# Amos-Chen98/neo-planner

Measured on AMD Instinct MI355X. Metric: trajectories/sec (batched replan), higher is better.
Workload: dtype f32x; 1 GPU; cfg2: 40 x 4096 trajectories x 20 waypoints per step per GPU, 1 x 300^3 f32 ESDF per GPU (trilinear, pillars + 80 canopy boxes), each optimised to L-BFGS-B termination; batch_per_launch=4096, pieces=21, dims=3, esdf_voxels=27000000, layout=brick, parallelism=scene-sharded x1, launches_in_flight_per_gpu=4

## Files before the change

include/neo_planner.h:

```cpp
#ifndef NEO_PLANNER_H
#define NEO_PLANNER_H

#include <stddef.h>
#include <stdint.h>

#ifdef __cplusplus
extern "C" {
#endif

#define NEO_ABI_VERSION 1
#define NEO_MAX_PIECES 64
#define NEO_MAX_DIM 3
#define NEO_LBFGS_M 10

typedef struct neo_ctx neo_ctx;

enum {
  NEO_OK = 0,
  NEO_ERR_INVALID = 1,
  NEO_ERR_HIP = 2,
  NEO_ERR_NO_MAP = 3,
  NEO_ERR_UNSUPPORTED = 4,
};

enum {
  NEO_TRAJ_CONVERGED_GRAD = 0,
  NEO_TRAJ_CONVERGED_F = 1,
  NEO_TRAJ_ABNORMAL = 2,
  NEO_TRAJ_MAXITER = 3,
  NEO_TRAJ_NUMERIC_RANGE = 4,
  NEO_TRAJ_NONFINITE = 5,
  NEO_TRAJ_BAD_SCENE = 6,
  NEO_TRAJ_SUSPENDED = 7,
};
#define NEO_TRAJ_FLAG_COLLISION 0x100

enum {
  NEO_INTERP_NEAREST_2D_REF = 0,
  NEO_INTERP_TRILINEAR_3D = 1,
};

enum { NEO_F64 = 0, NEO_F32 = 1, NEO_F16 = 2 };

enum {
  NEO_LAYOUT_LINEAR = 0,
  NEO_LAYOUT_YZ4 = 1,
  NEO_LAYOUT_CELL8 = 2,
  NEO_LAYOUT_BRICK = 3,
};

typedef struct neo_params {
  double v_max;
  double T_min;
  double T_max;
  double safe_dis;
  double delta_t;
  double weights[4];
  double collision_cost_tol;
  double ftol;
  double gtol;
  int32_t maxls;
  int32_t maxiter;
  int32_t maxfun;
  int32_t bugcompat_stale_T;
  int32_t sample_dtype;
  int32_t flags;
} neo_params;

#define NEO_FLAG_ONE_WAVE_PER_SIMD 32
#define NEO_FLAG_TWO_WAVES_PER_SIMD 64
#define NEO_FLAG_LANE_GROUPS 128
#define NEO_FLAG_F32_SOLVE 2048

int neo_abi_version(void);
int neo_ctx_create(int device_id, void *stream, neo_ctx **out);
int neo_ctx_destroy(neo_ctx *ctx);
const char *neo_last_error(neo_ctx *ctx);
int neo_params_default(neo_params *p);
int neo_params_set(neo_ctx *ctx, const neo_params *p);
int neo_ctx_synchronize(neo_ctx *ctx);
int neo_ctx_set_stream(neo_ctx *ctx, void *stream);

int neo_esdf_upload_2d(neo_ctx *ctx, int scene_id, const double *dist, const double *grad_x,
                       const double *grad_y, int width, int height, double resolution,
                       double origin_x, double origin_y);
int neo_esdf_build_2d(neo_ctx *ctx, int scene_id, const int8_t *occupancy, int width, int height,
                      double resolution, double origin_x, double origin_y, double *out_dist,
                      double *out_grad_x, double *out_grad_y);
int neo_esdf_build_2d_batch_dev(neo_ctx *ctx, const int32_t *scene_ids, int n, const int8_t *occupancy, int width,
                                int height, double resolution, const double *origins);
int neo_esdf_upload_3d(neo_ctx *ctx, int scene_id, const void *dist, int src_dtype,
                       int src_is_device, int nx, int ny, int nz, double resolution,
                       const double origin[3], int store_dtype, int layout);
int neo_esdf_build_3d(neo_ctx *ctx, int scene_id, const uint8_t *occupancy, int occ_is_device, int nx,
                      int ny, int nz, double resolution, const double origin[3], int store_dtype,
                      int layout, float *out_dist);
#define NEO_EDT_GENERIC_LINES 1
int neo_esdf_build_config(neo_ctx *ctx, int flags);
int neo_esdf_drop(neo_ctx *ctx, int scene_id);
int neo_esdf_query(neo_ctx *ctx, int scene_id, int n, const double *pts, double *dist, double *grad);

int neo_cost_grad_batch(neo_ctx *ctx, int scene_id, int B, int M, int D, const double *x,
                        const double *head, const double *tail, double *cost, double *costs4,
                        double *grad, double *coeffs, int32_t *status);
int neo_cost_grad_batch_dev(neo_ctx *ctx, int scene_id, int B, int M, int D, const double *x,
                            const double *head, const double *tail, double *cost, double *costs4,
                            double *grad, double *coeffs, int32_t *status);

int neo_sampled_terms_batch(neo_ctx *ctx, int scene_id, int B, int M, int D, const double *coeffs,
                            const double *ts, double *costs2, double *grad_C, double *grad_T);
int neo_sampled_terms_batch_dev(neo_ctx *ctx, int scene_id, int B, int M, int D, const double *coeffs,
                                const double *ts, double *costs2, double *grad_C, double *grad_T);
int neo_sampled_terms_batch_f32(neo_ctx *ctx, int scene_id, int B, int M, int D, const float *coeffs,
                                const double *ts, double *costs2, float *grad_C, float *grad_T);
int neo_sampled_terms_batch_f32_dev(neo_ctx *ctx, int scene_id, int B, int M, int D, const float *coeffs,
                                    const double *ts, double *costs2, float *grad_C, float *grad_T);

int neo_optimize_batch(neo_ctx *ctx, int scene_id, const int32_t *scene_ids, int B, int M, int D,
                       double *x, const double *head, const double *tail, double *costs4,
                       double *costs4_last, int32_t *nit, int32_t *nfev, int32_t *status);
int neo_optimize_batch_dev(neo_ctx *ctx, int scene_id, const int32_t *scene_ids, int B, int M,
                           int D, double *x, const double *head, const double *tail,
                           double *costs4, double *costs4_last, int32_t *nit, int32_t *nfev,
                           int32_t *status);
int neo_optimize_batch_from_dev(neo_ctx *ctx, int scene_id, const int32_t *scene_ids, int B, int M,
                                int D, const double *x0, double *x, const double *head,
                                const double *tail, double *costs4, double *costs4_last, int32_t *nit,
                                int32_t *nfev, int32_t *status);
size_t neo_optimize_state_bytes(int M, int D);
int neo_optimize_batch_budget_dev(neo_ctx *ctx, int scene_id, int B, int M, int D, const double *x0, double *x,
                                  const double *head, const double *tail, double *costs4, double *costs4_last,
                                  int32_t *nit, int32_t *nfev, int32_t *status, void *state, int eval_budget,
                                  const int32_t *subset, int n_subset, int resume);
int neo_scene_slot(neo_ctx *ctx, int scene_id);
size_t neo_optimize_workspace_bytes(int B, int M, int D);

int neo_eval_traj_batch(neo_ctx *ctx, int B, int M, int D, const double *x, const double *head,
                        const double *tail, double hz, int K, double *state, int32_t *count);

enum {
  NEO_AUDIT_PATH_LENGTH = 0,
  NEO_AUDIT_FEASIBILITY = 1,
  NEO_AUDIT_COLLISION = 2,
  NEO_AUDIT_WEIGHTED = 3,
  NEO_AUDIT_MIN_CLEARANCE = 4,
  NEO_AUDIT_T_MIN_CLEARANCE = 5,
  NEO_AUDIT_MAX_SPEED = 6,
  NEO_AUDIT_MAX_ACC = 7,
  NEO_AUDIT_T_FIRST_UNSAFE = 8,
  NEO_AUDIT_DURATION = 9,
  NEO_AUDIT_FIELDS = 10,
};
#define NEO_AUDIT_FLAG_UNSAFE 1
#define NEO_AUDIT_FLAG_METRIC_FAIL 2
#define NEO_AUDIT_FLAG_OUTSIDE_MAP 4
#define NEO_AUDIT_FLAG_NONFINITE 8
int neo_audit_traj_batch(neo_ctx *ctx, int scene_id, const int32_t *scene_ids, int B, int M, int D,
                         const double *x, const double *head, const double *tail, double hz,
                         const double *weights3, double *audit, int32_t *count, int32_t *flags);
int neo_audit_traj_batch_dev(neo_ctx *ctx, int scene_id, const int32_t *scene_ids, int B, int M, int D,
                             const double *x, const double *head, const double *tail, double hz,
                             const double *weights3, double *audit, int32_t *count, int32_t *flags);

#define NEO_GEO_FLAG_NO_PATH 1
#define NEO_GEO_FLAG_START_OUTSIDE 2
#define NEO_GEO_FLAG_CAPPED 4
#define NEO_GEO_FLAG_PATH_TRUNCATED 8
#define NEO_GEO_FLAG_BAD_SCENE 16
int neo_geo_search_batch(neo_ctx *ctx, int scene_id, const int32_t *scene_ids, int B, const double *start,
                         const double *target, int max_expansions, int path_cap, double *key_pts, double *path,
                         int32_t *path_len, double *path_cost, int32_t *expansions, int32_t *flags);
int neo_geo_search_batch_dev(neo_ctx *ctx, int scene_id, const int32_t *scene_ids, int B, const double *start,
                             const double *target, int max_expansions, int path_cap, double *key_pts, double *path,
                             int32_t *path_len, double *path_cost, int32_t *expansions, int32_t *flags);
int neo_geo_prune_batch(neo_ctx *ctx, int scene_id, const int32_t *scene_ids, int B, const double *paths,
                        const int32_t *path_len, int path_stride, double *key_pts);
int neo_geo_workspace_budget(neo_ctx *ctx, size_t bytes);

#define NEO_FLEET_FLAG_TARGET_CAPPED 1
#define NEO_FLEET_FLAG_CMD_FULL 2
#define NEO_FLEET_FLAG_BAD_SCENE 4
#define NEO_FLEET_FLAG_SPLICE_FAILED 8
#define NEO_FLEET_FLAG_ABANDONED 16
int neo_fleet_target_batch(neo_ctx *ctx, int scene_id, const int32_t *scene_ids, int B, const int32_t *subset,
                           int n_subset, const double *cur_pos, const double *goal, const double *jitter,
                           double longitu_step_dis, double lateral_step_length, double move_vel, double *tail,
                           int32_t *near_goal, int32_t *lateral_steps, int32_t *flags);
int neo_fleet_target_batch_dev(neo_ctx *ctx, int scene_id, const int32_t *scene_ids, int B, const int32_t *subset,
                               int n_subset, const double *cur_pos, const double *goal, const double *jitter,
                               double longitu_step_dis, double lateral_step_length, double move_vel, double *tail,
                               int32_t *near_goal, int32_t *lateral_steps, int32_t *flags);
int neo_fleet_advance_dev(neo_ctx *ctx, int B, const int32_t *subset, int n_subset, const double *cmd, int cap,
                          const int32_t *cmd_len, int32_t *cmd_index, int32_t *future_index, int step, int ahead,
                          double *cur_pos, double *head);
int neo_fleet_pose_dev(neo_ctx *ctx, int B, const int32_t *subset, int n_subset, const double *cmd, int cap,
                       const int32_t *cmd_len, const int32_t *cmd_index, const double *cur_pos, const double *goal,
                       double eye_z, double *pose);
int neo_fleet_splice_dev(neo_ctx *ctx, int B, const int32_t *subset, int n_subset, int M, const double *x,
                         const double *head, const double *tail, const int32_t *solved, double hz, int first,
                         double *cmd, int cap, int32_t *cmd_len, int32_t *cmd_index, int32_t *future_index,
                         int32_t *flags);
int neo_fleet_audit_batch(neo_ctx *ctx, int scene_id, const int32_t *scene_ids, int B, const int32_t *subset,
                          int n_subset, const double *cmd, int cap, const int32_t *n_flown, int stride, double cmd_hz,
                          const double *weights3, double *audit, int32_t *count, int32_t *flags);
int neo_fleet_audit_batch_dev(neo_ctx *ctx, int scene_id, const int32_t *scene_ids, int B, const int32_t *subset,
                              int n_subset, const double *cmd, int cap, const int32_t *n_flown, int stride,
                              double cmd_hz, const double *weights3, double *audit, int32_t *count, int32_t *flags);

int neo_record_state_dev(neo_ctx *ctx, int B, const int32_t *subset, int n_subset, const double *cmd, int cap,
                         const int32_t *cmd_len, const int32_t *cmd_index, const double *head, double *cur_vel);
int neo_record_commit_dev(neo_ctx *ctx, int B, const int32_t *subset, int n_subset, int M, const double *x,
                          const double *head, const double *tail, const int32_t *solved, const double *pose,
                          const double *cur_vel, const uint8_t *staging, int width, int height,
                          const int32_t *mission_ids, int tick, int round, int capacity, double *motion,
                          double *wpts_local, double *tau, double *pose_rows, int32_t *meta, uint8_t *images,
                          int32_t *row_of, int32_t *n_rows, int32_t *dropped);

#define NEO_BATCH_MAX_CANDIDATES 8
int neo_batch_candidates(neo_ctx *ctx, int B, const int32_t *subset, int n_subset, int M, int D, int K,
                         const double *head, const double *tail, const int32_t *slots, const double *tau,
                         const double *lateral_offsets, double *x0, double *head_k, double *tail_k, int32_t *slots_k);
int neo_batch_candidates_dev(neo_ctx *ctx, int B, const int32_t *subset, int n_subset, int M, int D, int K,
                             const double *head, const double *tail, const int32_t *slots, const double *tau,
                             const double *lateral_offsets, double *x0, double *head_k, double *tail_k,
                             int32_t *slots_k);
int neo_batch_select(neo_ctx *ctx, int B, const int32_t *subset, int n_subset, int M, int D, int K, const double *x_k,
                     const double *costs4_k, const double *costs4_last_k, const int32_t *nit_k, const int32_t *nfev_k,
                     const int32_t *status_k, const double *weights4, int32_t *chosen, double *cand_cost,
                     int32_t *solved, double *x, double *costs4, double *costs4_last, int32_t *nit, int32_t *nfev,
                     int32_t *status, int32_t *nit_total, int32_t *opt_runs, int32_t *fallback, int32_t *n_fallback);
int neo_batch_select_dev(neo_ctx *ctx, int B, const int32_t *subset, int n_subset, int M, int D, int K,
                         const double *x_k, const double *costs4_k, const double *costs4_last_k, const int32_t *nit_k,
                         const int32_t *nfev_k, const int32_t *status_k, const double *weights4, int32_t *chosen,
                         double *cand_cost, int32_t *solved, double *x, double *costs4, double *costs4_last,
                         int32_t *nit, int32_t *nfev, int32_t *status, int32_t *nit_total, int32_t *opt_runs,
                         int32_t *fallback, int32_t *n_fallback);

int neo_plan_guess(neo_ctx *ctx, int B, const int32_t *subset, int n_subset, int M, int D, const double *head,
                   const double *tail, const int32_t *slots, const double *x_init, const double *noise,
                   const double *frac, const double *tau, double *x0, double *head_k, double *tail_k, int32_t *slots_k);
int neo_plan_guess_dev(neo_ctx *ctx, int B, const int32_t *subset, int n_subset, int M, int D, const double *head,
                       const double *tail, const int32_t *slots, const double *x_init, const double *noise,
                       const double *frac, const double *tau, double *x0, double *head_k, double *tail_k,
                       int32_t *slots_k);
int neo_plan_merge(neo_ctx *ctx, int B, const int32_t *subset, int n_subset, int M, int D, int reset, const double *x_k,
                   const double *costs4_k, const double *costs4_last_k, const int32_t *nit_k, const int32_t *nfev_k,
                   const int32_t *status_k, double *x, double *costs4, double *costs4_last, int32_t *nit, int32_t *nfev,
                   int32_t *status, int32_t *attempts, int64_t *nit_total, int32_t *solved, int32_t *failed,
                   int32_t *n_failed, int32_t *bad_scene);
int neo_plan_merge_dev(neo_ctx *ctx, int B, const int32_t *subset, int n_subset, int M, int D, int reset,
                       const double *x_k, const double *costs4_k, const double *costs4_last_k, const int32_t *nit_k,
                       const int32_t *nfev_k, const int32_t *status_k, double *x, double *costs4, double *costs4_last,
                       int32_t *nit, int32_t *nfev, int32_t *status, int32_t *attempts, int64_t *nit_total,
                       int32_t *solved, int32_t *failed, int32_t *n_failed, int32_t *bad_scene);

#define NEO_DEPTH_MAX_BOXES 1024
int neo_depth_render_batch(neo_ctx *ctx, int width, int height, double focal_px, double max_range, const double *boxes,
                           const int32_t *box_begin, int n_scenes, const int32_t *scene_index, int B, const double *pose,
                           float *depth_m, uint8_t *depth_u8, float *depth_max);
int neo_depth_render_batch_dev(neo_ctx *ctx, int width, int height, double focal_px, double max_range,
                               const double *boxes, const int32_t *box_begin, int n_scenes, const int32_t *scene_index,
                               int B, const double *pose, float *depth_m, uint8_t *depth_u8, float *depth_max);
int neo_depth_box_test_counter(neo_ctx *ctx, uint64_t *dev_count);

int neo_onboard_integrate_batch(neo_ctx *ctx, int B, const int32_t *subset, int n_subset, const float *depth_m,
                                const double *pose, int width, int height, double focal_px, double max_range, int grid_w,
                                int grid_h, double res, const double *origins, double sensor_range, double z_lo,
                                double z_hi, int hit, int miss, int lo, int hi, int8_t *logodds, int8_t *occupancy,
                                int32_t *changed);
int neo_onboard_integrate_batch_dev(neo_ctx *ctx, int B, const int32_t *subset, int n_subset, const float *depth_m,
                                    const double *pose, int width, int height, double focal_px, double max_range,
                                    int grid_w, int grid_h, double res, const double *origins, double sensor_range,
                                    double z_lo, double z_hi, int hit, int miss, int lo, int hi, int8_t *logodds,
                                    int8_t *occupancy, int32_t *changed);

enum { NEO_KERNEL_EVAL = 0, NEO_KERNEL_OPTIMIZE = 1, NEO_KERNEL_ESDF_BUILD = 2, NEO_KERNEL_ESDF_SAMPLE = 3, NEO_KERNEL_COUNT = 4 };
int neo_profile_enable(neo_ctx *ctx, int on);
int neo_optimize_sample_counter(neo_ctx *ctx, int64_t *dev_counts);
int neo_optimize_progress_counter(neo_ctx *ctx, int32_t *counter);
int neo_optimize_trace(neo_ctx *ctx, double *dev_trace, int cap);
int neo_optimize_trace_xg(neo_ctx *ctx, double *dev_xg, int cap);
int neo_optimize_dispatch_order(neo_ctx *ctx, const int32_t *dev_order, int B);
size_t neo_effort_order_scratch_bytes(int B);
int neo_effort_order_dev(neo_ctx *ctx, int B, int M, int D, const double *x0, const double *head, const double *tail,
                         void *scratch, int32_t *order);
int neo_optimize_dispatch_order_host(neo_ctx *ctx, const int32_t *host_order, int B);
int neo_pack_results_dev(neo_ctx *ctx, int B, int n, const double *x, const double *costs4, const double *weights4,
                         float *out);
int neo_sampled_terms_dispatch_order(neo_ctx *ctx, const int32_t *order, int on_device, int B);
int neo_profile_read(neo_ctx *ctx, int kernel, int64_t *launches, double *total_ms);
int neo_profile_reset(neo_ctx *ctx);

#ifdef __cplusplus
}
#endif
#endif
```

neo-planner_amd/csrc/neo_abi.hip:

```cpp
#include <cstring>
#include "neo_host.hpp"
#include <rocprim/device/device_radix_sort.hpp>
#include "neo_kernels.hpp"

namespace neo {

template <int D>
__global__ __launch_bounds__(kWave) void traj_state_kernel(int B, int M, DevParams prm,
                                                            const double *__restrict__ x,
                                                            const double *__restrict__ head,
                                                            const double *__restrict__ tail, double hz, int K,
                                                            double *__restrict__ state, int *__restrict__ count) {
  __shared__ double xs[kSlots * kWave];
  __shared__ double cs[kWave * 6 * D];
  __shared__ double tcum[kWave + 1];
  const int b = blockIdx.x;
  if (b >= B) return;
  struct NoMap {};
  struct NoLookup {
    __device__ explicit NoLookup(const NoMap &) {}
  };
  DevParams p = prm;
  NoMap nm;
  DevBackend<D, kSlots, double, NoMap, NoLookup> be(p, nm);
// ... 1747 lines not shown
  HostStage st(c, kStagedUpTo);
  const RowRefs fk = stage_rows_in(st, a.packed, P, (size_t)a.n);
  const auto fsub = st.in_optional(subset, (size_t)n_subset);
  const RowRefs fo = stage_rows_inout(st, a.out, bs, (size_t)a.n);
  const auto oat = st.inout(attempts, bs);
  const auto ont = st.inout(nit_total, bs);
  const auto oso = st.inout(solved, bs);
  const auto ofl = st.out(failed, P), onl = st.out(n_failed, 1), obs = st.out(bad_scene, 1);
  rc = st.upload();
  if (rc) return rc;
  const RunRowsIn k = as_const(staged_rows(st, fk));
  const RunRows o = staged_rows(st, fo);
  rc = neo_plan_merge_dev(c, B, st.dev(fsub), n_subset, M, D, reset, k.x, k.costs4, k.costs4_last, k.nit, k.nfev, k.status, o.x,
                          o.costs4, o.costs4_last, o.nit, o.nfev, o.status, st.dev(oat), st.dev(ont), st.dev(oso), st.dev(ofl),
                          st.dev(onl), st.dev(obs));
  if (rc) return rc;
  return st.download();
}

static int geo_check(neo_ctx *c, int B, const double *start, const double *target, int max_expansions, int path_cap,
                     const double *key_pts, const double *path, const int32_t *path_len, const double *path_cost,
                     const int32_t *expansions, const int32_t *flags) {
  if (!c) return NEO_ERR_INVALID;
  if (B < 1) return fail_locked(c, NEO_ERR_INVALID, "geo: B must be >= 1");
  if (max_expansions < 0 || path_cap < 0 || (path && path_cap < 1))
    return fail_locked(c, NEO_ERR_INVALID, "geo: max_expansions and path_cap must be >= 0 (path_cap >= 1 with a path)");
  if (!start || !target || !key_pts || !path_len || !path_cost || !expansions || !flags)
    return fail_locked(c, NEO_ERR_INVALID, "geo: null buffer");
  return NEO_OK;
}

static int geo_scene_kind(neo_ctx *c, int scene_id) {
  auto it = c->maps.find(scene_id);
  if (it == c->maps.end()) return fail(c, NEO_ERR_NO_MAP, "geo: no ESDF for this scene");
  if (it->second.kind != 0) return fail(c, NEO_ERR_UNSUPPORTED, "geo: the A* warm start needs a 2-D map");
  return NEO_OK;
}

int neo_geo_search_batch_dev(neo_ctx *c, int scene_id, const int32_t *scene_ids, int B, const double *start,
                             const double *target, int max_expansions, int path_cap, double *key_pts, double *path,
                             int32_t *path_len, double *path_cost, int32_t *expansions, int32_t *flags) {
  int rc = geo_check(c, B, start, target, max_expansions, path_cap, key_pts, path, path_len, path_cost, expansions, flags);
  if (rc) return rc;
  std::lock_guard<std::recursive_mutex> g(c->mu);
  hipSetDevice(c->device);
  rc = rebuild_tables(c);
  if (rc) return rc;
  rc = geo_scene_kind(c, scene_id);
  if (rc) return rc;
  const GeoArgs ga{B, scene_ids, start, target, max_expansions, path ? path_cap : 0, key_pts, path, path_cost,
                   path_len, expansions, flags};
  return geo_search(c, scene_id, ga);
}

int neo_geo_search_batch(neo_ctx *c, int scene_id, const int32_t *scene_ids, int B, const double *start,
                         const double *target, int max_expansions, int path_cap, double *key_pts, double *path,
                         int32_t *path_len, double *path_cost, int32_t *expansions, int32_t *flags) {
  int rc = geo_check(c, B, start, target, max_expansions, path_cap, key_pts, path, path_len, path_cost, expansions, flags);
  if (rc) return rc;
  std::lock_guard<std::recursive_mutex> g(c->mu);
  hipSetDevice(c->device);
  rc = rebuild_tables(c);
  if (rc) return rc;
  const size_t bs = (size_t)B, pc = path ? (size_t)path_cap : 0;
  std::vector<int> slots;
  rc = scene_ids ? scene_slots(c, scene_ids, bs, true, slots) : geo_scene_kind(c, scene_id);
  if (rc) return rc;
  HostStage st(c, 0);
  const auto fs = st.in(start, 2 * bs), ft = st.in(target, 2 * bs);
  const auto fsl = st.in(scene_ids ? slots.data() : nullptr, bs);
  const auto fk = st.out(key_pts, 8 * bs), fc = st.out(path_cost, bs), fp = st.out(path, 2 * bs * pc);
  const auto fl = st.out(path_len, bs), fe = st.out(expansions, bs), ff = st.out(flags, bs);
  rc = st.upload();
  if (rc) return rc;
  rc = neo_geo_search_batch_dev(c, scene_ids ? scene_ids[0] : scene_id, scene_ids ? st.dev(fsl) : nullptr, B, st.dev(fs),
                                st.dev(ft), max_expansions, path_cap, st.dev(fk), path ? st.dev(fp) : nullptr, st.dev(fl),
                                st.dev(fc), st.dev(fe), st.dev(ff));
  if (rc) return rc;
  return st.download();
}

int neo_geo_prune_batch(neo_ctx *c, int scene_id, const int32_t *scene_ids, int B, const double *paths,
                        const int32_t *path_len, int path_stride, double *key_pts) {
  if (!c) return NEO_ERR_INVALID;
  if (B < 1 || path_stride < 1) return fail_locked(c, NEO_ERR_INVALID, "geo prune: B and path_stride must be >= 1");
  if (!paths || !path_len || !key_pts) return fail_locked(c, NEO_ERR_INVALID, "geo prune: null buffer");
  for (int i = 0; i < B; ++i)
    if (path_len[i] < 1 || path_len[i] > path_stride)
      return fail_locked(c, NEO_ERR_INVALID, "geo prune: path_len must be in [1, path_stride]");
  std::lock_guard<std::recursive_mutex> g(c->mu);
  hipSetDevice(c->device);
  int rc = rebuild_tables(c);
  if (rc) return rc;
  const size_t bs = (size_t)B, ps = (size_t)path_stride;
  std::vector<int> slots;
  rc = scene_ids ? scene_slots(c, scene_ids, bs, true, slots) : geo_scene_kind(c, scene_id);
  if (rc) return rc;
  HostStage st(c, 0);
  const auto fp = st.in(paths, 2 * bs * ps);
  const auto fl = st.in(path_len, bs), fsl = st.in(scene_ids ? slots.data() : nullptr, bs);
  const auto fk = st.out(key_pts, 8 * bs);
  rc = st.upload();
  if (rc) return rc;
  rc = geo_prune(c, scene_ids ? scene_ids[0] : scene_id, B, scene_ids ? st.dev(fsl) : nullptr, st.dev(fp), st.dev(fl),
                 path_stride, st.dev(fk));
  if (rc) return rc;
  return st.download();
}

int neo_geo_workspace_budget(neo_ctx *c, size_t bytes) {
  if (!c) return NEO_ERR_INVALID;
  std::lock_guard<std::recursive_mutex> g(c->mu);
  c->geo.budget = bytes;
  return NEO_OK;
}

int neo_optimize_progress_counter(neo_ctx *c, int32_t *counter) {
  if (!c) return NEO_ERR_INVALID;
  std::lock_guard<std::recursive_mutex> g(c->mu);
  c->progress = counter;
  return NEO_OK;
}

int neo_optimize_sample_counter(neo_ctx *c, int64_t *dev_counts) {
  if (!c) return NEO_ERR_INVALID;
  std::lock_guard<std::recursive_mutex> g(c->mu);
  c->sample_counter = reinterpret_cast<long long *>(dev_counts);
  return NEO_OK;
}

int neo_optimize_trace(neo_ctx *c, double *dev_trace, int cap) {
  if (!c || cap < 0) return NEO_ERR_INVALID;
  std::lock_guard<std::recursive_mutex> g(c->mu);
  if (dev_trace && cap > 0 && c->trace_xg && c->trace_cap != cap)
    return fail(c, NEO_ERR_INVALID, "neo_optimize_trace: cap differs from neo_optimize_trace_xg's");
  c->trace = (dev_trace && cap > 0) ? dev_trace : nullptr;
  if (c->trace) c->trace_cap = cap;
  if (!c->trace_xg && !c->trace) c->trace_cap = 0;
  return NEO_OK;
}

int neo_optimize_trace_xg(neo_ctx *c, double *dev_xg, int cap) {
  if (!c || cap < 0) return NEO_ERR_INVALID;
  std::lock_guard<std::recursive_mutex> g(c->mu);
  if (dev_xg && cap > 0 && c->trace && c->trace_cap != cap)
    return fail(c, NEO_ERR_INVALID, "neo_optimize_trace_xg: cap differs from neo_optimize_trace's");
  c->trace_xg = (dev_xg && cap > 0) ? dev_xg : nullptr;
  if (c->trace_xg) c->trace_cap = cap;
  if (!c->trace_xg && !c->trace) c->trace_cap = 0;
  return NEO_OK;
}

int neo_optimize_dispatch_order(neo_ctx *c, const int32_t *dev_order, int B) {
  if (!c || B < 0) return NEO_ERR_INVALID;
  std::lock_guard<std::recursive_mutex> g(c->mu);
  c->dispatch_order = (dev_order && B > 0) ? dev_order : nullptr;
  c->order_B = c->dispatch_order ? B : 0;
  return NEO_OK;
}

int neo_optimize_dispatch_order_host(neo_ctx *c, const int32_t *host_order, int B) {
  if (!c || B < 0) return NEO_ERR_INVALID;
  std::lock_guard<std::recursive_mutex> g(c->mu);
  hipSetDevice(c->device);
  if (!host_order || B == 0) {
    c->dispatch_order = nullptr;
    c->order_B = 0;
    return NEO_OK;
  }
  if ((size_t)B > c->order_cap) {
    HIPCHK(c, hipStreamSynchronize(c->stream));
    if (c->order_buf) hipFree(c->order_buf);
    c->order_buf = nullptr;
    c->order_cap = 0;
    HIPCHK(c, hipMalloc((void **)&c->order_buf, (size_t)B * sizeof(int)));
    c->order_cap = (size_t)B;
  }
  HIPCHK(c, hipMemcpyAsync(c->order_buf, host_order, (size_t)B * sizeof(int), hipMemcpyHostToDevice, c->stream));
  HIPCHK(c, hipStreamSynchronize(c->stream));
  c->dispatch_order = c->order_buf;
  c->order_B = B;
  return NEO_OK;
}

namespace neo {
__global__ void pack_results_kernel(int B, int n, const double *__restrict__ x, const double *__restrict__ costs4, double w0, double w1,
                                    double w2, double w3, float *__restrict__ out) {
  const size_t i = (size_t)blockIdx.x * blockDim.x + threadIdx.x;
  const size_t row = i / (size_t)(n + 5);
  if (row >= (size_t)B) return;
  const int col = (int)(i - row * (size_t)(n + 5));
  const double *c4 = costs4 + row * 4;
  double v;
  if (col < n)
    v = x[row * (size_t)n + col];
  else if (col == n)
    v = ((c4[0] * w0 + c4[1] * w1) + c4[2] * w2) + c4[3] * w3;
  else
    v = c4[col - n - 1];
  out[i] = (float)v;
}
}

int neo_pack_results_dev(neo_ctx *c, int B, int n, const double *x, const double *costs4, const double *weights4, float *out) {
  if (!c || B < 0 || n < 1) return NEO_ERR_INVALID;
  if (!x || !costs4 || !weights4 || !out) return fail_locked(c, NEO_ERR_INVALID, "null buffer");
  if (B == 0) return NEO_OK;
  std::lock_guard<std::recursive_mutex> g(c->mu);
  hipSetDevice(c->device);
  const size_t total = (size_t)B * (size_t)(n + 5);
  hipLaunchKernelGGL(neo::pack_results_kernel, dim3((unsigned)((total + 255) / 256)), dim3(256), 0, c->stream, B, n, x, costs4,
                     weights4[0], weights4[1], weights4[2], weights4[3], out);
  HIPCHK(c, hipGetLastError());
  return NEO_OK;
}

namespace neo {
__global__ void effort_keys_kernel(int B, int M, int D, double T_min, double T_max, double v_max, const double *__restrict__ x0,
                                   const double *__restrict__ head, const double *__restrict__ tail, double *__restrict__ keys,
                                   int *__restrict__ idx) {
  const int b = blockIdx.x * blockDim.x + threadIdx.x;
  if (b >= B) return;
  idx[b] = b;
  const int nq = D * (M - 1), n = nq + M;
  double sum = 0.0;
  for (int p = 0; p < M; ++p) sum += (T_max - T_min) / (1.0 + exp(-x0[(size_t)b * n + nq + p])) + T_min;
  double d2 = 0.0;
  for (int d = 0; d < D; ++d) {
    const double e = tail[(size_t)b * 3 * D + d] - head[(size_t)b * 3 * D + d];
    d2 += e * e;
  }
  const double dist = sqrt(d2);
  const double k = dist == dist ? sum * v_max / fmax(dist, 1e-9) : NAN;
  keys[b] = isfinite(k) ? k : 0.0;
}
}

static size_t effort_sort_temp_bytes(int B) {
  size_t tb = 0;
  (void)rocprim::radix_sort_pairs_desc(nullptr, tb, (const double *)nullptr, (double *)nullptr, (const int *)nullptr, (int *)nullptr,
                                       (unsigned)B, 0, 64, (hipStream_t)0);
  return (tb + 255) / 256 * 256;
}

static size_t align256(size_t v) { return (v + 255) / 256 * 256; }

size_t neo_effort_order_scratch_bytes(int B) {
  if (B <= 0) return 0;
  return align256((size_t)B * 16) + align256((size_t)B * 4) + effort_sort_temp_bytes(B);
}

int neo_effort_order_dev(neo_ctx *c, int B, int M, int D, const double *x0, const double *head, const double *tail, void *scratch,
                         int32_t *order) {
  int rc = check_shape(c, B, M, D);
  if (rc) return rc;
  if (!x0 || !head || !tail || !scratch || !order) return fail_locked(c, NEO_ERR_INVALID, "null buffer");
  if (((uintptr_t)scratch) & 255) return fail_locked(c, NEO_ERR_INVALID, "scratch must be 256-byte aligned");
  if (B == 0) return NEO_OK;
  std::lock_guard<std::recursive_mutex> g(c->mu);
  hipSetDevice(c->device);
  double *keys = static_cast<double *>(scratch), *keys_out = keys + B;
  int *idx = reinterpret_cast<int *>(reinterpret_cast<char *>(scratch) + align256((size_t)B * 16));
  void *temp = reinterpret_cast<char *>(idx) + align256((size_t)B * 4);
  size_t tb = effort_sort_temp_bytes(B);
  hipLaunchKernelGGL(neo::effort_keys_kernel, dim3((unsigned)((B + 255) / 256)), dim3(256), 0, c->stream, B, M, D, c->params.T_min,
                     c->params.T_max, c->params.v_max, x0, head, tail, keys, idx);
  HIPCHK(c, rocprim::radix_sort_pairs_desc(temp, tb, (const double *)keys, keys_out, (const int *)idx, (int *)order, (unsigned)B, 0, 64,
                                           c->stream));
  HIPCHK(c, hipGetLastError());
  return NEO_OK;
}

int neo_sampled_terms_dispatch_order(neo_ctx *c, const int32_t *order, int on_device, int B) {
  if (!c || B < 0) return NEO_ERR_INVALID;
  std::lock_guard<std::recursive_mutex> g(c->mu);
  hipSetDevice(c->device);
  if (!order || B == 0) {
    c->sample_order_B = 0;
    return NEO_OK;
  }
  if ((size_t)B > c->sample_order_cap) {
    HIPCHK(c, hipStreamSynchronize(c->stream));
    if (c->sample_order) hipFree(c->sample_order);
    c->sample_order = nullptr;
    c->sample_order_cap = 0;
    c->sample_order_B = 0;
    HIPCHK(c, hipMalloc((void **)&c->sample_order, (size_t)B * sizeof(int)));
    c->sample_order_cap = (size_t)B;
  }
  HIPCHK(c, hipMemcpyAsync(c->sample_order, order, (size_t)B * sizeof(int),
                           on_device ? hipMemcpyDeviceToDevice : hipMemcpyHostToDevice, c->stream));
  HIPCHK(c, hipStreamSynchronize(c->stream));
  c->sample_order_B = B;
  return NEO_OK;
}

int neo_esdf_build_config(neo_ctx *c, int flags) {
  if (!c || (flags & ~NEO_EDT_GENERIC_LINES)) return NEO_ERR_INVALID;
  std::lock_guard<std::recursive_mutex> g(c->mu);
  c->edt_flags = flags;
  return NEO_OK;
}

int neo_profile_enable(neo_ctx *c, int on) {
  if (!c) return NEO_ERR_INVALID;
  std::lock_guard<std::recursive_mutex> g(c->mu);
  c->profile = on != 0;
  return NEO_OK;
}

int neo_profile_read(neo_ctx *c, int kernel, int64_t *launches, double *total_ms) {
  if (!c || kernel < 0 || kernel >= NEO_KERNEL_COUNT) return NEO_ERR_INVALID;
  std::lock_guard<std::recursive_mutex> g(c->mu);
  hipSetDevice(c->device);
  drain_profile(c);
  if (launches) *launches = c->prof[kernel].launches;
  if (total_ms) *total_ms = c->prof[kernel].ms;
  return NEO_OK;
}

int neo_profile_reset(neo_ctx *c) {
  if (!c) return NEO_ERR_INVALID;
  std::lock_guard<std::recursive_mutex> g(c->mu);
  hipSetDevice(c->device);
  drain_profile(c);
  for (int k = 0; k < NEO_KERNEL_COUNT; ++k) {
    c->prof[k].launches = 0;
    c->prof[k].ms = 0.0;
  }
  return NEO_OK;
}

}
```

neo-planner_amd/csrc/neo_device.hpp:

```cpp
#pragma once
#include <type_traits>
#include <hip/hip_runtime.h>
#include <hip/hip_fp16.h>

#include "../../include/neo_planner.h"
#include "neo_wave.hpp"

namespace neo {

constexpr int kSlots = 4;

struct DevParams {
  double v_max, T_min, T_max, safe_dis, delta_t;
  double w[4];
  double coll_tol;
  double ftol, gtol;
  int maxls, maxiter, maxfun, stale_T;
  int dbg;
  struct F32 {
    float T_min, T_span;
    float dt, inv_dt;
    float vmax2, safe;
    float w[4];
  } f;
// ... 92 lines not shown
    if (!a.inside) return Real(10000);
    g[0] = (Real)q.r.y;
    g[1] = (Real)q.r.z;
    return (Real)q.r.x;
  }
  template <int D>
  __device__ __forceinline__ Real fetch(const Real (&pos)[D], Real (&g)[D], bool &inside) const {
    const Addr a = prepare<D>(pos);
    inside = a.inside;
    return finish<D>(a, load(a), g);
  }
};

template <typename E>
__device__ __forceinline__ float elem_to_float(E v);
template <>
__device__ __forceinline__ float elem_to_float<float>(float v) { return v; }
template <>
__device__ __forceinline__ float elem_to_float<__half>(__half v) { return __half2float(v); }

typedef unsigned long long u64_align4 __attribute__((aligned(4)));
typedef unsigned int u32_align2 __attribute__((aligned(2)));
template <typename E>
__device__ __forceinline__ void load_pair(const E *p, float &a, float &b);
template <>
__device__ __forceinline__ void load_pair<float>(const float *p, float &a, float &b) {
  const unsigned long long u = *reinterpret_cast<const u64_align4 *>(p);
  a = __uint_as_float((unsigned int)(u & 0xffffffffull));
  b = __uint_as_float((unsigned int)(u >> 32));
}
__device__ __forceinline__ void buffer_load_pair_f32(__amdgpu_buffer_rsrc_t rsrc, unsigned int off, unsigned int soff,
                                                     float &a, float &b) {
  const auto v = __builtin_amdgcn_raw_buffer_load_b64(rsrc, (int)off, (int)soff, 0);
  a = __uint_as_float(v[0]);
  b = __uint_as_float(v[1]);
}
template <>
__device__ __forceinline__ void load_pair<__half>(const __half *p, float &a, float &b) {
  const unsigned int u = *reinterpret_cast<const u32_align2 *>(p);
  a = __half2float(__ushort_as_half((unsigned short)(u & 0xffffu)));
  b = __half2float(__ushort_as_half((unsigned short)(u >> 16)));
}

template <typename Real, typename E, int LAYOUT>
struct Lookup3D {
  const Map3D &m;
  __amdgpu_buffer_rsrc_t rsrc;
  float inv, off[3], hi[3];
  __device__ __forceinline__ explicit Lookup3D(const Map3D &m_)
      : m(m_), rsrc(__builtin_amdgcn_make_buffer_rsrc(const_cast<void *>(m_.data), 0, (int)m_.bytes, 0x00020000)) {
    inv = m_.f_inv;
#pragma unroll
    for (int k = 0; k < 3; ++k) {
      off[k] = m_.f_off[k];
      hi[k] = m_.f_hi[k];
    }
  }
  struct Addr {
    int i0[3];
    Real fr[3];
    bool inside;
  };
  struct Raw {
    float c[2][2][2];
  };

  template <int D>
  __device__ __forceinline__ Addr prepare(const Real (&pos)[D], bool on = true) const {
#pragma clang fp contract(on)
    static_assert(D == 3, "the 3-D map needs D = 3");
    const int n[3] = {m.nx, m.ny, m.nz};
    const double org[3] = {m.ox, m.oy, m.oz};
    Addr a;
    a.inside = on;
    if constexpr (sizeof(Real) == 4) {
#pragma unroll
      for (int k = 0; k < 3; ++k) {
        const float um = fmaf(pos[k], inv, off[k]);
        if (!(um >= -0.5f && um < hi[k])) a.inside = false;
        const int i = min(max((int)floorf(um), 0), n[k] - 2);
        a.i0[k] = i;
        a.fr[k] = __builtin_amdgcn_fmed3f(um - (float)i, 0.0f, 1.0f);
      }
      if (!a.inside) a.i0[0] = a.i0[1] = a.i0[2] = 0;
      return a;
    }
#pragma unroll
    for (int k = 0; k < 3; ++k) {
      Real u = (Real)(((double)pos[k] - org[k]) * m.d_inv);
      if (!(u >= Real(0) && u < (Real)n[k])) a.inside = false;
      u -= Real(0.5);
      const int i = min(max((int)floor(u), 0), n[k] - 2);
      a.i0[k] = i;
      a.fr[k] = fmin(fmax(u - (Real)i, Real(0)), Real(1));
    }
    if (!a.inside) a.i0[0] = a.i0[1] = a.i0[2] = 0;
    return a;
  }
  __device__ __forceinline__ Raw load(const Addr &a) const {
    const E *vox = static_cast<const E *>(m.data);
    Raw q;
    if (LAYOUT == 2 || (LAYOUT == 9 && m.layout == NEO_LAYOUT_CELL8)) {
      const unsigned int cell = __umul24(__umul24((unsigned)a.i0[2], (unsigned)m.ny) + (unsigned)a.i0[1], (unsigned)m.nx) +
                                (unsigned)a.i0[0];
      if constexpr (sizeof(E) == 4) {
        const auto lo = __builtin_amdgcn_raw_buffer_load_b128(rsrc, (int)(cell * 32u), 0, 0);
        const auto hi = __builtin_amdgcn_raw_buffer_load_b128(rsrc, (int)(cell * 32u + 16u), 0, 0);
        q.c[0][0][0] = __uint_as_float(lo[0]); q.c[0][0][1] = __uint_as_float(lo[1]);
        q.c[0][1][0] = __uint_as_float(lo[2]); q.c[0][1][1] = __uint_as_float(lo[3]);
        q.c[1][0][0] = __uint_as_float(hi[0]); q.c[1][0][1] = __uint_as_float(hi[1]);
        q.c[1][1][0] = __uint_as_float(hi[2]); q.c[1][1][1] = __uint_as_float(hi[3]);
      } else {
        const auto v = __builtin_amdgcn_raw_buffer_load_b128(rsrc, (int)(cell * 16u), 0, 0);
#pragma unroll
        for (int w = 0; w < 4; ++w) {
          q.c[w >> 1][w & 1][0] = __half2float(__ushort_as_half((unsigned short)(v[w] & 0xffffu)));
          q.c[w >> 1][w & 1][1] = __half2float(__ushort_as_half((unsigned short)(v[w] >> 16)));
        }
      }
    } else if (LAYOUT == 3 || (LAYOUT == 9 && m.layout == NEO_LAYOUT_BRICK)) {
      constexpr int SHX = sizeof(E) == 4 ? 1 : 2, CX = (1 << SHX) + 1;
      const unsigned int bx = (unsigned)a.i0[0] >> SHX, by = (unsigned)a.i0[1] >> 1, bz = (unsigned)a.i0[2] >> 1;
      const unsigned int lx = (unsigned)a.i0[0] & ((1u << SHX) - 1u), ly = (unsigned)a.i0[1] & 1u, lz = (unsigned)a.i0[2] & 1u;
      const unsigned int blk = __umul24(__umul24(bz, (unsigned)m.nby) + by, (unsigned)m.nbx) + bx;
      const unsigned int in_line = (lz * 3u + ly) * (unsigned)CX + lx;
#pragma unroll
      for (int dz = 0; dz < 2; ++dz)
#pragma unroll
        for (int dy = 0; dy < 2; ++dy) {
          const unsigned int so = (unsigned)((dz * 3 + dy) * CX);
          if constexpr (sizeof(E) == 4) {
            const auto v = __builtin_amdgcn_raw_buffer_load_b64(rsrc, (int)(blk * 128u + in_line * 4u + so * 4u), 0, 0);
            q.c[dz][dy][0] = __uint_as_float(v[0]);
            q.c[dz][dy][1] = __uint_as_float(v[1]);
          } else {
            load_pair<E>(vox + blk * 64u + in_line + so, q.c[dz][dy][0], q.c[dz][dy][1]);
          }
        }
    } else if (LAYOUT == 0 || (LAYOUT == 9 && m.layout == NEO_LAYOUT_LINEAR)) {
      const unsigned int base = __umul24(__umul24((unsigned)a.i0[2], (unsigned)m.ny) + (unsigned)a.i0[1], (unsigned)m.nx) +
                                (unsigned)a.i0[0];
      const unsigned int sy = (unsigned)m.nx, sz = (unsigned)m.nx * (unsigned)m.ny;
#pragma unroll
      for (int dz = 0; dz < 2; ++dz)
#pragma unroll
        for (int dy = 0; dy < 2; ++dy) {
          const unsigned int so = (dy ? sy : 0u) + (dz ? sz : 0u);
          if constexpr (sizeof(E) == 4)
            buffer_load_pair_f32(rsrc, base * 4u, so * 4u, q.c[dz][dy][0], q.c[dz][dy][1]);
          else
            load_pair<E>(vox + base + so, q.c[dz][dy][0], q.c[dz][dy][1]);
        }
    } else {
      const unsigned int cell = __umul24(__umul24((unsigned)a.i0[2], (unsigned)m.ny) + (unsigned)a.i0[1], (unsigned)m.nx) +
                                (unsigned)a.i0[0];
      if constexpr (sizeof(E) == 4) {
        const auto lo = __builtin_amdgcn_raw_buffer_load_b128(rsrc, (int)(cell * 16u), 0, 0);
        const auto hi = __builtin_amdgcn_raw_buffer_load_b128(rsrc, (int)(cell * 16u + 16u), 0, 0);
        q.c[0][0][0] = __uint_as_float(lo[0]); q.c[0][1][0] = __uint_as_float(lo[1]);
        q.c[1][0][0] = __uint_as_float(lo[2]); q.c[1][1][0] = __uint_as_float(lo[3]);
        q.c[0][0][1] = __uint_as_float(hi[0]); q.c[0][1][1] = __uint_as_float(hi[1]);
        q.c[1][0][1] = __uint_as_float(hi[2]); q.c[1][1][1] = __uint_as_float(hi[3]);
      } else {
        const auto v = __builtin_amdgcn_raw_buffer_load_b128(rsrc, (int)(cell * 8u), 0, 0);
#pragma unroll
        for (int dx = 0; dx < 2; ++dx)
#pragma unroll
          for (int dz = 0; dz < 2; ++dz) {
            const unsigned int u = v[2 * dx + dz];
            q.c[dz][0][dx] = __half2float(__ushort_as_half((unsigned short)(u & 0xffffu)));
            q.c[dz][1][dx] = __half2float(__ushort_as_half((unsigned short)(u >> 16)));
          }
      }
    }
    return q;
  }
  template <int D>
  __device__ __forceinline__ Real finish(const Addr &a, const Raw &q, Real (&g)[D]) const {
#pragma clang fp contract(on)
#pragma unroll
    for (int d = 0; d < D; ++d) g[d] = Real(0);
    if (!a.inside) return Real(10000);
    const Real fx = a.fr[0], fy = a.fr[1], fz = a.fr[2];
    const Real inv_res = sizeof(Real) == 4 ? (Real)m.f_inv : (Real)m.d_inv;
    const Real c000 = (Real)q.c[0][0][0], c100 = (Real)q.c[0][0][1], c010 = (Real)q.c[0][1][0], c110 = (Real)q.c[0][1][1];
    const Real c001 = (Real)q.c[1][0][0], c101 = (Real)q.c[1][0][1], c011 = (Real)q.c[1][1][0], c111 = (Real)q.c[1][1][1];
    const Real dx00 = c100 - c000, dx10 = c110 - c010, dx01 = c101 - c001, dx11 = c111 - c011;
    const Real c00 = c000 + fx * dx00, c10 = c010 + fx * dx10;
    const Real c01 = c001 + fx * dx01, c11 = c011 + fx * dx11;
    const Real c0 = c00 + fy * (c10 - c00), c1 = c01 + fy * (c11 - c01);
    const Real dx0 = dx00 + fy * (dx10 - dx00), dx1 = dx01 + fy * (dx11 - dx01);
    const Real dy0 = c10 - c00, dy1 = c11 - c01;
    g[0] = (dx0 + fz * (dx1 - dx0)) * inv_res;
    g[1] = (dy0 + fz * (dy1 - dy0)) * inv_res;
    g[2] = (c1 - c0) * inv_res;
    return c0 + fz * (c1 - c0);
  }
  template <int D>
  __device__ __forceinline__ Real fetch(const Real (&pos)[D], Real (&g)[D], bool &inside) const {
    const Addr a = prepare<D>(pos);
    inside = a.inside;
    return finish<D>(a, load(a), g);
  }
};

__host__ __device__ __forceinline__ int sample_lanes_per_piece_fwd(int M);

struct WaveLanes {
  static constexpr int W = kWave;
  static constexpr int S = 1;
  static constexpr int dl(int D) { return D; }
  static __device__ __forceinline__ int lane() { return lane_id(); }
  static __device__ __forceinline__ int piece() { return lane_id(); }
  static __device__ __forceinline__ int dim0() { return 0; }
  static __device__ __forceinline__ int base() { return 0; }
  template <class T> static __device__ __forceinline__ T sum_dims(T v) { return v; }
  template <class T> static __device__ __forceinline__ T read(T v, int src ) { return rdlane(v, src); }
  template <class T> static __device__ __forceinline__ T prev(T v, T fill) { return from_prev(v, fill); }
  template <class T> static __device__ __forceinline__ T next(T v, T fill) { return from_next(v, fill); }
  template <class T> static __device__ __forceinline__ T sum(T v) { return wave_sum(v); }
  static __device__ __forceinline__ int any(int pred) { return __any(pred); }
  static __host__ __device__ __forceinline__ int lanes_per_piece(int M);
};

template <int W_>
struct GroupLanes {
  static_assert(W_ == 16 || W_ == 8, "a group is a DPP row or half of one");
  static constexpr int W = W_;
  static constexpr int S = 1;
  static constexpr int dl(int D) { return D; }
  static __device__ __forceinline__ int piece() { return lane_id() & (W - 1); }
  static __device__ __forceinline__ int dim0() { return 0; }
  static __device__ __forceinline__ int lane() { return lane_id() & (W - 1); }
  static __device__ __forceinline__ int base() { return lane_id() & ~(W - 1); }
  template <class T> static __device__ __forceinline__ T sum_dims(T v) { return v; }
  template <class T, class Op>
  static __device__ __forceinline__ T reduce(T v, Op op) {
    if constexpr (W == 16) {
      return __shfl(row_scan(v, op), base() + W - 1, kWave);
    } else {
      v = op(v, dpp<0xB1>(v)); v = op(v, dpp<0x4E>(v)); v = op(v, dpp<0x141>(v));
      return v;
    }
  }
  template <class T> static __device__ __forceinline__ T sum(T v) { return reduce(v, OpAdd()); }
  template <class T> static __device__ __forceinline__ T max_nonneg(T v) { return reduce(v, OpMax()); }
  static __device__ __forceinline__ int any(int pred) {
    return reduce(pred ? 1 : 0, [](int a, int b) { return a | b; });
  }
  template <class T>
  static __device__ __forceinline__ T read(T v, int src ) {
    return __shfl(v, base() + src, kWave);
  }
  template <class T> static __device__ __forceinline__ T prev(T v, T fill) {
    const T o = dpp<0x138>(v);
    return lane() == 0 ? fill : o;
  }
  template <class T> static __device__ __forceinline__ T next(T v, T fill) {
    const T o = dpp<0x130>(v);
    return lane() == W - 1 ? fill : o;
  }
  static __host__ __device__ __forceinline__ int lanes_per_piece(int M) {
    int L = W / M;
    if (L < 1) L = 1;
    if (L >= 8) L = (L >= 16 && W >= 16) ? 16 : 8;
    return L;
  }
};

template <int D_>
struct WaveLanesPD {
  static constexpr int W = kWave;
  static constexpr int S = D_;
  static constexpr int dl(int) { return 1; }
  static __device__ __forceinline__ int lane() { return lane_id(); }
  static __device__ __forceinline__ int base() { return 0; }
  static __device__ __forceinline__ int piece() { return (lane_id() * ((65536 + S - 1) / S)) >> 16; }
  static __device__ __forceinline__ int dim0() { return lane_id() - S * piece(); }
  template <class T> static __device__ __forceinline__ T read(T v, int q ) { return rdlane(v, S * q); }
  template <class T> static __device__ __forceinline__ T prev(T v, T fill) {
#pragma unroll
    for (int k = 0; k < S; ++k) v = dpp<0x138>(v);
    return lane_lt(S) ? fill : v;
  }
  template <class T> static __device__ __forceinline__ T next(T v, T fill) {
#pragma unroll
    for (int k = 0; k < S; ++k) v = dpp<0x130>(v);
    return lane_ge(kWave - S) ? fill : v;
  }
  template <class T> static __device__ __forceinline__ T sum(T v) { return wave_sum(v); }
  static __device__ __forceinline__ int any(int pred) { return __any(pred); }
  template <class T> static __device__ __forceinline__ T sum_dims(T v) {
    T acc = v, t = v;
#pragma unroll
    for (int k = 1; k < S; ++k) {
      t = dpp<0x130>(t);
      acc += t;
    }
    return acc;
  }
  static __host__ __device__ __forceinline__ int lanes_per_piece(int M) { return sample_lanes_per_piece_fwd(M); }
};

template <int D, int DL = D, typename Num = double>
struct Traj {
  int M, n, nq, L;
  Num T, tau;
  Num i1, i2, i3, i4;
  Num P0[DL], P1[DL];
  Num V0[DL], A0[DL], V1[DL], A1[DL];
  Num c[6][DL];
  int ns;
  Num N[2][2];
  const double *head, *tail;
  const Num *bnd;
  Num *pcr_xch = nullptr;
  Num *pcr_mult = nullptr;
};

template <int D, class LG, bool TAIL, int DL, typename Num>
__device__ __forceinline__ Num bstate(const Traj<D, DL, Num> &t, int k, int dl) {
  if constexpr (LG::S == 1 && LG::W == kWave)
    return (Num)(TAIL ? t.tail : t.head)[k * D + dl];
  else
    return t.bnd[((TAIL ? 3 : 0) + k) * D + (LG::S > 1 ? LG::dim0() : dl)];
}
template <int D, class LG, int DL, typename Num>
__device__ __forceinline__ void stage_boundary(Traj<D, DL, Num> &t, Num *lds) {
  if constexpr (LG::S > 1) {
    const int lane = lane_id();
    if (lane < 3 * D) lds[lane] = (Num)t.head[lane];
    if (lane < 3 * D) lds[3 * D + lane] = (Num)t.tail[lane];
    lds_wave_sync();
    t.bnd = lds;
  }
}

template <class LG = WaveLanes, typename Num = double>
__device__ __forceinline__ void thomas_factor(int M, const Num (&Lo)[2][2], const Num (&Di)[2][2],
                                              const Num (&Up)[2][2], Num (&N)[2][2], Num (&E)[2][2]) {
  const int lane = LG::piece();
#pragma unroll
  for (int i = 0; i < 2; ++i)
#pragma unroll
    for (int j = 0; j < 2; ++j) N[i][j] = E[i][j] = Num(0.0);
  for (int p = 1; p < M; ++p) {
    const Num e00 = LG::read(E[0][0], p - 1), e01 = LG::read(E[0][1], p - 1);
    const Num e10 = LG::read(E[1][0], p - 1), e11 = LG::read(E[1][1], p - 1);
    if (lane == p) {
      const Num h00 = fma(-Lo[0][1], e10, fma(-Lo[0][0], e00, Di[0][0]));
      const Num h01 = fma(-Lo[0][1], e11, fma(-Lo[0][0], e01, Di[0][1]));
      const Num h10 = fma(-Lo[1][1], e10, fma(-Lo[1][0], e00, Di[1][0]));
      const Num h11 = fma(-Lo[1][1], e11, fma(-Lo[1][0], e01, Di[1][1]));
      const Num det = fma(h00, h11, -(h01 * h10));
      const Num r = precise_rcp(det);
      N[0][0] = h11 * r;
      N[0][1] = -h01 * r;
      N[1][0] = -h10 * r;
      N[1][1] = h00 * r;
      E[0][0] = fma(N[0][0], Up[0][0], N[0][1] * Up[1][0]);
      E[0][1] = fma(N[0][0], Up[0][1], N[0][1] * Up[1][1]);
      E[1][0] = fma(N[1][0], Up[0][0], N[1][1] * Up[1][0]);
      E[1][1] = fma(N[1][0], Up[0][1], N[1][1] * Up[1][1]);
    }
  }
}

template <int DL, class LG = WaveLanes, typename Num = double>
__device__ __forceinline__ void thomas_solve(int M, const Num (&Lo)[2][2], const Num (&N)[2][2],
                                             const Num (&E)[2][2], const Num (&R)[2][DL],
                                             const Num (&y0)[2][DL], const Num (&yM)[2][DL],
                                             Num (&y)[2][DL]) {
  const int lane = LG::piece();
  Num A[2][2], b[2][DL];
  {
    const bool in = lane >= 1 && lane < M;
    A[0][0] = in ? -(N[0][0] * Lo[0][0] + N[0][1] * Lo[1][0]) : Num(0.0);
    A[0][1] = in ? -(N[0][0] * Lo[0][1] + N[0][1] * Lo[1][1]) : Num(0.0);
    A[1][0] = in ? -(N[1][0] * Lo[0][0] + N[1][1] * Lo[1][0]) : Num(0.0);
    A[1][1] = in ? -(N[1][0] * Lo[0][1] + N[1][1] * Lo[1][1]) : Num(0.0);
#pragma unroll
    for (int d = 0; d < DL; ++d) {
      const Num r0 = N[0][0] * R[0][d] + N[0][1] * R[1][d];
      const Num r1 = N[1][0] * R[0][d] + N[1][1] * R[1][d];
      b[0][d] = lane == 0 ? y0[0][d] : (in ? r0 : Num(0.0));
      b[1][d] = lane == 0 ? y0[1][d] : (in ? r1 : Num(0.0));
    }
  }
  for (int s = 1; s < M; s <<= 1) {
    Num As[2][2], bs[2][DL];
#pragma unroll
    for (int i = 0; i < 2; ++i) {
#pragma unroll
      for (int j = 0; j < 2; ++j) As[i][j] = __shfl_up(A[i][j], s * LG::S, kWave);
#pragma unroll
      for (int d = 0; d < DL; ++d) bs[i][d] = __shfl_up(b[i][d], s * LG::S, kWave);
    }
    if (lane >= s && lane < M) {
#pragma unroll
      for (int d = 0; d < DL; ++d) {
        const Num n0 = A[0][0] * bs[0][d] + A[0][1] * bs[1][d] + b[0][d];
        const Num n1 = A[1][0] * bs[0][d] + A[1][1] * bs[1][d] + b[1][d];
        b[0][d] = n0;
        b[1][d] = n1;
      }
      const Num a00 = A[0][0] * As[0][0] + A[0][1] * As[1][0], a01 = A[0][0] * As[0][1] + A[0][1] * As[1][1];
      const Num a10 = A[1][0] * As[0][0] + A[1][1] * As[1][0], a11 = A[1][0] * As[0][1] + A[1][1] * As[1][1];
      A[0][0] = a00; A[0][1] = a01; A[1][0] = a10; A[1][1] = a11;
    }
  }
  {
    const bool in = lane >= 1 && lane < M - 1;
#pragma unroll
    for (int d = 0; d < DL; ++d) {
      if (lane == M - 1) {
        b[0][d] -= E[0][0] * yM[0][d] + E[0][1] * yM[1][d];
        b[1][d] -= E[1][0] * yM[0][d] + E[1][1] * yM[1][d];
      }
    }
    A[0][0] = in ? -E[0][0] : Num(0.0);
    A[0][1] = in ? -E[0][1] : Num(0.0);
    A[1][0] = in ? -E[1][0] : Num(0.0);
    A[1][1] = in ? -E[1][1] : Num(0.0);
  }
  for (int s = 1; s < M; s <<= 1) {
    Num As[2][2], bs[2][DL];
#pragma unroll
    for (int i = 0; i < 2; ++i) {
#pragma unroll
      for (int j = 0; j < 2; ++j) As[i][j] = __shfl_down(A[i][j], s * LG::S, kWave);
#pragma unroll
      for (int d = 0; d < DL; ++d) bs[i][d] = __shfl_down(b[i][d], s * LG::S, kWave);
    }
    if (lane >= 1 && lane + s <= M - 1) {
#pragma unroll
      for (int d = 0; d < DL; ++d) {
        const Num n0 = A[0][0] * bs[0][d] + A[0][1] * bs[1][d] + b[0][d];
        const Num n1 = A[1][0] * bs[0][d] + A[1][1] * bs[1][d] + b[1][d];
        b[0][d] = n0;
        b[1][d] = n1;
      }
      const Num a00 = A[0][0] * As[0][0] + A[0][1] * As[1][0], a01 = A[0][0] * As[0][1] + A[0][1] * As[1][1];
      const Num a10 = A[1][0] * As[0][0] + A[1][1] * As[1][0], a11 = A[1][0] * As[0][1] + A[1][1] * As[1][1];
      A[0][0] = a00; A[0][1] = a01; A[1][0] = a10; A[1][1] = a11;
    }
  }
#pragma unroll
  for (int d = 0; d < DL; ++d) {
    y[0][d] = b[0][d];
    y[1][d] = b[1][d];
  }
}

template <int DL, class LG, typename Num>
__device__ __forceinline__ void pcr_solve(int M, Num (&L)[2][2], Num (&Dg)[2][2], Num (&U)[2][2], Num (&R)[2][DL],
                                          Num (&y)[2][DL], Num *mult = nullptr, Num *xch = nullptr) {
  static_assert(LG::W == kWave, "written for lane groups that span the wavefront");
  const int p = LG::piece();
  const bool in = p >= 1 && p < M;
#pragma unroll
  for (int i = 0; i < 2; ++i) {
#pragma unroll
    for (int j = 0; j < 2; ++j) {
      L[i][j] = in ? L[i][j] : Num(0.0);
      U[i][j] = in ? U[i][j] : Num(0.0);
      Dg[i][j] = in ? Dg[i][j] : Num(i == j ? 1.0 : 0.0);
    }
#pragma unroll
    for (int d = 0; d < DL; ++d) R[i][d] = in ? R[i][d] : Num(0.0);
  }
  const int lane = lane_id();
  const int s_end = sizeof(Num) == 4 ? min(M - 1, 32) : M - 1;
  typedef Num Quad __attribute__((ext_vector_type(4)));
  const bool writer = mult != nullptr && in && LG::dim0() == opaque_uniform(0);
  int level = 0;
  if constexpr (sizeof(Num) == 4) {
    typedef float f2 __attribute__((ext_vector_type(2)));
    auto fma2 = [](f2 x, f2 y, f2 z) { return __builtin_elementwise_fma(x, y, z); };
    f2 Lr[2] = {{L[0][0], L[0][1]}, {L[1][0], L[1][1]}}, Dr[2] = {{Dg[0][0], Dg[0][1]}, {Dg[1][0], Dg[1][1]}};
    f2 Ur[2] = {{U[0][0], U[0][1]}, {U[1][0], U[1][1]}}, Ir[2];
    auto invert = [&]() {
      const float det = fmaf(Dr[0].x, Dr[1].y, -(Dr[0].y * Dr[1].x));
      const float r = precise_rcp(det);
      Ir[0].x = Dr[1].y * r;
      Ir[0].y = -Dr[0].y * r;
      Ir[1].x = -Dr[1].x * r;
      Ir[1].y = Dr[0].x * r;
    };
    auto fetch = [&](const f2 v, int src) { return f2{__shfl(v.x, src, kWave), __shfl(v.y, src, kWave)}; };
    const bool keep = mult != nullptr;
    const int ps = min(p, M);
    for (int s = 1; s < s_end; s <<= 1, ++level) {
      invert();
      const int sp = lane - s * LG::S, sn = lane + s * LG::S;
      f2 Ip[2], Lp[2], Upv[2], In[2], Ln[2], Un[2];
      Num Rp[2][DL], Rn[2][DL];
      if (xch != nullptr) {
        Quad *tab = reinterpret_cast<Quad *>(xch);
        f2 *rx = reinterpret_cast<f2 *>(xch + (size_t)(M + 1) * 12);
        lds_wave_sync();
        tab[ps * 3 + 0] = Quad{Ir[0].x, Ir[0].y, Ir[1].x, Ir[1].y};
        tab[ps * 3 + 1] = Quad{Lr[0].x, Lr[0].y, Lr[1].x, Lr[1].y};
        tab[ps * 3 + 2] = Quad{Ur[0].x, Ur[0].y, Ur[1].x, Ur[1].y};
#pragma unroll
        for (int d = 0; d < DL; ++d) rx[lane * DL + d] = f2{R[0][d], R[1][d]};
        lds_wave_sync();
        const int pp = min(max(p - s, 0), M - 1), pn = min(p + s, M - 1);
        const Quad qi = tab[pp * 3 + 0], ql = tab[pp * 3 + 1], qu = tab[pp * 3 + 2];
        const Quad ni = tab[pn * 3 + 0], nl = tab[pn * 3 + 1], nu = tab[pn * 3 + 2];
        Ip[0] = qi.xy; Ip[1] = qi.zw; Lp[0] = ql.xy; Lp[1] = ql.zw; Upv[0] = qu.xy; Upv[1] = qu.zw;
        In[0] = ni.xy; In[1] = ni.zw; Ln[0] = nl.xy; Ln[1] = nl.zw; Un[0] = nu.xy; Un[1] = nu.zw;
#pragma unroll
        for (int d = 0; d < DL; ++d) {
          const f2 rp = rx[(sp & (kWave - 1)) * DL + d], rn = rx[(sn & (kWave - 1)) * DL + d];
          Rp[0][d] = rp.x; Rp[1][d] = rp.y;
          Rn[0][d] = rn.x; Rn[1][d] = rn.y;
        }
      } else {
#pragma unroll
        for (int i = 0; i < 2; ++i) {
          Ip[i] = fetch(Ir[i], sp);
          Upv[i] = fetch(Ur[i], sp);
          In[i] = fetch(Ir[i], sn);
          Ln[i] = fetch(Lr[i], sn);
          Lp[i] = fetch(Lr[i], sp);
          Un[i] = fetch(Ur[i], sn);
#pragma unroll
          for (int d = 0; d < DL; ++d) {
            Rp[i][d] = __shfl(R[i][d], sp, kWave);
            Rn[i][d] = __shfl(R[i][d], sn, kWave);
          }
        }
      }
      f2 pa[2], pg[2];
#pragma unroll
      for (int i = 0; i < 2; ++i) {
        pa[i] = fma2(Lr[i].xx, Ip[0], Lr[i].yy * Ip[1]);
        pg[i] = fma2(Ur[i].xx, In[0], Ur[i].yy * In[1]);
      }
      if (keep) {
        Quad *dst = reinterpret_cast<Quad *>(mult + ((size_t)level * (M + 1) + ps) * 8);
        dst[0] = Quad{pa[0].x, pa[0].y, pa[1].x, pa[1].y};
        dst[1] = Quad{pg[0].x, pg[0].y, pg[1].x, pg[1].y};
      }
#pragma unroll
      for (int i = 0; i < 2; ++i) {
        const f2 ai = -pa[i], gi = -pg[i];
        const f2 ln2 = fma2(ai.xx, Lp[0], ai.yy * Lp[1]);
        const f2 un2 = fma2(gi.xx, Un[0], gi.yy * Un[1]);
        Dr[i] = fma2(gi.yy, Ln[1], fma2(gi.xx, Ln[0], fma2(ai.yy, Upv[1], fma2(ai.xx, Upv[0], Dr[i]))));
#pragma unroll
        for (int d = 0; d < DL; ++d)
          R[i][d] = fmaf(gi.y, Rn[1][d], fmaf(gi.x, Rn[0][d], fmaf(ai.y, Rp[1][d], fmaf(ai.x, Rp[0][d], R[i][d]))));
        Lr[i] = ln2;
        Ur[i] = un2;
      }
    }
    invert();
    if (xch != nullptr) lds_wave_sync();
    if (keep) *reinterpret_cast<Quad *>(mult + (size_t)level * (M + 1) * 8 + (size_t)ps * 4) = Quad{Ir[0].x, Ir[0].y, Ir[1].x, Ir[1].y};
#pragma unroll
    for (int d = 0; d < DL; ++d) {
      y[0][d] = fmaf(Ir[0].x, R[0][d], Ir[0].y * R[1][d]);
      y[1][d] = fmaf(Ir[1].x, R[0][d], Ir[1].y * R[1][d]);
    }
    return;
  }
  Num I[2][2];
  auto invert = [&]() {
    const Num det = fma(Dg[0][0], Dg[1][1], -(Dg[0][1] * Dg[1][0]));
    const Num r = precise_rcp(det);
    I[0][0] = Dg[1][1] * r;
    I[0][1] = -Dg[0][1] * r;
    I[1][0] = -Dg[1][0] * r;
    I[1][1] = Dg[0][0] * r;
  };
  for (int s = 1; s < s_end; s <<= 1, ++level) {
    invert();
    const int lp = lane - s * LG::S, ln = lane + s * LG::S;
    const int sp = lp >= 0 ? lp : lane, sn = ln < kWave ? ln : lane;
    const bool last = 2 * s >= s_end;
    Num Ip[2][2], Lp[2][2], Upv[2][2], Rp[2][DL], In[2][2], Ln[2][2], Un[2][2], Rn[2][DL];
#pragma unroll
    for (int i = 0; i < 2; ++i) {
#pragma unroll
      for (int j = 0; j < 2; ++j) {
        Ip[i][j] = __shfl(I[i][j], sp, kWave);
        Upv[i][j] = __shfl(U[i][j], sp, kWave);
        In[i][j] = __shfl(I[i][j], sn, kWave);
        Ln[i][j] = __shfl(L[i][j], sn, kWave);
        Lp[i][j] = Un[i][j] = Num(0.0);
        if (!last) {
          Lp[i][j] = __shfl(L[i][j], sp, kWave);
          Un[i][j] = __shfl(U[i][j], sn, kWave);
        }
      }
#pragma unroll
      for (int d = 0; d < DL; ++d) {
        Rp[i][d] = __shfl(R[i][d], sp, kWave);
        Rn[i][d] = __shfl(R[i][d], sn, kWave);
      }
    }
    Num a[2][2], g[2][2];
#pragma unroll
    for (int i = 0; i < 2; ++i)
#pragma unroll
      for (int j = 0; j < 2; ++j) {
        a[i][j] = -fma(L[i][0], Ip[0][j], L[i][1] * Ip[1][j]);
        g[i][j] = -fma(U[i][0], In[0][j], U[i][1] * In[1][j]);
      }
    if (writer) {
      Quad *dst = reinterpret_cast<Quad *>(mult + ((size_t)level * (M + 1) + p) * 8);
      dst[0] = Quad{-a[0][0], -a[0][1], -a[1][0], -a[1][1]};
      dst[1] = Quad{-g[0][0], -g[0][1], -g[1][0], -g[1][1]};
    }
    Num Ln2[2][2], Un2[2][2];
#pragma unroll
    for (int i = 0; i < 2; ++i) {
#pragma unroll
      for (int j = 0; j < 2; ++j) {
        Ln2[i][j] = Un2[i][j] = Num(0.0);
        if (!last) {
          Ln2[i][j] = fma(a[i][0], Lp[0][j], a[i][1] * Lp[1][j]);
          Un2[i][j] = fma(g[i][0], Un[0][j], g[i][1] * Un[1][j]);
        }
        Dg[i][j] = fma(g[i][1], Ln[1][j], fma(g[i][0], Ln[0][j], fma(a[i][1], Upv[1][j], fma(a[i][0], Upv[0][j], Dg[i][j]))));
      }
#pragma unroll
      for (int d = 0; d < DL; ++d)
        R[i][d] = fma(g[i][1], Rn[1][d], fma(g[i][0], Rn[0][d], fma(a[i][1], Rp[1][d], fma(a[i][0], Rp[0][d], R[i][d]))));
    }
#pragma unroll
    for (int i = 0; i < 2; ++i)
#pragma unroll
      for (int j = 0; j < 2; ++j) {
        L[i][j] = Ln2[i][j];
        U[i][j] = Un2[i][j];
      }
  }
  invert();
  if (writer) *reinterpret_cast<Quad *>(mult + (size_t)level * (M + 1) * 8 + (size_t)p * 4) = Quad{I[0][0], I[0][1], I[1][0], I[1][1]};
#pragma unroll
  for (int d = 0; d < DL; ++d) {
    y[0][d] = fma(I[0][0], R[0][d], I[0][1] * R[1][d]);
    y[1][d] = fma(I[1][0], R[0][d], I[1][1] * R[1][d]);
  }
}

__host__ __device__ __forceinline__ int pcr_levels(int M, bool f32 = true) {
  const int s_end = f32 ? (M - 1 < 32 ? M - 1 : 32) : M - 1;
  int n = 0;
  for (int s = 1; s < s_end; s <<= 1) ++n;
  return n;
}
__host__ __device__ __forceinline__ int pcr_xch_elems(int M, int DL) { return (M + 1) * 12 + kWave * 2 * DL; }
__host__ __device__ __forceinline__ int pcr_mult_elems(int M) { return (pcr_levels(M) * 8 + 4) * (M + 1); }

template <int DL, class LG, typename Num>
__device__ __forceinline__ void pcr_solve_transposed(int M, const Num *mult, const Num (&R)[2][DL], Num (&y)[2][DL]) {
  static_assert(LG::W == kWave, "written for lane groups that span the wavefront");
  typedef Num Quad __attribute__((ext_vector_type(4)));
  const int p = LG::piece();
  const bool in = p >= 1 && p < M;
  const int pj = in ? p : 1;
  const int lane = lane_id();
  const int nlev = pcr_levels(M, sizeof(Num) == 4);
  Num w[2][DL];
  {
    const Quad I = *reinterpret_cast<const Quad *>(mult + (size_t)nlev * (M + 1) * 8 + (size_t)pj * 4);
#pragma unroll
    for (int d = 0; d < DL; ++d) {
      w[0][d] = in ? fma(I.x, R[0][d], I.z * R[1][d]) : Num(0.0);
      w[1][d] = in ? fma(I.y, R[0][d], I.w * R[1][d]) : Num(0.0);
    }
  }
  for (int k = nlev - 1; k >= 0; --k) {
    const int s = 1 << k;
    const Quad *src = reinterpret_cast<const Quad *>(mult + ((size_t)k * (M + 1) + pj) * 8);
    const Quad a = src[0], g = src[1];
    const int ln = lane + s * LG::S, lp = lane - s * LG::S;
    const bool hn = ln < kWave, hp = lp >= 0;
#pragma unroll
    for (int d = 0; d < DL; ++d) {
      const Num pa0 = fma(a.x, w[0][d], a.z * w[1][d]), pa1 = fma(a.y, w[0][d], a.w * w[1][d]);
      const Num qg0 = fma(g.x, w[0][d], g.z * w[1][d]), qg1 = fma(g.y, w[0][d], g.w * w[1][d]);
      const Num n0 = __shfl(pa0, hn ? ln : lane, kWave), n1 = __shfl(pa1, hn ? ln : lane, kWave);
      const Num m0 = __shfl(qg0, hp ? lp : lane, kWave), m1 = __shfl(qg1, hp ? lp : lane, kWave);
      if (in) {
        w[0][d] -= (hn ? n0 : Num(0.0)) + (hp ? m0 : Num(0.0));
        w[1][d] -= (hn ? n1 : Num(0.0)) + (hp ? m1 : Num(0.0));
      }
    }
  }
#pragma unroll
  for (int d = 0; d < DL; ++d) {
    y[0][d] = w[0][d];
    y[1][d] = w[1][d];
  }
}

template <class TrajT, typename Num>
__device__ __forceinline__ void joint_blocks(const TrajT &t, Num a1, Num a2, Num a3,
                                             Num (&Lo)[2][2], Num (&Di)[2][2], Num (&Up)[2][2]) {
  Lo[0][0] = -Num(24.0) * a2;  Lo[0][1] = -Num(3.0) * a1;
  Lo[1][0] = -Num(168.0) * a3; Lo[1][1] = -Num(24.0) * a2;
  Di[0][0] = -Num(36.0) * a2 + Num(36.0) * t.i2;    Di[0][1] = Num(9.0) * a1 + Num(9.0) * t.i1;
  Di[1][0] = -Num(192.0) * a3 - Num(192.0) * t.i3;  Di[1][1] = Num(36.0) * a2 - Num(36.0) * t.i2;
  Up[0][0] = Num(24.0) * t.i2;   Up[0][1] = -Num(3.0) * t.i1;
  Up[1][0] = -Num(168.0) * t.i3; Up[1][1] = Num(24.0) * t.i2;
}

template <int D, class LG = WaveLanes, typename Num = double, bool PCR = (sizeof(Num) == 4 && LG::W == kWave)>
__device__ __forceinline__ int minco_forward(Traj<D, LG::dl(D), Num> &t, const DevParams &prm, double &energy,
                                             double &time_sum) {
  constexpr int DL = LG::dl(D);
  const int lane = LG::piece();
  const bool act = lane < t.M;
  int bad = 0;
  {
    const Num tau = act ? t.tau : Num(0.0);
    if (-tau > Num(709.782712893384)) bad = 1;
    Num ex;
    if constexpr (sizeof(Num) == 8 || LG::W != kWave) {
      ex = exp(-tau);
      t.T = par_T_span<Num>(prm) / (Num(1.0) + ex) + par_T_min<Num>(prm);
    } else {
      ex = __expf(-tau);
      t.T = fmaf(par_T_span<Num>(prm), precise_rcp(Num(1.0) + ex), par_T_min<Num>(prm));
    }
    if constexpr (sizeof(Num) == 8) t.tau = ex; else t.tau = -tau;
  }
  if (LG::any(bad)) return 4;
  t.i1 = (sizeof(Num) == 8 || LG::W != kWave) ? Num(1.0) / t.T : precise_rcp(t.T);
  t.i2 = t.i1 * t.i1;
  t.i3 = t.i2 * t.i1;
  t.i4 = t.i2 * t.i2;
  if constexpr (sizeof(Num) == 8 || LG::W != kWave)
    t.ns = act ? (int)(t.T / par_dt<Num>(prm)) : 0;
  else
    t.ns = act ? (int)(t.T * par_inv_dt<Num>(prm)) : 0;

  if (t.M > 1) {
    Num Lo[2][2], Di[2][2], Up[2][2], E[2][2], R[2][DL], y0[2][DL], yM[2][DL], y[2][DL];
    const Num a1 = LG::prev(t.i1, Num(1.0)), a2 = a1 * a1, a3 = a2 * a1, a4 = a2 * a2;
    joint_blocks(t, a1, a2, a3, Lo, Di, Up);
    constexpr bool kPcr = PCR;
    if constexpr (!kPcr) thomas_factor<LG, Num>(NEO_DBG(prm, 2 | 8) ? 1 : t.M, Lo, Di, Up, t.N, E);
#pragma unroll
    for (int d = 0; d < DL; ++d) {
      const Num dPb = t.P1[d] - t.P0[d];
      const Num dPa = LG::prev(dPb, Num(0.0));
      R[0][d] = -(Num(60.0) * a3 * dPa - Num(60.0) * t.i3 * dPb);
      R[1][d] = -(Num(360.0) * a4 * dPa + Num(360.0) * t.i4 * dPb);
      y0[0][d] = bstate<D, LG, false>(t, 1, d);
      y0[1][d] = bstate<D, LG, false>(t, 2, d);
      yM[0][d] = bstate<D, LG, true>(t, 1, d);
      yM[1][d] = bstate<D, LG, true>(t, 2, d);
    }
    if constexpr (kPcr) {
#pragma unroll
      for (int d = 0; d < DL; ++d) {
        if (lane == 1) {
          R[0][d] -= Lo[0][0] * y0[0][d] + Lo[0][1] * y0[1][d];
          R[1][d] -= Lo[1][0] * y0[0][d] + Lo[1][1] * y0[1][d];
        }
        if (lane == t.M - 1) {
          R[0][d] -= Up[0][0] * yM[0][d] + Up[0][1] * yM[1][d];
          R[1][d] -= Up[1][0] * yM[0][d] + Up[1][1] * yM[1][d];
        }
      }
#pragma unroll
      for (int i = 0; i < 2; ++i)
#pragma unroll
        for (int j = 0; j < 2; ++j) {
          Lo[i][j] = lane == 1 ? Num(0.0) : Lo[i][j];
          Up[i][j] = lane == t.M - 1 ? Num(0.0) : Up[i][j];
        }
      NEO_MARK("fwd_pcr_begin");
      pcr_solve<DL, LG, Num>(t.M, Lo, Di, Up, R, y, t.pcr_mult, t.pcr_xch);
      NEO_MARK("fwd_pcr_end");
    } else {
      thomas_solve<DL, LG, Num>(NEO_DBG(prm, 2 | 16) ? 1 : t.M, Lo, t.N, E, R, y0, yM, y);
    }
#pragma unroll
    for (int d = 0; d < DL; ++d) {
      t.V0[d] = lane == 0 ? bstate<D, LG, false>(t, 1, d) : y[0][d];
      t.A0[d] = lane == 0 ? bstate<D, LG, false>(t, 2, d) : y[1][d];
    }
  } else {
#pragma unroll
    for (int d = 0; d < DL; ++d) {
      t.V0[d] = bstate<D, LG, false>(t, 1, d);
      t.A0[d] = bstate<D, LG, false>(t, 2, d);
    }
  }
#pragma unroll
  for (int d = 0; d < DL; ++d) {
    const Num v1 = LG::next(t.V0[d], Num(0.0)), a1 = LG::next(t.A0[d], Num(0.0));
    t.V1[d] = (lane == t.M - 1) ? bstate<D, LG, true>(t, 1, d) : v1;
    t.A1[d] = (lane == t.M - 1) ? bstate<D, LG, true>(t, 2, d) : a1;
  }
  Num e = Num(0.0);
  const Num T = t.T, T2 = T * T, T3 = T2 * T, T4 = T2 * T2, T5 = T4 * T;
#pragma unroll
  for (int d = 0; d < DL; ++d) {
    const Num ep = t.P1[d] - t.P0[d] - T * t.V0[d] - Num(0.5) * T2 * t.A0[d];
    const Num ev = t.V1[d] - t.V0[d] - T * t.A0[d];
    const Num ea = t.A1[d] - t.A0[d];
    t.c[0][d] = t.P0[d];
    t.c[1][d] = t.V0[d];
    t.c[2][d] = Num(0.5) * t.A0[d];
    t.c[3][d] = (Num(10.0) * ep - Num(4.0) * T * ev + Num(0.5) * T2 * ea) * t.i3;
    t.c[4][d] = (-Num(15.0) * ep + Num(7.0) * T * ev - T2 * ea) * t.i4;
    t.c[5][d] = (Num(6.0) * ep - Num(3.0) * T * ev + Num(0.5) * T2 * ea) * t.i4 * t.i1;
    const Num c3 = t.c[3][d], c4 = t.c[4][d], c5 = t.c[5][d];
    e += Num(36.0) * T * c3 * c3 + Num(144.0) * T2 * c3 * c4 + Num(240.0) * T3 * c3 * c5 + Num(192.0) * T3 * c4 * c4 +
         Num(720.0) * T4 * c4 * c5 + Num(720.0) * T5 * c5 * c5;
  }
  energy = LG::sum(act ? e : Num(0.0));
  time_sum = LG::sum((act && LG::dim0() == opaque_uniform(0)) ? t.T : Num(0.0));
  return 0;
}

template <typename Real, int D>
__device__ __forceinline__ void piece_pos_vel(const Real (&c)[6][D], Real s, Real (&pos)[D], Real (&vel)[D]) {
#pragma clang fp contract(on)
#pragma unroll
  for (int d = 0; d < D; ++d) {
    if constexpr (sizeof(Real) == 4) {
      Real a = c[5][d], b = c[5][d];
      a = fmaf(a, s, c[4][d]); b = fmaf(b, s, a);
      a = fmaf(a, s, c[3][d]); b = fmaf(b, s, a);
      a = fmaf(a, s, c[2][d]); b = fmaf(b, s, a);
      a = fmaf(a, s, c[1][d]); b = fmaf(b, s, a);
      a = fmaf(a, s, c[0][d]);
      pos[d] = a;
      vel[d] = b;
    } else {
      pos[d] = c[0][d] + s * (c[1][d] + s * (c[2][d] + s * (c[3][d] + s * (c[4][d] + s * c[5][d]))));
      vel[d] = c[1][d] + s * (Real(2) * c[2][d] + s * (Real(3) * c[3][d] + s * (Real(4) * c[4][d] + s * (Real(5) * c[5][d]))));
    }
  }
}

__host__ __device__ __forceinline__ int sample_lanes_per_piece(int M) {
  int L = kWave / M;
  if (L < 1) L = 1;
  if (L >= 8) L = L >= 64 ? 64 : (L >= 32 ? 32 : (L >= 16 ? 16 : 8));
  return L;
}

__host__ __device__ __forceinline__ int WaveLanes::lanes_per_piece(int M) { return sample_lanes_per_piece(M); }
__host__ __device__ __forceinline__ int sample_lanes_per_piece_fwd(int M) { return sample_lanes_per_piece(M); }

template <typename Real, int N>
__device__ __forceinline__ void fold_piece_lanes(Real (&v)[N], int L, int r) {
  if (L <= 4) {
    Real t[N];
#pragma unroll
    for (int q = 0; q < N; ++q) t[q] = v[q];
    for (int i = 1; i < L; ++i) {
#pragma unroll
      for (int q = 0; q < N; ++q) {
        t[q] = dpp<0x130>(t[q]);
        v[q] += t[q];
      }
    }
    return;
  }
  if ((L & (L - 1)) == 0) {
    if (L >= 16) {
#pragma unroll
      for (int q = 0; q < N; ++q) v[q] += dpp<0x108>(v[q]);
    }
#pragma unroll
    for (int q = 0; q < N; ++q) {
      v[q] += dpp<0x104>(v[q]);
      v[q] += dpp<0x102>(v[q]);
      v[q] += dpp<0x101>(v[q]);
    }
    if (L >= 32) {
#pragma unroll
      for (int q = 0; q < N; ++q) v[q] += __shfl_down(v[q], 16, kWave);
    }
    if (L >= 64) {
#pragma unroll
      for (int q = 0; q < N; ++q) v[q] += __shfl_down(v[q], 32, kWave);
    }
    return;
  }
  for (int sft = 1; sft < L; sft <<= 1) {
#pragma unroll
    for (int q = 0; q < N; ++q) {
      const Real o = __shfl_down(v[q], sft, kWave);
      if (r + sft < L) v[q] += o;
    }
  }
}

struct SampleLanes {
  int piece;
  int r;
  int L;
  bool act;
  int rounds;
  int lmax;
  int first;
  int Lp;
  int total;
};

template <class LG>
__device__ __forceinline__ SampleLanes fixed_sample_lanes(int M, int L, int ns_of_my_piece_if_known = -1) {
  (void)ns_of_my_piece_if_known;
  const int lane = LG::lane();
  SampleLanes sl;
  sl.piece = (lane * ((65536 + L - 1) / L)) >> 16;
  sl.r = lane - sl.piece * L;
  sl.L = L;
  sl.act = sl.piece < M;
  sl.rounds = -1;
  sl.lmax = 0;
  sl.first = lane * L;
  sl.Lp = L;
  sl.total = -1;
  return sl;
}

template <class LG>
__device__ __forceinline__ SampleLanes group_sample_lanes(int M, int ns_piece) {
  constexpr int W = LG::W;
  const int L0 = W / M, extra = W - M * L0;
  if (extra == 0) return fixed_sample_lanes<LG>(M, L0);
  const int lane = LG::lane();
  const int base = LG::base();
  const int mine = lane < M ? ns_piece : -1;
  int rank = 0;
  for (int q = 0; q < M; ++q) {
    const int o = __shfl(mine, base + q, kWave);
    rank += (o > mine || (o == mine && q < lane)) ? 1 : 0;
  }
  const int Lp = lane < M ? L0 + (rank < extra ? 1 : 0) : 0;
  SampleLanes sl;
  sl.piece = 0;
  sl.r = 0;
  sl.L = L0;
  sl.first = 0;
  int acc = 0;
  for (int q = 0; q < M; ++q) {
    const int lq = __shfl(Lp, base + q, kWave);
    if (q == lane) sl.first = acc;
    if (lane >= acc && lane < acc + lq) {
      sl.piece = q;
      sl.r = lane - acc;
      sl.L = lq;
    }
    acc += lq;
  }
  sl.act = lane < acc;
  sl.rounds = -1;
  sl.lmax = L0 + 1;
  sl.Lp = Lp;
  sl.total = -1;
  return sl;
}

__device__ __forceinline__ SampleLanes balanced_sample_lanes(int M, int ns_piece, int *seg) {
  const int lane = lane_id();
  lds_wave_sync();
  const int mine = lane < M ? ns_piece : 0;
  const int total = wave_sum(mine);
  int R = max(1, (total + kWave - 1) / kWave);
  int Lp = 0;
  for (;;) {
    const float fr = (float)R;
    Lp = mine > 0 ? (int)(((float)mine + fr - 0.5f) * __builtin_amdgcn_rcpf(fr)) : 0;
    if (wave_sum(Lp) <= kWave) break;
    ++R;
  }
  const int incl = wave_scan_add(Lp);
  const int start = incl - Lp;
  seg[lane] = 0;
  lds_wave_sync();
  if (Lp > 0) seg[start] = ((lane + 1) << 16) | (Lp << 8) | start;
  lds_wave_sync();
  const int key = wave_scan_max_nonneg(seg[lane]);
  lds_wave_sync();
  SampleLanes sl;
  sl.piece = max((key >> 16) - 1, 0);
  sl.L = max((key >> 8) & 0xff, 1);
  sl.r = lane - (key & 0xff);
  sl.act = key != 0 && sl.r < sl.L;
  sl.rounds = R;
  sl.lmax = wave_max_nonneg(Lp);
  sl.first = start;
  sl.Lp = Lp;
  sl.total = total;
  return sl;
}

template <typename Real, int N>
__device__ __forceinline__ void fold_piece_segments(Real (&v)[N], int r, int L, int lmax) {
  for (int sft = 1; sft < lmax; sft <<= 1) {
#pragma unroll
    for (int q = 0; q < N; ++q) {
      const Real o = __shfl_down(v[q], sft, kWave);
      if (r + sft < L) v[q] += o;
    }
  }
}

template <typename Real, int D, class LookupT>
__device__ __forceinline__ void sample_accumulate(const Real (&c)[6][D], int j, int ns, Real s, Real inv_ns, const Real (&vel)[D],
                                                  Real vv, Real vd, const LookupT &lk, const typename LookupT::Addr &ad,
                                                  const typename LookupT::Raw &rw, Real dt, Real w2, Real w3, Real (&aC)[6][D],
                                                  Real &aT, Real &aF, Real &aK) {
#pragma clang fp contract(on)
  const Real omg = (j == 0 || j == ns - 1) ? Real(0.5) : Real(1);
  const Real s2 = s * s, s3 = s2 * s, s4 = s2 * s2, s5 = s4 * s;
  if (vv > Real(0)) {
    const Real vq = vv;
    aF += omg * dt * vq * vq * vq;
    Real av = Real(0);
#pragma unroll
    for (int d = 0; d < D; ++d) {
      const Real acc = Real(2) * c[2][d] + s * (Real(6) * c[3][d] + s * (Real(12) * c[4][d] + s * (Real(20) * c[5][d])));
      av += acc * vel[d];
    }
    const Real dK = Real(3) * dt * omg * vq * vq;
    const Real b1[6] = {Real(0), Real(1), Real(2) * s, Real(3) * s2, Real(4) * s3, Real(5) * s4};
#pragma unroll
    for (int d = 0; d < D; ++d) {
      const Real uu = w2 * dK * Real(2) * vel[d];
#pragma unroll
      for (int k = 1; k < 6; ++k) aC[k][d] += b1[k] * uu;
    }
    aT += w2 * (omg * vq * vq * vq * inv_ns + dK * Real(2) * av * (Real)j * inv_ns);
  }
  if (vd > Real(0)) {
    Real g[D];
    (void)lk.template finish<D>(ad, rw, g);
    const Real vq = vd;
    aK += omg * dt * vq * vq * vq;
    const Real dK = Real(3) * dt * omg * vq * vq;
    const Real b0[6] = {Real(1), s, s2, s3, s4, s5};
    Real gv = Real(0);
#pragma unroll
    for (int d = 0; d < D; ++d) {
      gv += g[d] * vel[d];
      const Real uu = -(w3 * dK * g[d]);
#pragma unroll
      for (int k = 0; k < 6; ++k) aC[k][d] += b0[k] * uu;
    }
    aT += w3 * (omg * vq * vq * vq * inv_ns + dK * (-gv) * (Real)j * inv_ns);
  }
}

__host__ __device__ constexpr int fold_acc_stride(int D) { return (6 * D + 1 + 3) / 4 * 4; }

template <typename Real, int D, class LookupT, int U, bool SAMPLE_IO = false, class LG = WaveLanes>
__device__ __forceinline__ void minco_sample(int M, const SampleLanes &sl, int ns_in, const Real (&cp)[6][LG::dl(D)],
                                             const DevParams &prm, const LookupT &lk, Real (&gC)[6][LG::dl(D)], Real &gT,
                                             double &cost_feas, double &cost_coll, Real *fold_rows = nullptr,
                                             bool fold_acc = false) {
#pragma clang fp contract(on)
  const int lane = LG::lane();
  const int piece = sl.piece, r = sl.r, L = sl.L;
  const bool act = sl.act;
  Real c[6][D];
  int ns;
  if constexpr (SAMPLE_IO) {
#pragma unroll
    for (int k = 0; k < 6; ++k)
#pragma unroll
      for (int d = 0; d < D; ++d) c[k][d] = cp[k][d];
    ns = act ? ns_in : 0;
  } else {
#pragma unroll
    for (int k = 0; k < 6; ++k)
#pragma unroll
      for (int d = 0; d < D; ++d) {
        if constexpr (LG::S == 1)
          c[k][d] = __shfl(cp[k][d], LG::base() + piece, kWave);
        else
          c[k][d] = __shfl(cp[k][0], LG::S * piece + d, kWave);
      }
    const int ns_sh = __shfl(ns_in, LG::base() + LG::S * piece, kWave);
    ns = act ? ns_sh : 0;
  }
  const int iters = NEO_DBG(prm, 1) ? 0 : (sl.rounds >= 0 ? sl.rounds : wave_max_nonneg((ns + L - 1) / L));

  const Real dt = par_dt<Real>(prm), vmax2 = par_vmax2<Real>(prm), safe = par_safe<Real>(prm);
  const Real w2 = par_w2<Real>(prm), w3 = par_w3<Real>(prm);
  Real inv_ns;
  if constexpr (sizeof(Real) == 4 && LG::W == kWave)
    inv_ns = ns > 0 ? __builtin_amdgcn_rcpf((float)ns) : Real(0);
  else
    inv_ns = ns > 0 ? Real(1) / (Real)ns : Real(0);
  Real aC[6][D];
#pragma unroll
  for (int k = 0; k < 6; ++k)
#pragma unroll
    for (int d = 0; d < D; ++d) aC[k][d] = Real(0);
  Real aT = Real(0), aF = Real(0), aK = Real(0);

  NEO_MARK("loop_begin");
  for (int it0 = 0; it0 < iters; it0 += U) {
    Real sv[U], vel[U][D];
    typename LookupT::Addr ad[U];
    typename LookupT::Raw rw[U];
    bool on[U];
    if constexpr (SAMPLE_IO)
      if (r + it0 * L >= ns) continue;
    constexpr bool kVelLate = SAMPLE_IO && sizeof(Real) == 4;
#pragma unroll
    for (int u = 0; u < U; ++u) {
      const int j = r + (it0 + u) * L;
      on[u] = j < ns;
      const Real s = (Real)((double)j * prm.delta_t);
      sv[u] = s;
      Real pos[D];
      if constexpr (kVelLate) {
#pragma unroll
        for (int d = 0; d < D; ++d)
          pos[d] = fmaf(fmaf(fmaf(fmaf(fmaf(c[5][d], s, c[4][d]), s, c[3][d]), s, c[2][d]), s, c[1][d]), s, c[0][d]);
      } else {
        piece_pos_vel<Real, D>(c, s, pos, vel[u]);
      }
      ad[u] = lk.template prepare<D>(pos, on[u]);
    }
#pragma unroll
    for (int u = 0; u < U; ++u) rw[u] = lk.load(ad[u]);
    if constexpr (kVelLate) {
#pragma unroll
      for (int u = 0; u < U; ++u) {
        Real pos[D];
        piece_pos_vel<Real, D>(c, sv[u], pos, vel[u]);
      }
    }
    Real vv[U], vd[U];
    bool any_violation = false;
#pragma unroll
    for (int u = 0; u < U; ++u) {
      Real v2 = Real(0);
#pragma unroll
      for (int d = 0; d < D; ++d) v2 += vel[u][d] * vel[u][d];
      vv[u] = v2 - vmax2;
      Real gdrop[D];
      vd[u] = safe - lk.template finish<D>(ad[u], rw[u], gdrop);
      if (on[u] && (vv[u] > Real(0) || vd[u] > Real(0))) any_violation = true;
    }
    if (any_violation) {
#pragma unroll
      for (int u = 0; u < U; ++u) {
        if (!on[u]) continue;
        sample_accumulate<Real, D, LookupT>(c, r + (it0 + u) * L, ns, sv[u], inv_ns, vel[u], vv[u], vd[u], lk, ad[u], rw[u], dt, w2,
                                            w3, aC, aT, aF, aK);
      }
    }
  }
  NEO_MARK("loop_end");
  if constexpr (sizeof(Real) == 4 && !SAMPLE_IO && LG::S > 1) {
    if (fold_rows != nullptr && fold_acc && sl.lmax != 0) {
      typedef Real Quad __attribute__((ext_vector_type(4)));
      constexpr int RS = fold_acc_stride(D), NQ = RS / 4;
      Quad v[NQ];
      {
        Real f[RS];
#pragma unroll
        for (int q = 0; q < RS; ++q) f[q] = Real(0);
#pragma unroll
        for (int d = 0; d < D; ++d)
#pragma unroll
          for (int k = 0; k < 6; ++k) f[d * 6 + k] = aC[k][d];
        f[6 * D] = aT;
#pragma unroll
        for (int q = 0; q < NQ; ++q) v[q] = Quad{f[4 * q], f[4 * q + 1], f[4 * q + 2], f[4 * q + 3]};
      }
      Quad *mine = reinterpret_cast<Quad *>(fold_rows + (size_t)(act ? piece : 0) * RS);
      lds_wave_sync();
      for (int i = 0; i < sl.lmax; ++i) {
        if (act && r == i) {
          if (i == 0) {
#pragma unroll
            for (int q = 0; q < NQ; ++q) mine[q] = v[q];
          } else {
#pragma unroll
            for (int q = 0; q < NQ; ++q) mine[q] = mine[q] + v[q];
          }
        }
        lds_wave_sync();
      }
      {
        const int pc = LG::piece();
        const int Lp = __shfl(sl.Lp, pc < M ? pc : 0, kWave);
        const bool have = pc < M && Lp > 0;
        typedef Real Pair __attribute__((ext_vector_type(2), may_alias));
        const Pair *src = reinterpret_cast<const Pair *>(fold_rows + (size_t)(have ? pc : 0) * RS + LG::dim0() * 6);
        const Pair p0 = src[0], p1 = src[1], p2 = src[2];
        const Real tpart = fold_rows[(size_t)(have ? pc : 0) * RS + 6 * D];
        gC[0][0] = have ? p0.x : Real(0); gC[1][0] = have ? p0.y : Real(0);
        gC[2][0] = have ? p1.x : Real(0); gC[3][0] = have ? p1.y : Real(0);
        gC[4][0] = have ? p2.x : Real(0); gC[5][0] = have ? p2.y : Real(0);
        gT = have ? tpart : Real(0);
      }
      lds_wave_sync();
      cost_feas = (double)LG::sum(act ? aF : Real(0));
      cost_coll = (double)LG::sum(act ? aK : Real(0));
      return;
    }
  }
  if constexpr (sizeof(Real) == 4) {
    if (fold_rows != nullptr && sl.lmax != 0) {
      typedef Real Quad __attribute__((ext_vector_type(4)));
      constexpr int DR = LG::dl(D);
      Quad *row = reinterpret_cast<Quad *>(fold_rows + (size_t)lane * (8 * D));
#pragma unroll
      for (int d = 0; d < D; ++d) {
        row[2 * d] = Quad{aC[0][d], aC[1][d], aC[2][d], aC[3][d]};
        row[2 * d + 1] = Quad{aC[4][d], aC[5][d], aT, Real(0)};
      }
      lds_wave_sync();
      int first, Lp, dim_base = 0;
      if constexpr (SAMPLE_IO) {
        first = lane;
        Lp = (act && r == 0) ? L : 0;
      } else {
        first = sl.first;
        Lp = sl.Lp;
        if constexpr (LG::S > 1) {
          first = __shfl(sl.first, LG::piece(), kWave);
          Lp = __shfl(sl.Lp, LG::piece(), kWave);
        }
        if (LG::piece() >= M) Lp = 0;
        dim_base = LG::dim0();
      }
      Quad lo[DR], hi[DR];
#pragma unroll
      for (int dd = 0; dd < DR; ++dd) lo[dd] = hi[dd] = Quad{Real(0), Real(0), Real(0), Real(0)};
      const Quad *src = reinterpret_cast<const Quad *>(fold_rows + (size_t)first * (8 * D)) + 2 * dim_base;
      for (int i = 0; i < sl.lmax; ++i) {
        if (i < Lp) {
#pragma unroll
          for (int dd = 0; dd < DR; ++dd) {
            lo[dd] += src[i * 2 * D + 2 * dd];
            hi[dd] += src[i * 2 * D + 2 * dd + 1];
          }
        }
      }
      lds_wave_sync();
#pragma unroll
      for (int dd = 0; dd < DR; ++dd) {
        gC[0][dd] = lo[dd].x; gC[1][dd] = lo[dd].y; gC[2][dd] = lo[dd].z; gC[3][dd] = lo[dd].w;
        gC[4][dd] = hi[dd].x; gC[5][dd] = hi[dd].y;
      }
      gT = hi[0].z;
      cost_feas = (double)LG::sum(act ? aF : Real(0));
      cost_coll = (double)LG::sum(act ? aK : Real(0));
      return;
    }
  }
  Real fv[6 * D + 3];
#pragma unroll
  for (int k = 0; k < 6; ++k)
#pragma unroll
    for (int d = 0; d < D; ++d) fv[k * D + d] = aC[k][d];
  fv[6 * D] = aT;
  fv[6 * D + 1] = aF;
  fv[6 * D + 2] = aK;
  if (sl.lmax == 0)
    fold_piece_lanes<Real, 6 * D + 3>(fv, L, r);
  else
    fold_piece_segments<Real, 6 * D + 3>(fv, r, L, sl.lmax);
  if constexpr (!SAMPLE_IO) {
    int src = LG::base() + sl.first;
    if constexpr (LG::S > 1) src = __shfl(sl.first, LG::piece(), kWave);
#pragma unroll
    for (int q = 0; q < 6 * D + 3; ++q) fv[q] = __shfl(fv[q], src, kWave);
  }
  if constexpr (LG::S == 1) {
#pragma unroll
    for (int k = 0; k < 6; ++k)
#pragma unroll
      for (int d = 0; d < D; ++d) gC[k][d] = fv[k * D + d];
  } else {
    const int dm = LG::dim0();
#pragma unroll
    for (int k = 0; k < 6; ++k) {
      Real v = fv[k * D];
#pragma unroll
      for (int j = 1; j < D; ++j) v = (dm == j) ? fv[k * D + j] : v;
      gC[k][0] = v;
    }
  }
  gT = fv[6 * D];
  const Real pf = fv[6 * D + 1], pk = fv[6 * D + 2];
  const bool mine = SAMPLE_IO ? (act && r == 0) : (LG::piece() < M && LG::dim0() == opaque_uniform(0));
  cost_feas = LG::sum(mine ? (double)pf : 0.0);
  cost_coll = LG::sum(mine ? (double)pk : 0.0);
}

template <int D, class LG = WaveLanes, typename Num = double, bool PCR = (sizeof(Num) == 4 && LG::W == kWave)>
__device__ __forceinline__ int minco_backward(const Traj<D, LG::dl(D), Num> &t, const DevParams &prm,
                                              Num (&gC)[6][LG::dl(D)], Num gT, Num (&gq)[LG::dl(D)], Num &gtau) {
  constexpr int DL = LG::dl(D);
  const int lane = LG::piece();
  const int M = t.M;
  int pow_overflow = 0;
  const Num a1 = LG::prev(t.i1, Num(1.0)), a2 = a1 * a1, a3 = a2 * a1, a4 = a2 * a2;
  const Num T = t.T, T2 = T * T, T3 = T2 * T, T4 = T2 * T2, T5 = T4 * T;
  const Num w0 = par_w0<Num>(prm);
  Num jerk_end[DL], snap_end[DL], crackle[DL];
  gT = (LG::dim0() == opaque_uniform(0)) ? gT + par_w1<Num>(prm) : Num(0.0);
#pragma unroll
  for (int d = 0; d < DL; ++d) {
    const Num c3 = t.c[3][d], c4 = t.c[4][d], c5 = t.c[5][d];
    gC[3][d] += Num(2.0) * w0 * (Num(36.0) * T * c3 + Num(72.0) * T2 * c4 + Num(120.0) * T3 * c5);
    gC[4][d] += Num(2.0) * w0 * (Num(72.0) * T2 * c3 + Num(192.0) * T3 * c4 + Num(360.0) * T4 * c5);
    gC[5][d] += Num(2.0) * w0 * (Num(120.0) * T3 * c3 + Num(360.0) * T4 * c4 + Num(720.0) * T5 * c5);
    jerk_end[d] = Num(6.0) * c3 + Num(24.0) * T * c4 + Num(60.0) * T2 * c5;
    snap_end[d] = Num(24.0) * c4 + Num(120.0) * T * c5;
    crackle[d] = Num(120.0) * c5;
    if constexpr (sizeof(Num) == 8) {
      if (lane < M && fabs(jerk_end[d]) > Num(1.3407807929942596e154)) pow_overflow = 1;
    } else {
      if (lane < M && !(fabs(jerk_end[d]) <= Num(3.4028234663852886e38))) pow_overflow = 1;
    }
    gT += w0 * jerk_end[d] * jerk_end[d];
  }
  Num gz[6][DL];
#pragma unroll
  for (int d = 0; d < DL; ++d) {
    const Num gep = Num(10.0) * gC[3][d] * t.i3 - Num(15.0) * gC[4][d] * t.i4 + Num(6.0) * gC[5][d] * t.i4 * t.i1;
    const Num gev = -Num(4.0) * gC[3][d] * t.i2 + Num(7.0) * gC[4][d] * t.i3 - Num(3.0) * gC[5][d] * t.i4;
    const Num gea = Num(0.5) * gC[3][d] * t.i1 - gC[4][d] * t.i2 + Num(0.5) * gC[5][d] * t.i3;
    gz[0][d] = gC[0][d] - gep;
    gz[1][d] = gC[1][d] - T * gep - gev;
    gz[2][d] = Num(0.5) * gC[2][d] - Num(0.5) * T2 * gep - T * gev - gea;
    gz[3][d] = gep;
    gz[4][d] = gev;
    gz[5][d] = gea;
  }
  Num S[3][DL];
#pragma unroll
  for (int k = 0; k < 3; ++k)
#pragma unroll
    for (int d = 0; d < DL; ++d) S[k][d] = LG::prev(gz[3 + k][d], Num(0.0)) + gz[k][d];

  Num lam[2][DL];
#pragma unroll
  for (int d = 0; d < DL; ++d) lam[0][d] = lam[1][d] = Num(0.0);
  constexpr bool kPcr = PCR;
  if constexpr (kPcr) {
    if (M > 1 && t.pcr_mult != nullptr) {
      Num R[2][DL], y[2][DL];
#pragma unroll
      for (int d = 0; d < DL; ++d) {
        R[0][d] = S[1][d];
        R[1][d] = S[2][d];
      }
      NEO_MARK("bwd_pcr_begin");
      pcr_solve_transposed<DL, LG, Num>(M, t.pcr_mult, R, y);
      NEO_MARK("bwd_pcr_end");
#pragma unroll
      for (int d = 0; d < DL; ++d) {
        lam[0][d] = (lane >= 1 && lane < M) ? y[0][d] : Num(0.0);
        lam[1][d] = (lane >= 1 && lane < M) ? y[1][d] : Num(0.0);
      }
    } else if (M > 1) {
      Num LoT[2][2], DiT[2][2], UpT[2][2], R[2][DL], y[2][DL];
      LoT[0][0] = Num(24.0) * a2;  LoT[0][1] = -Num(168.0) * a3;
      LoT[1][0] = -Num(3.0) * a1;  LoT[1][1] = Num(24.0) * a2;
      DiT[0][0] = -Num(36.0) * a2 + Num(36.0) * t.i2;  DiT[0][1] = -Num(192.0) * a3 - Num(192.0) * t.i3;
      DiT[1][0] = Num(9.0) * a1 + Num(9.0) * t.i1;     DiT[1][1] = Num(36.0) * a2 - Num(36.0) * t.i2;
      UpT[0][0] = -Num(24.0) * t.i2;  UpT[0][1] = -Num(168.0) * t.i3;
      UpT[1][0] = -Num(3.0) * t.i1;   UpT[1][1] = -Num(24.0) * t.i2;
#pragma unroll
      for (int i = 0; i < 2; ++i)
#pragma unroll
        for (int j = 0; j < 2; ++j) {
          LoT[i][j] = lane == 1 ? Num(0.0) : LoT[i][j];
          UpT[i][j] = lane == M - 1 ? Num(0.0) : UpT[i][j];
        }
#pragma unroll
      for (int d = 0; d < DL; ++d) {
        R[0][d] = S[1][d];
        R[1][d] = S[2][d];
      }
      NEO_MARK("bwd_pcr_begin");
      pcr_solve<DL, LG, Num>(M, LoT, DiT, UpT, R, y);
      NEO_MARK("bwd_pcr_end");
#pragma unroll
      for (int d = 0; d < DL; ++d) {
        lam[0][d] = (lane >= 1 && lane < M) ? y[0][d] : Num(0.0);
        lam[1][d] = (lane >= 1 && lane < M) ? y[1][d] : Num(0.0);
      }
    }
  } else if (M > 1) {
    Num LoT[2][2], NT[2][2], ET[2][2], R[2][DL], z0[2][DL], y[2][DL];
    LoT[0][0] = Num(24.0) * a2;  LoT[0][1] = -Num(168.0) * a3;
    LoT[1][0] = -Num(3.0) * a1;  LoT[1][1] = Num(24.0) * a2;
    NT[0][0] = t.N[0][0]; NT[0][1] = t.N[1][0]; NT[1][0] = t.N[0][1]; NT[1][1] = t.N[1][1];
    {
      const Num u00 = -Num(24.0) * t.i2, u01 = -Num(168.0) * t.i3;
      const Num u10 = -Num(3.0) * t.i1, u11 = -Num(24.0) * t.i2;
      ET[0][0] = NT[0][0] * u00 + NT[0][1] * u10;
      ET[0][1] = NT[0][0] * u01 + NT[0][1] * u11;
      ET[1][0] = NT[1][0] * u00 + NT[1][1] * u10;
      ET[1][1] = NT[1][0] * u01 + NT[1][1] * u11;
    }
#pragma unroll
    for (int d = 0; d < DL; ++d) {
      R[0][d] = S[1][d];
      R[1][d] = S[2][d];
      z0[0][d] = z0[1][d] = Num(0.0);
    }
    thomas_solve<DL, LG, Num>(NEO_DBG(prm, 2 | 16) ? 1 : M, LoT, NT, ET, R, z0, z0, y);
#pragma unroll
    for (int d = 0; d < DL; ++d) {
      lam[0][d] = (lane >= 1 && lane < M) ? y[0][d] : Num(0.0);
      lam[1][d] = (lane >= 1 && lane < M) ? y[1][d] : Num(0.0);
    }
  }
  Num Gt[3][DL];
#pragma unroll
  for (int d = 0; d < DL; ++d) {
    const Num l1 = lam[0][d], l2 = lam[1][d];
    const Num dp_prev = -Num(60.0) * a3 * l1 - Num(360.0) * a4 * l2;
    const Num dp_here = (Num(60.0) * a3 + Num(60.0) * t.i3) * l1 + (Num(360.0) * a4 - Num(360.0) * t.i4) * l2;
    const Num dp_next = -Num(60.0) * t.i3 * l1 + Num(360.0) * t.i4 * l2;
    const Num from_left = LG::prev(dp_next, Num(0.0));
    const Num from_right = LG::next(dp_prev, Num(0.0));
    gq[d] = S[0][d] - dp_here - (lane >= 2 ? from_left : Num(0.0)) - (lane + 1 <= M - 1 ? from_right : Num(0.0));
    const Num lt1 = (M > 1) ? l1 : Num(0.0), lt2 = (M > 1) ? l2 : Num(0.0);
    Gt[0][d] = gz[3][d] - (-Num(60.0) * t.i3 * lt1 + Num(360.0) * t.i4 * lt2);
    Gt[1][d] = gz[4][d] - (Num(24.0) * t.i2 * lt1 - Num(168.0) * t.i3 * lt2);
    Gt[2][d] = gz[5][d] - (-Num(3.0) * t.i1 * lt1 + Num(24.0) * t.i2 * lt2);
  }
  Num gTt = gT;
#pragma unroll
  for (int d = 0; d < DL; ++d) {
    const Num v1 = t.V1[d], a1 = t.A1[d], je = jerk_end[d];
    gTt -= gz[3][d] * v1 + gz[4][d] * a1 + gz[5][d] * je;
    const Num ln1 = LG::next(lam[0][d], Num(0.0)), ln2 = LG::next(lam[1][d], Num(0.0));
    if (lane + 1 <= M - 1) {
      const Num d_je = snap_end[d] - (Num(60.0) * t.i3 * v1 - Num(36.0) * t.i2 * a1 + Num(9.0) * t.i1 * je);
      const Num d_se = crackle[d] - (Num(360.0) * t.i4 * v1 - Num(192.0) * t.i3 * a1 + Num(36.0) * t.i2 * je);
      gTt -= ln1 * d_je + ln2 * d_se;
    }
    if (lane >= 1) {
      const Num d_js = -(Num(60.0) * t.i3 * v1 - Num(24.0) * t.i2 * a1 + Num(3.0) * t.i1 * je);
      const Num d_ss = -(-Num(360.0) * t.i4 * v1 + Num(168.0) * t.i3 * a1 - Num(24.0) * t.i2 * je);
      gTt += lam[0][d] * d_js + lam[1][d] * d_ss;
    }
  }
  {
    const Num Ts = LG::prev(T, T);
    if (prm.stale_T && M >= 2 && lane == M - 1) {
      const Num S2 = Ts * Ts, S3 = S2 * Ts, S4 = S2 * S2;
#pragma unroll
      for (int d = 0; d < DL; ++d) {
        const Num c1 = t.c[1][d], c2 = t.c[2][d], c3 = t.c[3][d], c4 = t.c[4][d], c5 = t.c[5][d];
        const Num velL = c1 + Num(2.0) * T * c2 + Num(3.0) * T2 * c3 + Num(4.0) * T3 * c4 + Num(5.0) * T4 * c5;
        const Num velS = c1 + Num(2.0) * Ts * c2 + Num(3.0) * S2 * c3 + Num(4.0) * S3 * c4 + Num(5.0) * S4 * c5;
        const Num accL = Num(2.0) * c2 + Num(6.0) * T * c3 + Num(12.0) * T2 * c4 + Num(20.0) * T3 * c5;
        const Num accS = Num(2.0) * c2 + Num(6.0) * Ts * c3 + Num(12.0) * S2 * c4 + Num(20.0) * S3 * c5;
        const Num jrkL = Num(6.0) * c3 + Num(24.0) * T * c4 + Num(60.0) * T2 * c5;
        const Num jrkS = Num(6.0) * c3 + Num(24.0) * Ts * c4 + Num(60.0) * S2 * c5;
        gTt += Gt[0][d] * (velL - velS) + Gt[1][d] * (accL - accS) + Gt[2][d] * (jrkL - jrkS);
      }
    }
  }
  if constexpr (sizeof(Num) == 8) {
    const Num ex = t.tau;
    if (lane < M && (Num(1.0) + ex) > Num(1.3407807929942596e154)) pow_overflow = 1;
    gtau = LG::sum_dims(gTt) * (Num(prm.T_max) - Num(prm.T_min)) * ex / ((Num(1.0) + ex) * (Num(1.0) + ex));
  } else {
    const Num nt = t.tau;
    if (lane < M && nt > Num(354.891356446692)) pow_overflow = 1;
    Num ex, s;
    if constexpr (LG::W == kWave) {
      ex = fmin(__expf(nt), Num(3.4028234663852886e38));
      s = precise_rcp(Num(1.0) + ex);
    } else {
      ex = fmin(exp(nt), Num(3.4028234663852886e38));
      s = Num(1.0) / (Num(1.0) + ex);
    }
    gtau = LG::sum_dims(gTt) * par_T_span<Num>(prm) * ((ex * s) * s);
  }
  return LG::any(pow_overflow) ? 4 : 0;
}

}
```

neo-planner_amd/csrc/neo_host.hpp:

```cpp
#pragma once
#include <hip/hip_runtime.h>

#include <algorithm>
#include <cmath>
#include <cstdint>
#include <cstdio>
#include <cstring>
#include <map>
#include <mutex>
#include <string>
#include <vector>

#include "../../include/neo_planner.h"
#include "neo_device.hpp"
#include "neo_launch_list.hpp"

namespace neo {
struct MapEntry {
  int kind = -1;
  int elem = NEO_F64;
  void *data = nullptr;
  Map2D m2{};
  Map3D m3{};
  int slot = -1;
  unsigned long long version = 0;
};

struct GeoMask {
  void *bits = nullptr;
  unsigned long long version = 0;
};
struct GeoState {
  std::map<int, GeoMask> masks;
  void *cells = nullptr, *heap = nullptr;
  unsigned *epochs = nullptr;
  int *work = nullptr;
  size_t cells_cap = 0;
  int nslots = 0;
  unsigned long long searches = 0;
  size_t budget = size_t(2) << 30;
  void *table = nullptr;
  std::vector<char> table_host;
};

struct DepthState {
  float *uv = nullptr;
  unsigned *max_bits = nullptr;
  size_t max_cap = 0;
  unsigned long long *box_tests = nullptr;
};

struct ProfileSlot {
  std::vector<std::pair<hipEvent_t, hipEvent_t>> pending;
  int64_t launches = 0;
  double ms = 0.0;
};

}

struct neo_ctx {
  int device = 0;
  hipStream_t stream = nullptr;
  bool own_stream = false;
  hipStream_t home_stream = nullptr;
  neo_params params{};
  neo::DevParams dev{};
  std::map<int, neo::MapEntry> maps;
  std::string err;
  std::recursive_mutex mu;
  int *tickets = nullptr;
  unsigned ticket_next = 0;
  void *table2d = nullptr, *table3d = nullptr;
  int n2d = 0, n3d = 0;
  bool table_dirty = true;
  void *scratch = nullptr;
  size_t scratch_bytes = 0;
  void *pinned = nullptr;
  size_t pinned_bytes = 0;
  bool profile = false;
  neo::ProfileSlot prof[NEO_KERNEL_COUNT];
  long long *sample_counter = nullptr;
  int *progress = nullptr;
  const int *dispatch_order = nullptr;
  int order_B = 0;
  double *trace = nullptr;
  double *trace_xg = nullptr;
  int trace_cap = 0;
  int *order_buf = nullptr;
  size_t order_cap = 0;
  int *sample_order = nullptr;
  size_t sample_order_cap = 0;
  int sample_order_B = 0;
  int edt_flags = 0;
  unsigned long long map_serial = 0;
  neo::GeoState geo;
  neo::DepthState depth;
};

namespace neo {

inline int fail(neo_ctx *c, int code, const std::string &msg) {
  if (c) c->err = msg;
  return code;
}

#define HIPCHK(c, call)                                                                     \
  do {                                                                                      \
    hipError_t e_ = (call);                                                                 \
    if (e_ != hipSuccess)                                                                   \
      return fail(c, NEO_ERR_HIP, std::string(#call) + ": " + hipGetErrorString(e_));       \
  } while (0)

struct DevBuf {
  void *p = nullptr;
  DevBuf() = default;
  DevBuf(const DevBuf &) = delete;
  DevBuf &operator=(const DevBuf &) = delete;
  ~DevBuf() {
    if (p) hipFree(p);
  }
  hipError_t alloc(size_t bytes) { return hipMalloc(&p, bytes); }
  void *release() {
    void *q = p;
    p = nullptr;
    return q;
  }
  template <typename T>
  T *as() const { return static_cast<T *>(p); }
};

struct ProfScope {
  neo_ctx *c;
  int k;
  hipEvent_t a = nullptr, b = nullptr;
  ProfScope(neo_ctx *c_, int k_) : c(c_), k(k_) {
    if (c->profile) {
      hipEventCreate(&a);
      hipEventCreate(&b);
      hipEventRecord(a, c->stream);
    }
  }
  ~ProfScope() {
    if (c->profile) {
      hipEventRecord(b, c->stream);
      c->prof[k].pending.emplace_back(a, b);
    }
  }
};

struct EvalArgs {
  int B, M;
  const double *x, *head, *tail;
  double *cost, *costs4, *grad, *coeffs;
  int *status;
};

struct OptArgs {
  int B, M;
  const void *table;
  const int *slots;
  int nmaps;
  const double *x0;
  double *x;
  const double *head, *tail;
  double *costs4, *costs4_last;
  int *nit, *nfev, *status;
  double *state = nullptr;
  int state_doubles = 0;
  int budget = 0;
  int resume = 0;
  const int *subset = nullptr;
  int n_subset = 0;
  int traj_total = 0;
};

struct SampleArgs {
  int B, M;
  const void *coeffs;
  const double *ts;
  double *costs2;
  void *grad_C, *grad_T;
  bool io32 = false;
};

struct AuditArgs {
  int B, M;
  MapRef maps;
  const double *x, *head, *tail;
  double hz, w[3];
  double *audit;
  int *count, *flags;
};

struct FleetTargetArgs {
  const double *cur_pos, *goal, *jitter;
  double longitu, lateral, move_vel;
  double *tail;
  int *near_goal, *lateral_steps, *flags;
};
struct FleetCmd {
  double *cmd;
  int cap;
  int *cmd_len, *cmd_index, *future_index;
};
struct FleetSpliceArgs {
  int M;
  const double *x, *head, *tail;
  const int *solved;
  double hz;
  int first;
  int *flags;
};
struct FleetAuditArgs {
  const double *cmd;
  int cap;
  const int *n_flown;
  int stride;
  double hz, w[3];
  double *audit;
  int *count, *flags;
};
int fleet_target(neo_ctx *c, const LaunchList &l, const MapRef &m, const FleetTargetArgs &a);
int fleet_advance(neo_ctx *c, const LaunchList &l, const FleetCmd &m, int step, int ahead, double *cur_pos, double *head);
int fleet_splice(neo_ctx *c, const LaunchList &l, const FleetCmd &m, const FleetSpliceArgs &a);
int fleet_audit(neo_ctx *c, const LaunchList &l, const MapRef &m, const FleetAuditArgs &a);
int fleet_pose(neo_ctx *c, const LaunchList &l, const FleetCmd &m, const double *cur_pos, const double *goal, double eye_z,
               double *pose);

struct RecordCommitArgs {
  int M;
  const double *x, *head, *tail;
  const int *solved;
  const double *pose, *cur_vel;
  const unsigned char *staging;
  int W, H;
  const int *mission_ids;
  int tick, round, capacity;
  double *motion, *wpts_local, *tau, *pose_rows;
  int *meta;
  unsigned char *images;
  int *row_of, *n_rows, *dropped;
};
int record_state(neo_ctx *c, const LaunchList &l, const double *cmd, int cap, const int *cmd_len, const int *cmd_index,
                 const double *head, double *cur_vel);
int record_commit(neo_ctx *c, const LaunchList &l, const RecordCommitArgs &a);

struct BatchCandArgs {
  int M, K;
  const double *head, *tail;
  const int *slots;
  const double *tau, *off;
  double *x0, *head_k, *tail_k;
  int *slots_k;
};
struct BatchSelectArgs {
  int n, K;
  RunRowsIn packed;
  const double *w;
  int *chosen;
  double *cand_cost;
  int *solved;
  RunRows out;
  int *nit_total, *opt_runs;
  int *fallback, *n_fallback;
};
int batch_candidates(neo_ctx *c, const LaunchList &l, const BatchCandArgs &a);
int batch_select(neo_ctx *c, const LaunchList &l, const BatchSelectArgs &a);
int batch_compact(neo_ctx *c, int P, int *pending, int *n_pending);

struct PlanGuessArgs {
  int M;
  const double *head, *tail;
  const int *slots;
  const double *x_init;
  const double *noise;
  const double *frac, *tau;
  double *x0, *head_k, *tail_k;
  int *slots_k;
};
struct PlanMergeArgs {
  int n, reset;
  RunRowsIn packed;
  RunRows out;
  int *attempts;
  long long *nit_total;
  int *solved;
  int *failed, *n_failed, *bad_scene;
};
int plan_guess(neo_ctx *c, const LaunchList &l, int D, const PlanGuessArgs &a);
int plan_merge(neo_ctx *c, const LaunchList &l, const PlanMergeArgs &a);

struct GeoArgs {
  int B;
  const int *slots;
  const double *start, *target;
  int max_exp, path_cap;
  double *key_pts, *path, *path_cost;
  int *path_len, *expansions, *flags;
};
int geo_search(neo_ctx *c, int scene_id, const GeoArgs &a);
int geo_prune(neo_ctx *c, int scene_id, int B, const int *slots, const double *paths, const int *path_len, int stride,
              double *key_pts);
void geo_release(neo_ctx *c);
void geo_forget(neo_ctx *c, int scene_id);

struct DepthCall {
  int W, H;
  double focal, max_range;
  const double *boxes;
  const int *box_begin;
  int n_scenes;
  const int *scene_index;
  int B;
  const double *pose;
  float *depth_m;
  unsigned char *depth_u8;
  float *depth_max;
};
int depth_render(neo_ctx *c, const DepthCall &a);
void depth_release(neo_ctx *c);

struct OnboardCall {
  LaunchList list;
  const float *depth_m;
  const double *pose;
  int W, H;
  double focal;
  int grid_w, grid_h;
  double res;
  const double *origins;
  double range, z_lo, z_hi;
  int l_hit, l_miss, l_lo, l_hi;
  int N, half;
  int8_t *logodds, *occupancy;
  int *changed;
};
int onboard_window_half(int width, double focal, double range, double res);
size_t onboard_lds_need(int half, int N, int height);
size_t onboard_lds_limit();
int onboard_integrate(neo_ctx *c, const OnboardCall &k);

struct Edt2DWork {
  const int8_t *occ;
  int *g, *v;
  double *z;
  double *dist, *gx, *gy;
};
void esdf_build_2d(neo_ctx *c, const Edt2DWork &w, int W, int H, double res, double4 *rec);
void esdf_build_2d_batch(neo_ctx *c, const Edt2DWork &w, int nmap, int W, int H, double res, double4 *const *recs);
void esdf_pack_2d(neo_ctx *c, const double *dist, const double *gx, const double *gy, size_t ncell, double4 *rec);
void esdf_pack_3d(neo_ctx *c, const void *src, int src_dtype, int nx, int ny, int nz, int store_dtype, int layout, int nbx,
                  int nby, int nbz, void *dst);
void esdf_edt_3d(neo_ctx *c, const uint8_t *occ, int nx, int ny, int nz, double res, uint16_t *gx, uint32_t *sq, float *dist);
void esdf_query(neo_ctx *c, const MapEntry &e, int n, const double *pts, double *dist, double *grad);

inline int slots_for(int M, int D) {
  const int n = D * (M - 1) + M;
  const int ns = (n + kWave - 1) / kWave;
  return ns <= 3 ? (ns < 1 ? 1 : ns) : 4;
}

template <class T>
struct Type {
  using type = T;
};
template <class Tag>
using type_of = typename Tag::type;
template <int V>
using Int = std::integral_constant<int, V>;
template <typename... E>
struct Elems {};
template <int... LAY>
struct Layouts {};
template <typename E>
constexpr int elem_code = std::is_same<E, float>::value ? NEO_F32 : NEO_F16;

template <typename Real, typename E, class F, int... LAY>
bool visit_layout(int layout, int &rc, F &f, Layouts<LAY...>) {
  return ((layout == LAY && (rc = f(Type<Lookup3D<Real, E, LAY>>{}), true)) || ...);
}
template <typename Real, class F, typename... E, int... LAY>
int visit_field(neo_ctx *c, int elem, int layout, Elems<E...>, Layouts<LAY...> lays, F f) {
  int rc = NEO_OK;
  if (((elem == elem_code<E> && visit_layout<Real, E>(layout, rc, f, lays)) || ...)) return rc;
// ... 43 lines not shown
```

neo-planner_amd/csrc/neo_kernels.hpp:

```cpp
#pragma once
#include <type_traits>
#include <hip/hip_runtime.h>
#include <hip/hip_fp16.h>

#include "../../include/neo_planner.h"
#ifndef NEO_FUSED_U
#define NEO_FUSED_U (sizeof(Real) == 4 ? 4 : 2)
#endif
#ifndef NEO_W2_U
#define NEO_W2_U 1
#endif
#ifndef NEO_W2_OCC
#define NEO_W2_OCC 2
#endif
#ifndef NEO_X_OCC
#define NEO_X_OCC 3
#endif
#ifndef NEO_SM_MAX_SLOTS
#define NEO_SM_MAX_SLOTS 2
#endif
#ifndef NEO_W2_MAX_SLOTS
#define NEO_W2_MAX_SLOTS 4
#endif
#include "neo_device.hpp"
#include "neo_lbfgs.hpp"
#include "neo_lbfgs_sm.hpp"

namespace neo {

template <typename Num, int NS>
using opt_scalar_t = std::conditional_t<sizeof(Num) == 4 && (NS <= NEO_SM_MAX_SLOTS), float, double>;

template <int D, int NS, typename Real>
__host__ __device__ constexpr int stage_doubles() {
  constexpr int fold = sizeof(Real) == 4 ? kWave * 8 * D * (int)sizeof(Real) : 0;
  return (NS * kWave * 8 > fold ? NS * kWave * 8 : fold) / 8;
}

constexpr int kSlCacheInts = kWave / 4 + kWave + 4;

template <typename Real, int NS, int WAVES>
__host__ __device__ constexpr bool pairs_in_f32() {
  return sizeof(Real) == 4 && WAVES == 2 && NS > 2;
}
template <int D, int NS, typename Real, class MapT, class LookupT, int SU = NEO_FUSED_U, class LG = WaveLanes,
          bool PAIRS32 = false, typename Num = double>
struct DevBackend {
  static constexpr int DL = LG::dl(D);
  static constexpr int kSlotsN = NS;
  static constexpr bool kPcr = sizeof(Num) == 4 && LG::W == kWave;
  struct Vec {
    Num v[NS];
  };
  Traj<D, DL, Num> t;
  const DevParams &prm;
  const MapT &map;
  double *xs;
  static constexpr int kStage = stage_doubles<D, NS, Real>();
  int *sl_cache = nullptr;
  bool fold_rows = true;
  bool fold_acc = false;
  using Scalar = opt_scalar_t<Num, NS>;
  LineSearchT<Scalar> *lsp;
  double *cst;
  using Hist = std::conditional_t<PAIRS32, float, double>;
  Hist *hist;
  int npad, m;
  double *coeff_out;
  long long samples = 0;
  int last_ns = 0;
  double *trace = nullptr;
  double *trace_xg = nullptr;
  int trace_cap = 0;

  __device__ DevBackend(const DevParams &p, const MapT &mp) : prm(p), map(mp) {}

  __device__ __forceinline__ double dot(const Vec &a, const Vec &b) const {
    Num s = Num(0);
#pragma unroll
    for (int k = 0; k < NS; ++k) s += a.v[k] * b.v[k];
    return uni((double)wave_sum(s));
  }
  __device__ __forceinline__ double uni(double v) const { return uniform(v); }
  __device__ __forceinline__ float uni(float v) const { return uniform(v); }
  __device__ __forceinline__ double amax(const Vec &a) const {
    Num s = Num(0);
#pragma unroll
    for (int k = 0; k < NS; ++k) s = fmax(s, fabs(a.v[k]));
    return wave_max_nonneg(s);
  }
  __device__ __forceinline__ void copy(Vec &d, const Vec &s) const {
#pragma unroll
    for (int k = 0; k < NS; ++k) d.v[k] = s.v[k];
  }
  __device__ __forceinline__ void neg(Vec &d, const Vec &s) const {
#pragma unroll
    for (int k = 0; k < NS; ++k) d.v[k] = -s.v[k];
  }
  __device__ __forceinline__ void axpy(double a, const Vec &x, Vec &y) const {
#pragma unroll
    for (int k = 0; k < NS; ++k) y.v[k] += (Num)a * x.v[k];
  }
  __device__ __forceinline__ void lincomb(Vec &o, const Vec &a, double s, const Vec &b) const {
#pragma unroll
    for (int k = 0; k < NS; ++k) o.v[k] = a.v[k] + (Num)s * b.v[k];
  }
  __device__ __forceinline__ void scale(Vec &v, double s) const {
#pragma unroll
    for (int k = 0; k < NS; ++k) v.v[k] *= (Num)s;
  }
  static constexpr int kFull = NS == 3 ? 2 : NS / 2;
  __device__ __forceinline__ bool in_range(int k, int lane) const { return k < kFull || k * kWave + lane < t.n; }
  __device__ __forceinline__ void hist_put(int slot, const Vec &s, const Vec &y) {
    const int lane = lane_id();
#pragma unroll
    for (int k = 0; k < NS; ++k)
      if (in_range(k, lane)) {
        hist[slot * t.n + k * kWave + lane] = (Hist)s.v[k];
        hist[(m + slot) * t.n + k * kWave + lane] = (Hist)y.v[k];
      }
    lds_wave_sync();
  }
  __device__ __forceinline__ void hist_get(int row, Vec &v) const {
    const int lane = lane_id();
#pragma unroll
    for (int k = 0; k < NS; ++k) v.v[k] = in_range(k, lane) ? (Num)hist[row * t.n + k * kWave + lane] : Num(0);
  }
  __device__ __forceinline__ void hist_get_s(int slot, Vec &v) const { hist_get(slot, v); }
  __device__ __forceinline__ void hist_get_y(int slot, Vec &v) const { hist_get(m + slot, v); }
  __device__ __forceinline__ void hist_get_sy(int slot, Vec &s, Vec &y) const {
    const int lane = lane_id();
    const Hist *ps = hist + slot * t.n + lane, *py = hist + (m + slot) * t.n + lane;
#pragma unroll
    for (int k = 0; k < NS; ++k) {
      s.v[k] = Num(0);
      y.v[k] = Num(0);
      if (in_range(k, lane)) {
        s.v[k] = (Num)ps[k * kWave];
        y.v[k] = (Num)py[k * kWave];
      }
    }
  }
  Num sreg = Num(0);
  __device__ __forceinline__ void sput(int i, double v) { sreg = (lane_id() == i) ? (Num)v : sreg; }
  __device__ __forceinline__ double sget(int i) const { return (double)rdlane(sreg, i); }
  __device__ __forceinline__ double sdiff(int i, double b) const { return (double)(rdlane(sreg, i) - (Num)b); }
  __device__ __forceinline__ double rho_dot(int slot, const Vec &a, const Vec &b) const {
    Num s = Num(0);
#pragma unroll
    for (int k = 0; k < NS; ++k) s += a.v[k] * b.v[k];
    return (double)(rdlane(sreg, slot) * wave_sum(s));
  }
  static constexpr bool kOwnDirection = sizeof(Num) == 4;
  __device__ __forceinline__ void direction(const Vec &g, Vec &d, int col, int head, int mm, Num theta) {
    if (col == 0) {
      neg(d, g);
      return;
    }
    auto slot_of = [&](int k) { return head + k < mm ? head + k : head + k - mm; };
    auto dot3 = [&](const Vec &a0, const Vec &b0, const Vec &a1, const Vec &b1, const Vec &a2, const Vec &b2, Num &t0, Num &t1,
                    Num &t2) {
      Num p0 = Num(0), p1 = Num(0), p2 = Num(0);
#pragma unroll
      for (int k = 0; k < NS; ++k) {
        p0 += a0.v[k] * b0.v[k];
        p1 += a1.v[k] * b1.v[k];
        p2 += a2.v[k] * b2.v[k];
      }
      Num unused;
      wave_sum4((float)p0, (float)p1, (float)p2, 0.0f, t0, t1, t2, unused);
    };
    copy(d, g);
    Vec sA, yA, sB, yB;
    int k = col - 1;
    for (; k >= 1; k -= 2) {
      const int A = slot_of(k), B = slot_of(k - 1);
      hist_get_sy(A, sA, yA);
      hist_get_sy(B, sB, yB);
      Num t0, t1, t2;
      dot3(sA, d, sB, d, sB, yA, t0, t1, t2);
      const Num aA = rdlane(sreg, A) * t0;
      const Num aB = rdlane(sreg, B) * (t1 - aA * t2);
      sput(mm + A, (double)aA);
      sput(mm + B, (double)aB);
#pragma unroll
      for (int q = 0; q < NS; ++q) d.v[q] = (d.v[q] - aA * yA.v[q]) - aB * yB.v[q];
    }
    if (k == 0) {
      const int A = slot_of(0);
      hist_get_sy(A, sA, yA);
      const Num aA = (Num)rho_dot(A, sA, d);
      sput(mm + A, (double)aA);
      axpy(-(double)aA, yA, d);
    }
    scale(d, (double)(Num(1) / theta));
    k = 0;
    for (; k + 1 < col; k += 2) {
      const int A = slot_of(k), B = slot_of(k + 1);
      hist_get_sy(A, sA, yA);
      hist_get_sy(B, sB, yB);
      Num t0, t1, t2;
      dot3(yA, d, yB, d, yB, sA, t0, t1, t2);
      const Num cA = rdlane(sreg, mm + A) - rdlane(sreg, A) * t0;
      const Num cB = rdlane(sreg, mm + B) - rdlane(sreg, B) * (t1 + cA * t2);
#pragma unroll
      for (int q = 0; q < NS; ++q) d.v[q] = (d.v[q] + cA * sA.v[q]) + cB * sB.v[q];
    }
    if (k < col) {
      const int A = slot_of(k);
      hist_get_sy(A, sA, yA);
      const double b = rho_dot(A, yA, d);
      axpy(sdiff(mm + A, b), sA, d);
    }
    scale(d, -1.0);
  }

  __device__ __forceinline__ LineSearchT<Scalar> &ls() { return *lsp; }
  __device__ __forceinline__ double *cost_store() { return cst; }

  __device__ __forceinline__ void note_eval(int nfev, int iter, double stp, double f, const Vec &x, const Vec &g) {
    if (nfev > trace_cap) return;
    if (trace != nullptr && lane_id() == 0) {
      double *r = trace + (size_t)(nfev - 1) * 4;
      r[0] = f;
      r[1] = stp;
      r[2] = (double)last_ns;
      r[3] = (double)iter;
    }
    if (trace_xg != nullptr) {
      const int lane = lane_id();
      double *r = trace_xg + (size_t)(nfev - 1) * 2 * t.n;
#pragma unroll
      for (int k = 0; k < NS; ++k)
        if (k * kWave + lane < t.n) {
          r[k * kWave + lane] = (double)x.v[k];
          r[t.n + k * kWave + lane] = (double)g.v[k];
        }
    }
  }

  __device__ __forceinline__ void scatter_x(const Vec &x) {
    const int lane = opaque(lane_id());
    lds_wave_sync();
    Num *xn = reinterpret_cast<Num *>(xs);
#pragma unroll
    for (int k = 0; k < NS; ++k)
      if (in_range(k, lane)) xn[k * kWave + lane] = x.v[k];
    lds_wave_sync();
    const int M = t.M;
    const int p = opaque(LG::piece());
    const bool act = p < M;
    t.tau = act ? xn[t.nq + p] : Num(0);
#pragma unroll
    for (int d = 0; d < DL; ++d) {
      const int dg = LG::dim0() + d;
      t.P0[d] = (p == 0 || !act) ? bstate<D, LG, false>(t, 0, d) : xn[dg * (M - 1) + (p > 0 ? p - 1 : 0)];
      t.P1[d] = (p >= M - 1) ? bstate<D, LG, true>(t, 0, d) : xn[dg * (M - 1) + p];
    }
  }

  __device__ __forceinline__ int eval(const Vec &x, double &f, Vec &g, double *costs) {
    const int lane = lane_id();
    const int p = LG::piece();
    NEO_MARK("eval_begin");
    const int M_all = t.M;
    t.M = opaque_uniform(M_all);
    scatter_x(x);
    NEO_MARK("scatter_done");
    Num *xn = reinterpret_cast<Num *>(xs);
    double energy, tsum;
    const int st = minco_forward<D, LG, Num, kPcr>(t, prm, energy, tsum);
    NEO_MARK("forward_done");
    if (st != 0) {
      f = 0.0;
#pragma unroll
      for (int k = 0; k < 4; ++k) costs[k] = 0.0;
      return st;
    }
    if (coeff_out != nullptr && p < t.M) {
#pragma unroll
      for (int k = 0; k < 6; ++k)
#pragma unroll
        for (int d = 0; d < DL; ++d) coeff_out[(size_t)(6 * p + k) * D + LG::dim0() + d] = (double)t.c[k][d];
    }
    Num gC[6][DL], gT = Num(0);
    double cf, ck;
    {
      Real cr[6][DL], gCr[6][DL], gTr;
#pragma unroll
      for (int k = 0; k < 6; ++k)
#pragma unroll
        for (int d = 0; d < DL; ++d) cr[k][d] = (Real)t.c[k][d];
      LookupT lk(map);
      int ns_by_piece = t.ns;
      if constexpr (LG::S > 1) ns_by_piece = __shfl(t.ns, min(LG::S * lane, kWave - 1), kWave);
      NEO_MARK("assign_begin");
      t.M = opaque_uniform(M_all);
      SampleLanes sl;
      bool cached = false;
      const int ns_key = lane < t.M ? ns_by_piece : 0;
      if (sl_cache != nullptr) cached = __ballot(ns_key == (int)reinterpret_cast<const unsigned char *>(sl_cache)[lane]) == ~0ull;
      if (cached) {
        const unsigned pk = (unsigned)sl_cache[kWave / 4 + lane];
        sl.piece = pk & 63;
        sl.r = (pk >> 6) & 63;
        sl.L = (pk >> 12) & 127;
        sl.act = ((pk >> 19) & 1) != 0;
        sl.first = (pk >> 20) & 63;
        sl.Lp = pk >> 26;
        sl.rounds = __builtin_amdgcn_readfirstlane(sl_cache[kWave / 4 + kWave]);
        sl.lmax = __builtin_amdgcn_readfirstlane(sl_cache[kWave / 4 + kWave + 1]);
        sl.total = __builtin_amdgcn_readfirstlane(sl_cache[kWave / 4 + kWave + 2]);
      } else {
        sl = balanced_sample_lanes(t.M, ns_by_piece, reinterpret_cast<int *>(xs));
        if (sl_cache != nullptr) {
          const bool fits = sl.lmax < 64 && ns_key < 255;
          reinterpret_cast<unsigned char *>(sl_cache)[lane] = (unsigned char)(__ballot(!fits) == 0 ? ns_key : 255);
          sl_cache[kWave / 4 + lane] = (int)((unsigned)sl.piece | ((unsigned)sl.r << 6) | ((unsigned)sl.L << 12) |
                                             ((sl.act ? 1u : 0u) << 19) | ((unsigned)sl.first << 20) | ((unsigned)sl.Lp << 26));
          if (lane == 0) {
            sl_cache[kWave / 4 + kWave] = sl.rounds;
            sl_cache[kWave / 4 + kWave + 1] = sl.lmax;
            sl_cache[kWave / 4 + kWave + 2] = sl.total;
          }
          lds_wave_sync();
        }
      }
      last_ns = sl.total;
      samples += (long long)last_ns;
      NEO_MARK("assign_done");
      minco_sample<Real, D, LookupT, SU, false, LG>(t.M, sl, t.ns, cr, prm, lk, gCr, gTr, cf, ck,
                                                    fold_rows ? reinterpret_cast<Real *>(xs) : nullptr, fold_acc);
#pragma unroll
      for (int k = 0; k < 6; ++k)
#pragma unroll
        for (int d = 0; d < DL; ++d) gC[k][d] = (Num)gCr[k][d];
      gT = (Num)gTr;
    }
    costs[0] = uniform(energy);
    costs[1] = uniform(tsum);
    costs[2] = uniform(cf);
    costs[3] = uniform(ck);
    f = uniform(costs[0] * prm.w[0] + costs[1] * prm.w[1] + costs[2] * prm.w[2] + costs[3] * prm.w[3]);
    Num gq[DL], gtau;
    NEO_MARK("sample_done");
    t.M = opaque_uniform(M_all);
    const int bst = minco_backward<D, LG, Num, kPcr>(t, prm, gC, gT, gq, gtau);
    NEO_MARK("backward_done");
    if (bst != 0) return bst;
    lds_wave_sync();
    const int pg = opaque(p), lg = opaque(lane);
    if (pg >= 1 && pg < t.M) {
#pragma unroll
      for (int d = 0; d < DL; ++d) xn[(LG::dim0() + d) * (t.M - 1) + pg - 1] = gq[d];
    }
    if (pg < t.M && LG::dim0() == opaque_uniform(0)) xn[t.nq + pg] = gtau;
    lds_wave_sync();
#pragma unroll
    for (int k = 0; k < NS; ++k) g.v[k] = in_range(k, lg) ? xn[k * kWave + lg] : Num(0);
    NEO_MARK("gather_done");
    return 0;
  }
};

__host__ __device__ inline size_t opt_state_doubles(int n, int m) { return 64 + 5 * (size_t)n + kWave + 2 * (size_t)m * (size_t)n; }

template <class BE, class Mach>
__device__ __forceinline__ void save_run(BE &be, const Mach &mc, double *st) {
  const int lane = lane_id(), n = be.t.n;
  lds_wave_sync();
  if (lane == 0) {
    const int iv[9] = {mc.phase, mc.status, mc.nfev, mc.nit, mc.iter, mc.col, mc.head, mc.task, mc.ifun};
#pragma unroll
    for (int k = 0; k < 9; ++k) st[k] = (double)iv[k];
    const double dv[7] = {(double)mc.f, (double)mc.fold, (double)mc.stp, (double)mc.gd, (double)mc.gdold, (double)mc.theta,
                          (double)mc.stp_evaluated};
#pragma unroll
    for (int k = 0; k < 7; ++k) st[9 + k] = dv[k];
    st[16] = (double)be.samples;
    st[17] = (double)be.last_ns;
    const auto &L = *be.lsp;
    const double lv[20] = {(double)L.ftol, (double)L.gtol, (double)L.xtol, (double)L.stpmin, (double)L.stpmax, (double)L.brackt,
                           (double)L.stage, (double)L.ginit, (double)L.gtest, (double)L.gx, (double)L.gy, (double)L.finit,
                           (double)L.fx, (double)L.fy, (double)L.stx, (double)L.sty, (double)L.stmin, (double)L.stmax,
                           (double)L.width, (double)L.width1};
#pragma unroll
    for (int k = 0; k < 20; ++k) st[20 + k] = lv[k];
#pragma unroll
    for (int k = 0; k < 12; ++k) st[40 + k] = be.cst[k];
  }
  double *v = st + 64;
#pragma unroll
  for (int k = 0; k < BE::kSlotsN; ++k)
    if (k * kWave + lane < n) {
      const int e = k * kWave + lane;
      v[e] = (double)mc.x.v[k];
      v[n + e] = (double)mc.g.v[k];
      v[2 * n + e] = (double)mc.t.v[k];
      v[3 * n + e] = (double)mc.r.v[k];
      v[4 * n + e] = (double)mc.d.v[k];
    }
  v[5 * n + lane] = (double)be.sreg;
  double *h = v + 5 * n + kWave;
  for (int i = lane; i < 2 * be.m * n; i += kWave) h[i] = (double)be.hist[i];
}

template <class BE, class Mach>
__device__ __forceinline__ void load_run(BE &be, Mach &mc, const double *st) {
  using Num = decltype(be.sreg);
  const int lane = lane_id(), n = be.t.n;
  auto iu = [&](int k) { return (int)uniform(st[k]); };
  mc.phase = iu(0); mc.status = iu(1); mc.nfev = iu(2); mc.nit = iu(3); mc.iter = iu(4);
  mc.col = iu(5); mc.head = iu(6); mc.task = iu(7); mc.ifun = iu(8);
  using S = typename Mach::S;
  mc.f = (S)uniform(st[9]); mc.fold = (S)uniform(st[10]); mc.stp = (S)uniform(st[11]); mc.gd = (S)uniform(st[12]);
  mc.gdold = (S)uniform(st[13]); mc.theta = (S)uniform(st[14]); mc.stp_evaluated = (S)uniform(st[15]);
  be.samples = (long long)uniform(st[16]);
  be.last_ns = iu(17);
  if (lane == 0) {
    auto &L = *be.lsp;
    L.ftol = (S)st[20]; L.gtol = (S)st[21]; L.xtol = (S)st[22]; L.stpmin = (S)st[23]; L.stpmax = (S)st[24];
    L.brackt = (int)st[25]; L.stage = (int)st[26];
    L.ginit = (S)st[27]; L.gtest = (S)st[28]; L.gx = (S)st[29]; L.gy = (S)st[30]; L.finit = (S)st[31]; L.fx = (S)st[32];
    L.fy = (S)st[33]; L.stx = (S)st[34]; L.sty = (S)st[35]; L.stmin = (S)st[36]; L.stmax = (S)st[37]; L.width = (S)st[38];
    L.width1 = (S)st[39];
#pragma unroll
    for (int k = 0; k < 12; ++k) be.cst[k] = st[40 + k];
  }
  const double *v = st + 64;
#pragma unroll
  for (int k = 0; k < BE::kSlotsN; ++k) {
    const int e = k * kWave + lane;
    const bool in = e < n;
    mc.x.v[k] = in ? (Num)v[e] : Num(0);
    mc.g.v[k] = in ? (Num)v[n + e] : Num(0);
    mc.t.v[k] = in ? (Num)v[2 * n + e] : Num(0);
    mc.r.v[k] = in ? (Num)v[3 * n + e] : Num(0);
    mc.d.v[k] = in ? (Num)v[4 * n + e] : Num(0);
  }
  be.sreg = (Num)v[5 * n + lane];
  const double *h = v + 5 * n + kWave;
  for (int i = lane; i < 2 * be.m * n; i += kWave) be.hist[i] = (typename BE::Hist)h[i];
  lds_wave_sync();
}

template <class LG = WaveLanes, int D, int DL, typename Num>
__device__ __forceinline__ void load_boundary(Traj<D, DL, Num> &t, const double *head, const double *tail, int M,
                                              Num *bnd_lds = nullptr) {
  t.M = M;
  t.nq = D * (M - 1);
  t.n = t.nq + M;
  t.L = sample_lanes_per_piece(M);
  t.head = head;
  t.tail = tail;
  stage_boundary<D, LG>(t, bnd_lds);
}

struct MapTable {
  const void *maps;
};

template <int D, int NS, typename Real, class MapT, class LookupT, class LG = WaveLanes, typename Num = double>
__global__ __launch_bounds__(kWave) void eval_kernel(int B, int M, DevParams prm, MapT map,
                                                      const double *__restrict__ x,
                                                      const double *__restrict__ head,
                                                      const double *__restrict__ tail,
                                                      double *__restrict__ cost, double *__restrict__ costs4,
                                                      double *__restrict__ grad, double *__restrict__ coeffs,
                                                      int *__restrict__ status) {
  __shared__ __attribute__((aligned(16))) double xs[stage_doubles<D, NS, Real>()];
  __shared__ LineSearchT<opt_scalar_t<Num, NS>> lsm;
  __shared__ double cst[12];
  __shared__ Num bnd[6 * D];
  constexpr bool kKeep = sizeof(Num) == 4 && LG::S > 1;
  __shared__ __attribute__((aligned(16))) Num mult_s[kKeep ? (5 * 8 + 4) * (kWave / LG::S + 1) : 4];
  const int b = blockIdx.x;
  if (b >= B) return;
  using BE = DevBackend<D, NS, Real, MapT, LookupT, NEO_FUSED_U, LG, false, Num>;
  BE be(prm, map);
  if constexpr (kKeep) be.t.pcr_mult = mult_s;
  be.xs = xs;
  if constexpr (sizeof(Num) == 4 && LG::W == kWave)
    if (pcr_xch_elems(M, LG::dl(D)) * (int)sizeof(Num) <= stage_doubles<D, NS, Real>() * 8) be.t.pcr_xch = reinterpret_cast<Num *>(xs);
  be.lsp = &lsm;
  be.cst = cst;
  be.hist = nullptr;
  be.m = NEO_LBFGS_M;
  load_boundary<LG>(be.t, head + (size_t)b * 3 * D, tail + (size_t)b * 3 * D, M, bnd);
  const int n = be.t.n;
  be.npad = NS * kWave;
  be.coeff_out = coeffs ? coeffs + (size_t)b * 6 * M * D : nullptr;
  const int lane = lane_id();
  typename BE::Vec xv, gv;
#pragma unroll
  for (int k = 0; k < NS; ++k) xv.v[k] = (k * kWave + lane < n) ? x[(size_t)b * n + k * kWave + lane] : 0.0;
  double f;
  double *costs = cst;
  const int st = be.eval(xv, f, gv, costs);
#pragma unroll
  for (int k = 0; k < NS; ++k)
    if (k * kWave + lane < n) grad[(size_t)b * n + k * kWave + lane] = gv.v[k];
  if (lane == 0) {
    cost[b] = f;
#pragma unroll
    for (int k = 0; k < 4; ++k) costs4[(size_t)b * 4 + k] = costs[k];
    if (status) status[b] = st;
  }
}

template <int D, int NS, typename Real, class MapT, class LookupT, int WAVES, class LG = WaveLanes, typename Num = double,
          bool BUDGET = false>
__global__ __launch_bounds__(kWave, (WAVES == 2 ? (sizeof(Num) == 4 && NS <= 2 ? NEO_X_OCC : NEO_W2_OCC) : 1)) void optimize_kernel(int B, int M, DevParams prm, const MapT *maps,
                                                          const int *__restrict__ scene_slot, int nmaps,
                                                          const double *x0, double *x,
                                                          const double *__restrict__ head,
                                                          const double *__restrict__ tail,
                                                          double *__restrict__ costs4,
                                                          double *__restrict__ costs4_last,
                                                          int *__restrict__ nit, int *__restrict__ nfev,
                                                          int *__restrict__ status,
                                                          long long *__restrict__ nsamples,
                                                          const int *__restrict__ order, double *__restrict__ trace,
                                                          double *__restrict__ trace_xg, int trace_cap, int stage, int pcr_off,
                                                          double *state, int state_doubles, int budget, int resume,
                                                          int traj_total) {
  extern __shared__ __attribute__((aligned(16))) double dyn_lds[];
  __shared__ LineSearchT<opt_scalar_t<Num, NS>> lsm;
  __shared__ double cst[12];
  __shared__ Num bnd[6 * D];
  constexpr bool kSlCache = sizeof(Num) == 4;
  __shared__ __attribute__((aligned(8))) int slc[kSlCache ? kSlCacheInts : 2];
  if ((int)blockIdx.x >= B) return;
  const int b = order ? order[blockIdx.x] : (int)blockIdx.x;
  if constexpr (BUDGET)
    if (b < 0 || b >= traj_total) return;
  using BE = DevBackend<D, NS, Real, MapT, LookupT, (WAVES == 2 ? NEO_W2_U : NEO_FUSED_U), LG,
                        pairs_in_f32<Real, NS, WAVES>() || sizeof(Num) == 4, Num>;
  const int slot = scene_slot ? scene_slot[b] : 0;
  if (slot < 0 || slot >= nmaps) {
    if (lane_id() == 0) {
      status[b] = NEO_TRAJ_BAD_SCENE;
      nit[b] = 0;
      nfev[b] = 0;
      if constexpr (!BUDGET)
        if (state != nullptr) __hip_atomic_fetch_add(reinterpret_cast<int *>(state), 1, __ATOMIC_RELEASE, __HIP_MEMORY_SCOPE_SYSTEM);
    }
    return;
  }
  const MapT map = maps[slot];
  BE be(prm, map);
  be.xs = dyn_lds;
  be.fold_rows = stage >= stage_doubles<D, NS, Real>();
  if constexpr (sizeof(Num) == 4 && LG::S > 1) {
    if (pcr_off != 0) {
      be.t.pcr_mult = reinterpret_cast<Num *>(dyn_lds + pcr_off);
      be.fold_rows = true;
      be.fold_acc = true;
    }
  }
  if constexpr (sizeof(Num) == 4 && LG::W == kWave)
    if (be.fold_rows && pcr_xch_elems(M, LG::dl(D)) * (int)sizeof(Num) <= stage * 8) be.t.pcr_xch = reinterpret_cast<Num *>(dyn_lds);
  be.lsp = &lsm;
  be.cst = cst;
  be.m = NEO_LBFGS_M;
  be.coeff_out = nullptr;
  if constexpr (kSlCache) {
    if (lane_id() < kWave / 4) slc[lane_id()] = -1;
    be.sl_cache = slc;
  }
  be.trace = trace ? trace + (size_t)b * trace_cap * 4 : nullptr;
  be.trace_cap = (trace != nullptr || trace_xg != nullptr) ? trace_cap : 0;
  be.trace_xg = trace_xg ? trace_xg + (size_t)b * trace_cap * 2 * (D * (M - 1) + M) : nullptr;
  load_boundary<LG>(be.t, head + (size_t)b * 3 * D, tail + (size_t)b * 3 * D, M, bnd);
  const int n = be.t.n;
  be.npad = NS * kWave;
  be.hist = reinterpret_cast<typename BE::Hist *>(dyn_lds + stage);
  const int lane = lane_id();
  typename BE::Vec xv;
#pragma unroll
  for (int k = 0; k < NS; ++k) xv.v[k] = (k * kWave + lane < n) ? x0[(size_t)b * n + k * kWave + lane] : 0.0;
  LbfgsOpts o{prm.ftol, prm.gtol, prm.maxls, prm.maxiter, prm.maxfun, NEO_LBFGS_M};
  LbfgsResult res;
  bool suspended = false;
  if constexpr (NS <= NEO_SM_MAX_SLOTS) {
    LbfgsMachine<BE> mach(be, o);
    if constexpr (BUDGET) {
      double *st = state + (size_t)b * (size_t)state_doubles;
      if (resume) {
        if (status[b] != NEO_TRAJ_SUSPENDED) return;
        load_run(be, mach, st);
      } else {
        mach.x = xv;
        mach.begin();
      }
      int evals = 0;
      while (mach.need_eval()) {
        if (evals >= budget) {
          save_run(be, mach, st);
          suspended = true;
          break;
        }
        double fe;
        const int est = be.eval(mach.x, fe, mach.g, mach.costs());
        mach.f = (typename BE::Scalar)fe;
        mach.advance(est);
        ++evals;
      }
    } else {
      mach.x = xv;
      mach.begin();
      while (mach.need_eval()) {
        double fe;
        const int est = be.eval(mach.x, fe, mach.g, mach.costs());
        mach.f = (typename BE::Scalar)fe;
        mach.advance(est);
      }
    }
    mach.result(res);
    xv = mach.x;
  } else {
    lbfgs_minimize<BE>(be, xv, o, res);
  }
#pragma unroll
  for (int k = 0; k < NS; ++k)
    if (k * kWave + lane < n) x[(size_t)b * n + k * kWave + lane] = xv.v[k];
  if (lane == 0) {
    int st = res.status;
    if (res.costs_last[3] * prm.w[3] > prm.coll_tol) st |= NEO_TRAJ_FLAG_COLLISION;
    if (suspended) st = NEO_TRAJ_SUSPENDED;
#pragma unroll
    for (int k = 0; k < 4; ++k) {
      costs4[(size_t)b * 4 + k] = res.costs[k];
      if (costs4_last) costs4_last[(size_t)b * 4 + k] = res.costs_last[k];
    }
    nit[b] = res.nit;
    nfev[b] = res.nfev;
    status[b] = st;
    if (nsamples) nsamples[b] = be.samples;
  }
  if constexpr (!BUDGET) {
    if (state != nullptr && lane == 0)
      __hip_atomic_fetch_add(reinterpret_cast<int *>(state), 1, __ATOMIC_RELEASE, __HIP_MEMORY_SCOPE_SYSTEM);
  }
}

#ifndef NEO_SAMPLE_U
#define NEO_SAMPLE_U 1
#endif
#ifndef NEO_SAMPLE_OCC
#define NEO_SAMPLE_OCC 5
#endif
template <int D, typename Real, class MapT, class LookupT, typename IO = double>
__device__ __forceinline__ void sample_wave_per_piece(int b, int M, const DevParams &prm, const MapT &map,
                                                      const IO *__restrict__ coeffs, const double *__restrict__ ts,
                                                      double *__restrict__ costs2, IO *__restrict__ grad_C,
                                                      IO *__restrict__ grad_T, int *seg, Real *rows) {
  typedef IO IOPair __attribute__((ext_vector_type(2)));
  const int lane = lane_id();
  const double Tp = lane < M ? ts[(size_t)b * M + lane] : 1.0;
  const int ns_p = lane < M ? (int)(Tp / prm.delta_t) : 0;
  const SampleLanes sl = balanced_sample_lanes(M, ns_p, seg);
  const int piece = sl.piece, r = sl.r;
  const bool act = sl.act;
  const double T = act ? ts[(size_t)b * M + piece] : 1.0;
  const int ns = act ? (int)(T / prm.delta_t) : 0;
  Real c[6][D], gC[6][D], gT;
  {
    const IOPair *src = reinterpret_cast<const IOPair *>(coeffs + ((size_t)b * 6 * M + 6 * (act ? piece : 0)) * D);
#pragma unroll
    for (int q = 0; q < 3 * D; ++q) {
      const IOPair v = src[q];
      const int e0 = 2 * q, e1 = 2 * q + 1;
      c[e0 / D][e0 % D] = act ? (Real)v.x : Real(0);
      c[e1 / D][e1 % D] = act ? (Real)v.y : Real(0);
    }
  }
  double cf, ck;
  LookupT lk(map);
  minco_sample<Real, D, LookupT, NEO_SAMPLE_U, true>(M, sl, ns, c, prm, lk, gC, gT, cf, ck, sizeof(Real) == 4 ? rows : nullptr);
  if (act && r == 0) {
    IOPair *dst = reinterpret_cast<IOPair *>(grad_C + ((size_t)b * 6 * M + 6 * piece) * D);
#pragma unroll
    for (int q = 0; q < 3 * D; ++q) {
      const int e0 = 2 * q, e1 = 2 * q + 1;
      dst[q] = IOPair{(IO)gC[e0 / D][e0 % D], (IO)gC[e1 / D][e1 % D]};
    }
    grad_T[(size_t)b * M + piece] = (IO)gT;
  }
  if (lane < M && ns_p == 0) {
    IOPair *dst = reinterpret_cast<IOPair *>(grad_C + ((size_t)b * 6 * M + 6 * lane) * D);
#pragma unroll
    for (int q = 0; q < 3 * D; ++q) dst[q] = IOPair{IO(0), IO(0)};
    grad_T[(size_t)b * M + lane] = IO(0);
  }
  if (lane == 0) {
    costs2[(size_t)b * 2 + 0] = cf;
    costs2[(size_t)b * 2 + 1] = ck;
  }
}

template <int D, typename Real, class MapT, class LookupT, typename IO = double>
__global__ __launch_bounds__(kWave, sizeof(Real) == 4 ? NEO_SAMPLE_OCC : 2) void sample_kernel(int B, int M, DevParams prm, MapT map,
                                                                                  const IO *__restrict__ coeffs,
                                                                                  const double *__restrict__ ts,
                                                                                  double *__restrict__ costs2,
                                                                                  IO *__restrict__ grad_C,
                                                                                  IO *__restrict__ grad_T,
                                                                                  const int *__restrict__ order) {
  if ((int)blockIdx.x >= B) return;
  const int b = order ? order[blockIdx.x] : (int)blockIdx.x;
  __shared__ int seg[kWave];
  __shared__ __attribute__((aligned(16))) Real rows[sizeof(Real) == 4 ? kWave * 8 * D : 4];
  sample_wave_per_piece<D, Real, MapT, LookupT, IO>(b, M, prm, map, coeffs, ts, costs2, grad_C, grad_T, seg, rows);
}

}
```

neo-planner_amd/csrc/neo_launch_opt.hpp:

```cpp
#pragma once
#include "neo_host.hpp"
#include "neo_kernels.hpp"

namespace neo {

struct OptLds {
  int stage, pcr_off;
  size_t dyn;
};

template <int D, int NS, typename Real, int WAVES, class LG, typename Num>
OptLds opt_lds_plan(int M, int flags) {
  const size_t pair_elems = (size_t)2 * NEO_LBFGS_M * (D * (M - 1) + M);
  const size_t cache = sizeof(Num) == 4 ? kSlCacheInts * sizeof(int) : 0;
  const size_t statics = 400;
  const size_t lds_share8 = (size_t)160 * 1024 / 8 / 1280 * 1280 - statics - cache,
               lds_share12 = (size_t)160 * 1024 / (4 * NEO_X_OCC) / 1280 * 1280 - statics - cache;
  const size_t pairs = pair_elems * ((pairs_in_f32<Real, NS, WAVES>() || sizeof(Num) == 4) ? sizeof(float) : sizeof(double));
  const int full = stage_doubles<D, NS, Real>(), small = NS * kWave;
  const size_t lds_share = (sizeof(Num) == 4 && NS <= 2) ? lds_share12 : lds_share8;
  OptLds l{pairs + (size_t)full * 8 <= lds_share ? full : small, 0, 0};
  l.dyn = pairs + (size_t)l.stage * 8;
  if (sizeof(Num) == 4 && LG::S > 1 && !(flags & 4096)) {
    const int acc = std::max(std::max(small, (M * fold_acc_stride(D) * 4 + 7) / 8), (pcr_xch_elems(M, 1) * 4 + 7) / 8);
    const size_t off = ((size_t)acc * 8 + pairs + 15) / 16 * 2;
    const size_t need = off * 8 + (size_t)pcr_mult_elems(M) * sizeof(float);
    if (need <= lds_share) {
      l.stage = acc;
      l.pcr_off = (int)off;
      l.dyn = need;
    }
  }
  return l;
}

template <int D, int NS, typename Real, class MapT, class LookupT, int WAVES, class LG, typename Num, bool BUDGET>
int launch_opt_kernel(neo_ctx *c, const OptArgs &a) {
  const int n_launch = a.subset ? a.n_subset : a.B;
  const int *launch_order = a.subset ? a.subset : (c->order_B == a.B ? c->dispatch_order : nullptr);
  const OptLds l = opt_lds_plan<D, NS, Real, WAVES, LG, Num>(a.M, c->params.flags);
  hipLaunchKernelGGL((optimize_kernel<D, NS, Real, MapT, LookupT, WAVES, LG, Num, BUDGET>), dim3(n_launch), dim3(kWave), l.dyn,
                     c->stream, n_launch, a.M, c->dev, static_cast<const MapT *>(a.table), a.slots, a.nmaps,
                     a.x0 ? a.x0 : a.x, a.x, a.head, a.tail, a.costs4, a.costs4_last, a.nit, a.nfev, a.status,
                     c->sample_counter, launch_order, c->trace, c->trace_xg, c->trace_cap, l.stage, l.pcr_off,
                     BUDGET ? a.state : reinterpret_cast<double *>(c->progress) ,
                     a.state_doubles, a.budget, a.resume, a.traj_total);
  return NEO_OK;
}

template <int D, typename Real, class MapT, class LookupT, int WAVES = 1, typename Num = double, bool BUDGET = false>
int launch_opt(neo_ctx *c, const OptArgs &a) {
  constexpr int max_ns = BUDGET ? 2 : (WAVES == 1 || NEO_W2_MAX_SLOTS >= 4) ? 4 : 2;
  if (const int ns = slots_for(a.M, D); ns > max_ns) {
    if (BUDGET) return fail(c, NEO_ERR_INVALID, "budgeted launches: n <= 128 variables");
    if (ns == 3) return fail(c, NEO_ERR_INVALID, "n > 128 variables: this build has no two-waves kernel for three FLAT slots");
    return fail(c, NEO_ERR_INVALID, "n > 128 variables: this build has no two-waves kernel for four FLAT slots "
                                    "(NEO_W2_MAX_SLOTS < 4)");
  }
  return visit_slots<D, max_ns>(a.M, c->params.flags, [&](auto ns, auto lg) {
    return launch_opt_kernel<D, decltype(ns)::value, Real, MapT, LookupT, WAVES, type_of<decltype(lg)>, Num, BUDGET>(c, a);
  });
}

}
```

neo-planner_amd/neo_planner_amd/_lib.py:

```python
import ctypes
import os
import sys

import numpy as np

PKG = os.path.dirname(os.path.abspath(__file__))
LIB_PATH = os.environ.get("NEO_PLANNER_LIB") or os.path.join(PKG, "libneo_planner_hip.so")

NEO_OK = 0
NEO_F64, NEO_F32, NEO_F16 = 0, 1, 2
NEO_LAYOUT_LINEAR, NEO_LAYOUT_YZ4, NEO_LAYOUT_CELL8, NEO_LAYOUT_BRICK = 0, 1, 2, 3
LAYOUTS = {"linear": NEO_LAYOUT_LINEAR, "yz4": NEO_LAYOUT_YZ4, "cell8": NEO_LAYOUT_CELL8, "brick": NEO_LAYOUT_BRICK}
NEO_TRAJ_CONVERGED_GRAD, NEO_TRAJ_CONVERGED_F, NEO_TRAJ_ABNORMAL = 0, 1, 2
NEO_TRAJ_MAXITER, NEO_TRAJ_NUMERIC_RANGE, NEO_TRAJ_NONFINITE, NEO_TRAJ_BAD_SCENE, NEO_TRAJ_SUSPENDED = 3, 4, 5, 6, 7
NEO_TRAJ_FLAG_COLLISION = 0x100
NEO_EDT_GENERIC_LINES = 1
NEO_KERNEL_EVAL, NEO_KERNEL_OPTIMIZE, NEO_KERNEL_ESDF_BUILD, NEO_KERNEL_ESDF_SAMPLE = 0, 1, 2, 3
NEO_FLAG_ONE_WAVE_PER_SIMD, NEO_FLAG_TWO_WAVES_PER_SIMD, NEO_FLAG_LANE_GROUPS = 32, 64, 128
NEO_FLAG_F32_SOLVE = 2048
AUDIT_FIELDS = ("path_length", "feasibility", "collision", "weighted", "min_clearance", "t_min_clearance", "max_speed",
                "max_acc", "t_first_unsafe", "duration")
NEO_AUDIT_FIELDS = len(AUDIT_FIELDS)
NEO_AUDIT_FLAG_UNSAFE, NEO_AUDIT_FLAG_METRIC_FAIL, NEO_AUDIT_FLAG_OUTSIDE_MAP, NEO_AUDIT_FLAG_NONFINITE = 1, 2, 4, 8
NEO_GEO_FLAG_NO_PATH, NEO_GEO_FLAG_START_OUTSIDE, NEO_GEO_FLAG_CAPPED, NEO_GEO_FLAG_PATH_TRUNCATED = 1, 2, 4, 8
NEO_GEO_FLAG_BAD_SCENE = 16
NEO_FLEET_FLAG_TARGET_CAPPED, NEO_FLEET_FLAG_CMD_FULL, NEO_FLEET_FLAG_BAD_SCENE, NEO_FLEET_FLAG_SPLICE_FAILED = 1, 2, 4, 8
NEO_FLEET_FLAG_ABANDONED = 16
NEO_BATCH_MAX_CANDIDATES = 8
NEO_DEPTH_MAX_BOXES = 1024

EXPORTS = [
    "neo_abi_version", "neo_ctx_create", "neo_ctx_destroy", "neo_last_error", "neo_params_default",
    "neo_params_set", "neo_ctx_synchronize", "neo_esdf_upload_2d", "neo_esdf_build_2d",
    "neo_esdf_upload_3d", "neo_esdf_drop", "neo_esdf_query", "neo_cost_grad_batch",
    "neo_cost_grad_batch_dev", "neo_optimize_batch", "neo_optimize_batch_dev", "neo_scene_slot",
    "neo_optimize_workspace_bytes", "neo_eval_traj_batch", "neo_profile_enable", "neo_profile_read",
    "neo_profile_reset", "neo_optimize_sample_counter", "neo_optimize_dispatch_order",
    "neo_sampled_terms_batch", "neo_sampled_terms_batch_dev", "neo_esdf_build_3d",
    "neo_optimize_dispatch_order_host", "neo_ctx_set_stream", "neo_optimize_trace",
    "neo_optimize_batch_from_dev", "neo_optimize_trace_xg", "neo_sampled_terms_dispatch_order",
    "neo_esdf_build_config", "neo_pack_results_dev", "neo_optimize_state_bytes", "neo_optimize_batch_budget_dev",
    "neo_sampled_terms_batch_f32", "neo_sampled_terms_batch_f32_dev", "neo_effort_order_dev",
    "neo_optimize_progress_counter", "neo_effort_order_scratch_bytes", "neo_audit_traj_batch",
    "neo_audit_traj_batch_dev", "neo_geo_search_batch", "neo_geo_search_batch_dev", "neo_geo_prune_batch",
    "neo_geo_workspace_budget", "neo_fleet_target_batch", "neo_fleet_target_batch_dev", "neo_fleet_advance_dev",
    "neo_fleet_splice_dev", "neo_fleet_audit_batch", "neo_fleet_audit_batch_dev", "neo_batch_candidates",
    "neo_batch_candidates_dev", "neo_batch_select", "neo_batch_select_dev", "neo_plan_guess", "neo_plan_guess_dev",
    "neo_plan_merge", "neo_plan_merge_dev", "neo_depth_render_batch", "neo_depth_render_batch_dev",
    "neo_depth_box_test_counter", "neo_onboard_integrate_batch", "neo_onboard_integrate_batch_dev",
    "neo_esdf_build_2d_batch_dev", "neo_fleet_pose_dev", "neo_record_state_dev", "neo_record_commit_dev",
]


class NeoParams(ctypes.Structure):
    _fields_ = [("v_max", ctypes.c_double), ("T_min", ctypes.c_double), ("T_max", ctypes.c_double),
                ("safe_dis", ctypes.c_double), ("delta_t", ctypes.c_double), ("weights", ctypes.c_double * 4),
                ("collision_cost_tol", ctypes.c_double), ("ftol", ctypes.c_double), ("gtol", ctypes.c_double),
                ("maxls", ctypes.c_int32), ("maxiter", ctypes.c_int32), ("maxfun", ctypes.c_int32),
                ("bugcompat_stale_T", ctypes.c_int32), ("sample_dtype", ctypes.c_int32),
                ("flags", ctypes.c_int32)]


_lib = None


class NeoError(RuntimeError):
    pass


def load():
    global _lib
    if _lib is not None:
        return _lib
    if not os.path.exists(LIB_PATH):
        raise NeoError(f"{LIB_PATH} is missing: build it with `python -m neo_planner_amd.build` "
                       "(hipcc, gfx950).  There is no CPU fallback.")
    if "torch" not in sys.modules and not os.environ.get("NEO_NO_TORCH_PRELOAD"):
        try:
            import torch
        except ImportError:
            pass
    L = ctypes.CDLL(LIB_PATH)
    c_p, c_i, c_d = ctypes.c_void_p, ctypes.c_int, ctypes.c_double
    L.neo_abi_version.restype = c_i
    L.neo_ctx_create.argtypes = [c_i, c_p, ctypes.POINTER(c_p)]
    L.neo_ctx_destroy.argtypes = [c_p]
    L.neo_last_error.argtypes = [c_p]
    L.neo_last_error.restype = ctypes.c_char_p
    L.neo_params_default.argtypes = [ctypes.POINTER(NeoParams)]
    L.neo_params_set.argtypes = [c_p, ctypes.POINTER(NeoParams)]
    L.neo_ctx_synchronize.argtypes = [c_p]
    L.neo_ctx_set_stream.argtypes = [c_p, c_p]
    L.neo_esdf_upload_2d.argtypes = [c_p, c_i, c_p, c_p, c_p, c_i, c_i, c_d, c_d, c_d]
    L.neo_esdf_build_2d.argtypes = [c_p, c_i, c_p, c_i, c_i, c_d, c_d, c_d, c_p, c_p, c_p]
    L.neo_esdf_upload_3d.argtypes = [c_p, c_i, c_p, c_i, c_i, c_i, c_i, c_i, c_d, c_p, c_i, c_i]
    L.neo_esdf_build_3d.argtypes = [c_p, c_i, c_p, c_i, c_i, c_i, c_i, c_d, c_p, c_i, c_i, c_p]
    L.neo_esdf_drop.argtypes = [c_p, c_i]
    L.neo_esdf_query.argtypes = [c_p, c_i, c_i, c_p, c_p, c_p]
    L.neo_cost_grad_batch.argtypes = [c_p, c_i, c_i, c_i, c_i] + [c_p] * 8
    L.neo_cost_grad_batch_dev.argtypes = [c_p, c_i, c_i, c_i, c_i] + [c_p] * 8
    L.neo_optimize_batch.argtypes = [c_p, c_i, c_p, c_i, c_i, c_i] + [c_p] * 8
    L.neo_optimize_batch_dev.argtypes = [c_p, c_i, c_p, c_i, c_i, c_i] + [c_p] * 8
    L.neo_optimize_batch_from_dev.argtypes = [c_p, c_i, c_p, c_i, c_i, c_i] + [c_p] * 9
    L.neo_scene_slot.argtypes = [c_p, c_i]
    L.neo_optimize_workspace_bytes.argtypes = [c_i, c_i, c_i]
    L.neo_optimize_workspace_bytes.restype = ctypes.c_size_t
    L.neo_eval_traj_batch.argtypes = [c_p, c_i, c_i, c_i, c_p, c_p, c_p, c_d, c_i, c_p, c_p]
    L.neo_audit_traj_batch.argtypes = [c_p, c_i, c_p, c_i, c_i, c_i, c_p, c_p, c_p, c_d] + [c_p] * 4
    L.neo_audit_traj_batch_dev.argtypes = [c_p, c_i, c_p, c_i, c_i, c_i, c_p, c_p, c_p, c_d] + [c_p] * 4
    L.neo_geo_search_batch.argtypes = [c_p, c_i, c_p, c_i, c_p, c_p, c_i, c_i] + [c_p] * 6
    L.neo_geo_search_batch_dev.argtypes = [c_p, c_i, c_p, c_i, c_p, c_p, c_i, c_i] + [c_p] * 6
    L.neo_geo_prune_batch.argtypes = [c_p, c_i, c_p, c_i, c_p, c_p, c_i, c_p]
    L.neo_geo_workspace_budget.argtypes = [c_p, ctypes.c_size_t]
    L.neo_fleet_target_batch.argtypes = [c_p, c_i, c_p, c_i, c_p, c_i, c_p, c_p, c_p, c_d, c_d, c_d] + [c_p] * 4
    L.neo_fleet_target_batch_dev.argtypes = [c_p, c_i, c_p, c_i, c_p, c_i, c_p, c_p, c_p, c_d, c_d, c_d] + [c_p] * 4
    L.neo_fleet_advance_dev.argtypes = [c_p, c_i, c_p, c_i, c_p, c_i, c_p, c_p, c_p, c_i, c_i, c_p, c_p]
    L.neo_fleet_splice_dev.argtypes = [c_p, c_i, c_p, c_i, c_i, c_p, c_p, c_p, c_p, c_d, c_i, c_p, c_i] + [c_p] * 4
    L.neo_fleet_audit_batch.argtypes = [c_p, c_i, c_p, c_i, c_p, c_i, c_p, c_i, c_p, c_i, c_d] + [c_p] * 4
    L.neo_fleet_audit_batch_dev.argtypes = [c_p, c_i, c_p, c_i, c_p, c_i, c_p, c_i, c_p, c_i, c_d] + [c_p] * 4
    L.neo_batch_candidates.argtypes = [c_p, c_i, c_p, c_i, c_i, c_i, c_i] + [c_p] * 9
    L.neo_batch_candidates_dev.argtypes = [c_p, c_i, c_p, c_i, c_i, c_i, c_i] + [c_p] * 9
    L.neo_batch_select.argtypes = [c_p, c_i, c_p, c_i, c_i, c_i, c_i] + [c_p] * 20
    L.neo_batch_select_dev.argtypes = [c_p, c_i, c_p, c_i, c_i, c_i, c_i] + [c_p] * 20
    L.neo_plan_guess.argtypes = [c_p, c_i, c_p, c_i, c_i, c_i] + [c_p] * 11
    L.neo_plan_guess_dev.argtypes = [c_p, c_i, c_p, c_i, c_i, c_i] + [c_p] * 11
    L.neo_plan_merge.argtypes = [c_p, c_i, c_p, c_i, c_i, c_i, c_i] + [c_p] * 18
    L.neo_plan_merge_dev.argtypes = [c_p, c_i, c_p, c_i, c_i, c_i, c_i] + [c_p] * 18
    L.neo_depth_render_batch.argtypes = [c_p, c_i, c_i, c_d, c_d, c_p, c_p, c_i, c_p, c_i] + [c_p] * 4
    L.neo_depth_render_batch_dev.argtypes = [c_p, c_i, c_i, c_d, c_d, c_p, c_p, c_i, c_p, c_i] + [c_p] * 4
    L.neo_depth_box_test_counter.argtypes = [c_p, c_p]
    _onboard = [c_p, c_i, c_p, c_i, c_p, c_p, c_i, c_i, c_d, c_d, c_i, c_i, c_d, c_p, c_d, c_d, c_d, c_i, c_i, c_i, c_i, c_p, c_p, c_p]
    L.neo_onboard_integrate_batch.argtypes = list(_onboard)
    L.neo_onboard_integrate_batch_dev.argtypes = list(_onboard)
    L.neo_esdf_build_2d_batch_dev.argtypes = [c_p, c_p, c_i, c_p, c_i, c_i, c_d, c_p]
    L.neo_fleet_pose_dev.argtypes = [c_p, c_i, c_p, c_i, c_p, c_i, c_p, c_p, c_p, c_p, c_d, c_p]
    L.neo_record_state_dev.argtypes = [c_p, c_i, c_p, c_i, c_p, c_i, c_p, c_p, c_p, c_p]
    L.neo_record_commit_dev.argtypes = [c_p, c_i, c_p, c_i, c_i] + [c_p] * 7 + [c_i, c_i, c_p, c_i, c_i, c_i] + [c_p] * 9
    L.neo_profile_enable.argtypes = [c_p, c_i]
    L.neo_profile_read.argtypes = [c_p, c_i, ctypes.POINTER(ctypes.c_int64), ctypes.POINTER(c_d)]
    L.neo_profile_reset.argtypes = [c_p]
    L.neo_optimize_sample_counter.argtypes = [c_p, c_p]
    L.neo_optimize_trace.argtypes = [c_p, c_p, c_i]
    L.neo_optimize_trace_xg.argtypes = [c_p, c_p, c_i]
    L.neo_optimize_dispatch_order.argtypes = [c_p, c_p, c_i]
    L.neo_optimize_dispatch_order_host.argtypes = [c_p, c_p, c_i]
    L.neo_sampled_terms_dispatch_order.argtypes = [c_p, c_p, c_i, c_i]
    L.neo_esdf_build_config.argtypes = [c_p, c_i]
    L.neo_pack_results_dev.argtypes = [c_p, c_i, c_i, c_p, c_p, c_p, c_p]
    L.neo_optimize_state_bytes.argtypes = [c_i, c_i]
    L.neo_optimize_state_bytes.restype = ctypes.c_size_t
    L.neo_optimize_batch_budget_dev.argtypes = [c_p, c_i, c_i, c_i, c_i] + [c_p] * 10 + [c_i, c_p, c_i, c_i]
    L.neo_sampled_terms_batch.argtypes = [c_p, c_i, c_i, c_i, c_i] + [c_p] * 5
    L.neo_sampled_terms_batch_dev.argtypes = [c_p, c_i, c_i, c_i, c_i] + [c_p] * 5
    L.neo_sampled_terms_batch_f32.argtypes = [c_p, c_i, c_i, c_i, c_i] + [c_p] * 5
    L.neo_sampled_terms_batch_f32_dev.argtypes = [c_p, c_i, c_i, c_i, c_i] + [c_p] * 5
    L.neo_effort_order_dev.argtypes = [c_p, c_i, c_i, c_i] + [c_p] * 5
    L.neo_optimize_progress_counter.argtypes = [c_p, c_p]
    L.neo_effort_order_scratch_bytes.argtypes = [c_i]
    L.neo_effort_order_scratch_bytes.restype = ctypes.c_size_t
    for name in EXPORTS:
        fn = getattr(L, name)
        if fn.restype is ctypes.c_int or name in ("neo_abi_version",):
            fn.restype = c_i
    _lib = L
    return L


def ptr(a):
    if a is None:
        return None
    assert a.flags["C_CONTIGUOUS"]
    return a.ctypes.data_as(ctypes.c_void_p)


def as_f64(a):
    return np.ascontiguousarray(a, dtype=np.float64)


def dev_ptr(t):
    return ctypes.c_void_p(t.data_ptr()) if t is not None else None


def launch_count(subset, B):
    return B if subset is None else int(subset.numel())


class Context:

    def __init__(self, device=0, stream=None):
        self.lib = load()
        h = ctypes.c_void_p()
        self.device = int(device)
        rc = self.lib.neo_ctx_create(int(device), ctypes.c_void_p(stream) if stream else None, ctypes.byref(h))
        if rc != NEO_OK:
            raise NeoError(f"neo_ctx_create(device={device}) failed with {rc}: no usable MI355X? "
                           "(the product path has no CPU fallback)")
        self.h = h
        self.params = NeoParams()
        self.lib.neo_params_default(ctypes.byref(self.params))
        self._next_scene = 0

    def check(self, rc):
        if rc != NEO_OK:
            raise NeoError(f"libneo_planner_hip error {rc}: {self.lib.neo_last_error(self.h).decode()}")

    def set_params(self, **kw):
        for k, v in kw.items():
            if k == "weights":
                for i in range(4):
                    self.params.weights[i] = float(v[i])
            else:
                setattr(self.params, k, v)
        self.check(self.lib.neo_params_set(self.h, ctypes.byref(self.params)))

    def new_scene_id(self):
        self._next_scene += 1
        return self._next_scene

    def synchronize(self):
        self.check(self.lib.neo_ctx_synchronize(self.h))

    def set_stream(self, stream=None):
        self.check(self.lib.neo_ctx_set_stream(self.h, ctypes.c_void_p(stream) if stream else None))

    def close(self):
        if self.h:
            self.lib.neo_ctx_destroy(self.h)
            self.h = None

    def __del__(self):
        try:
            self.close()
        except Exception:
            pass


_default_ctx = {}


def default_context(device=0):
    if device not in _default_ctx:
        _default_ctx[device] = Context(device)
    return _default_ctx[device]
```

Before: 1.512 million traj/s.

## Specialize optimize kernel with compile-time plan to drop runtime feature branches

Adds a compile-time Plan policy that fixes flags such as PCR multiplier/exchange buffers, fold rows/accumulate, the sample-lane cache, trace and coefficient output. For f32 multi-lane configurations the host launches a specialised kernel when its runtime conditions hold, and otherwise falls back to a dynamic variant. This removes per-evaluation branches and dead paths from the L-BFGS inner loop, which may lower register pressure. The cost is an extra kernel instantiation, and the plan check must match the runtime state exactly. Launch counters are added for diagnostics.

```diff
diff --git a/include/neo_planner.h b/include/neo_planner.h
--- a/include/neo_planner.h
+++ b/include/neo_planner.h
@@ -289,6 +289,7 @@
                          float *out);
 int neo_sampled_terms_dispatch_order(neo_ctx *ctx, const int32_t *order, int on_device, int B);
 int neo_profile_read(neo_ctx *ctx, int kernel, int64_t *launches, double *total_ms);
+int neo_optimize_plan_launches(neo_ctx *ctx, int64_t *fixed_plan, int64_t *dynamic_plan);
 int neo_profile_reset(neo_ctx *ctx);
 
 #ifdef __cplusplus
diff --git a/neo-planner_amd/csrc/neo_abi.hip b/neo-planner_amd/csrc/neo_abi.hip
--- a/neo-planner_amd/csrc/neo_abi.hip
+++ b/neo-planner_amd/csrc/neo_abi.hip
@@ -2073,6 +2073,14 @@
   return NEO_OK;
 }
 
+int neo_optimize_plan_launches(neo_ctx *c, int64_t *fixed_plan, int64_t *dynamic_plan) {
+  if (!c) return NEO_ERR_INVALID;
+  std::lock_guard<std::recursive_mutex> g(c->mu);
+  if (fixed_plan) *fixed_plan = c->opt_plan_launches[0];
+  if (dynamic_plan) *dynamic_plan = c->opt_plan_launches[1];
+  return NEO_OK;
+}
+
 int neo_profile_enable(neo_ctx *c, int on) {
   if (!c) return NEO_ERR_INVALID;
   std::lock_guard<std::recursive_mutex> g(c->mu);
diff --git a/neo-planner_amd/csrc/neo_device.hpp b/neo-planner_amd/csrc/neo_device.hpp
--- a/neo-planner_amd/csrc/neo_device.hpp
+++ b/neo-planner_amd/csrc/neo_device.hpp
@@ -418,6 +418,24 @@
   static __host__ __device__ __forceinline__ int lanes_per_piece(int M) { return sample_lanes_per_piece_fwd(M); }
 };
 
+struct PlanDynamic {
+  static constexpr bool dynamic = true;
+  static constexpr bool fold_acc = false, fold_rows = false, pcr_mult = false, pcr_xch = false, sl_cache = false,
+                        trace = false, coeff_out = false;
+};
+struct PlanFixedX {
+  static constexpr bool dynamic = false;
+  static constexpr bool fold_acc = true, fold_rows = true, pcr_mult = true, pcr_xch = true, sl_cache = true,
+                        trace = false, coeff_out = false;
+};
+template <class Plan, bool K>
+__host__ __device__ __forceinline__ constexpr bool plan_pick(bool run_time) {
+  if constexpr (Plan::dynamic)
+    return run_time;
+  else
+    return K;
+}
+
 template <int D, int DL = D, typename Num = double>
 struct Traj {
   int M, n, nq, L;
@@ -568,7 +586,7 @@
   }
 }
 
-template <int DL, class LG, typename Num>
+template <int DL, class LG, typename Num, class Plan = PlanDynamic>
 __device__ __forceinline__ void pcr_solve(int M, Num (&L)[2][2], Num (&Dg)[2][2], Num (&U)[2][2], Num (&R)[2][DL],
                                           Num (&y)[2][DL], Num *mult = nullptr, Num *xch = nullptr) {
   static_assert(LG::W == kWave, "written for lane groups that span the wavefront");
@@ -588,7 +606,8 @@
   const int lane = lane_id();
   const int s_end = sizeof(Num) == 4 ? min(M - 1, 32) : M - 1;
   typedef Num Quad __attribute__((ext_vector_type(4)));
-  const bool writer = mult != nullptr && in && LG::dim0() == opaque_uniform(0);
+  const bool keep = plan_pick<Plan, Plan::pcr_mult>(mult != nullptr), use_xch = plan_pick<Plan, Plan::pcr_xch>(xch != nullptr);
+  const bool writer = keep && in && LG::dim0() == opaque_uniform(0);
   int level = 0;
   if constexpr (sizeof(Num) == 4) {
     typedef float f2 __attribute__((ext_vector_type(2)));
@@ -604,14 +623,13 @@
       Ir[1].y = Dr[0].x * r;
     };
     auto fetch = [&](const f2 v, int src) { return f2{__shfl(v.x, src, kWave), __shfl(v.y, src, kWave)}; };
-    const bool keep = mult != nullptr;
     const int ps = min(p, M);
     for (int s = 1; s < s_end; s <<= 1, ++level) {
       invert();
       const int sp = lane - s * LG::S, sn = lane + s * LG::S;
       f2 Ip[2], Lp[2], Upv[2], In[2], Ln[2], Un[2];
       Num Rp[2][DL], Rn[2][DL];
-      if (xch != nullptr) {
+      if (use_xch) {
         Quad *tab = reinterpret_cast<Quad *>(xch);
         f2 *rx = reinterpret_cast<f2 *>(xch + (size_t)(M + 1) * 12);
         lds_wave_sync();
@@ -673,7 +691,7 @@
       }
     }
     invert();
-    if (xch != nullptr) lds_wave_sync();
+    if (use_xch) lds_wave_sync();
     if (keep) *reinterpret_cast<Quad *>(mult + (size_t)level * (M + 1) * 8 + (size_t)ps * 4) = Quad{Ir[0].x, Ir[0].y, Ir[1].x, Ir[1].y};
 #pragma unroll
     for (int d = 0; d < DL; ++d) {
@@ -826,7 +844,8 @@
   Up[1][0] = -Num(168.0) * t.i3; Up[1][1] = Num(24.0) * t.i2;
 }
 
-template <int D, class LG = WaveLanes, typename Num = double, bool PCR = (sizeof(Num) == 4 && LG::W == kWave)>
+template <int D, class LG = WaveLanes, typename Num = double, bool PCR = (sizeof(Num) == 4 && LG::W == kWave),
+          class Plan = PlanDynamic>
 __device__ __forceinline__ int minco_forward(Traj<D, LG::dl(D), Num> &t, const DevParams &prm, double &energy,
                                              double &time_sum) {
   constexpr int DL = LG::dl(D);
@@ -893,7 +912,7 @@
           Up[i][j] = lane == t.M - 1 ? Num(0.0) : Up[i][j];
         }
       NEO_MARK("fwd_pcr_begin");
-      pcr_solve<DL, LG, Num>(t.M, Lo, Di, Up, R, y, t.pcr_mult, t.pcr_xch);
+      pcr_solve<DL, LG, Num, Plan>(t.M, Lo, Di, Up, R, y, t.pcr_mult, t.pcr_xch);
       NEO_MARK("fwd_pcr_end");
     } else {
       thomas_solve<DL, LG, Num>(NEO_DBG(prm, 2 | 16) ? 1 : t.M, Lo, t.N, E, R, y0, yM, y);
@@ -1174,7 +1193,7 @@
 
 __host__ __device__ constexpr int fold_acc_stride(int D) { return (6 * D + 1 + 3) / 4 * 4; }
 
-template <typename Real, int D, class LookupT, int U, bool SAMPLE_IO = false, class LG = WaveLanes>
+template <typename Real, int D, class LookupT, int U, bool SAMPLE_IO = false, class LG = WaveLanes, class Plan = PlanDynamic>
 __device__ __forceinline__ void minco_sample(int M, const SampleLanes &sl, int ns_in, const Real (&cp)[6][LG::dl(D)],
                                              const DevParams &prm, const LookupT &lk, Real (&gC)[6][LG::dl(D)], Real &gT,
                                              double &cost_feas, double &cost_coll, Real *fold_rows = nullptr,
@@ -1276,8 +1295,9 @@
     }
   }
   NEO_MARK("loop_end");
+  constexpr bool kAccOnly = !Plan::dynamic && Plan::fold_rows && Plan::fold_acc && sizeof(Real) == 4 && !SAMPLE_IO && LG::S > 1;
   if constexpr (sizeof(Real) == 4 && !SAMPLE_IO && LG::S > 1) {
-    if (fold_rows != nullptr && fold_acc && sl.lmax != 0) {
+    if (plan_pick<Plan, Plan::fold_rows>(fold_rows != nullptr) && plan_pick<Plan, Plan::fold_acc>(fold_acc) && sl.lmax != 0) {
       typedef Real Quad __attribute__((ext_vector_type(4)));
       constexpr int RS = fold_acc_stride(D), NQ = RS / 4;
       Quad v[NQ];
@@ -1326,8 +1346,8 @@
       return;
     }
   }
-  if constexpr (sizeof(Real) == 4) {
-    if (fold_rows != nullptr && sl.lmax != 0) {
+  if constexpr (sizeof(Real) == 4 && !kAccOnly) {
+    if (plan_pick<Plan, Plan::fold_rows>(fold_rows != nullptr) && sl.lmax != 0) {
       typedef Real Quad __attribute__((ext_vector_type(4)));
       constexpr int DR = LG::dl(D);
       Quad *row = reinterpret_cast<Quad *>(fold_rows + (size_t)lane * (8 * D));
@@ -1384,10 +1404,14 @@
   fv[6 * D] = aT;
   fv[6 * D + 1] = aF;
   fv[6 * D + 2] = aK;
-  if (sl.lmax == 0)
+  if constexpr (kAccOnly) {
     fold_piece_lanes<Real, 6 * D + 3>(fv, L, r);
-  else
-    fold_piece_segments<Real, 6 * D + 3>(fv, r, L, sl.lmax);
+  } else {
+    if (sl.lmax == 0)
+      fold_piece_lanes<Real, 6 * D + 3>(fv, L, r);
+    else
+      fold_piece_segments<Real, 6 * D + 3>(fv, r, L, sl.lmax);
+  }
   if constexpr (!SAMPLE_IO) {
     int src = LG::base() + sl.first;
     if constexpr (LG::S > 1) src = __shfl(sl.first, LG::piece(), kWave);
@@ -1416,7 +1440,8 @@
   cost_coll = LG::sum(mine ? (double)pk : 0.0);
 }
 
-template <int D, class LG = WaveLanes, typename Num = double, bool PCR = (sizeof(Num) == 4 && LG::W == kWave)>
+template <int D, class LG = WaveLanes, typename Num = double, bool PCR = (sizeof(Num) == 4 && LG::W == kWave),
+          class Plan = PlanDynamic>
 __device__ __forceinline__ int minco_backward(const Traj<D, LG::dl(D), Num> &t, const DevParams &prm,
                                               Num (&gC)[6][LG::dl(D)], Num gT, Num (&gq)[LG::dl(D)], Num &gtau) {
   constexpr int DL = LG::dl(D);
@@ -1468,7 +1493,7 @@
   for (int d = 0; d < DL; ++d) lam[0][d] = lam[1][d] = Num(0.0);
   constexpr bool kPcr = PCR;
   if constexpr (kPcr) {
-    if (M > 1 && t.pcr_mult != nullptr) {
+    if (M > 1 && plan_pick<Plan, Plan::pcr_mult>(t.pcr_mult != nullptr)) {
       Num R[2][DL], y[2][DL];
 #pragma unroll
       for (int d = 0; d < DL; ++d) {
diff --git a/neo-planner_amd/csrc/neo_host.hpp b/neo-planner_amd/csrc/neo_host.hpp
--- a/neo-planner_amd/csrc/neo_host.hpp
+++ b/neo-planner_amd/csrc/neo_host.hpp
@@ -80,6 +80,7 @@
   bool profile = false;
   neo::ProfileSlot prof[NEO_KERNEL_COUNT];
   long long *sample_counter = nullptr;
+  int64_t opt_plan_launches[2] = {0, 0};
   int *progress = nullptr;
   const int *dispatch_order = nullptr;
   int order_B = 0;
diff --git a/neo-planner_amd/csrc/neo_kernels.hpp b/neo-planner_amd/csrc/neo_kernels.hpp
--- a/neo-planner_amd/csrc/neo_kernels.hpp
+++ b/neo-planner_amd/csrc/neo_kernels.hpp
@@ -44,7 +44,7 @@
   return sizeof(Real) == 4 && WAVES == 2 && NS > 2;
 }
 template <int D, int NS, typename Real, class MapT, class LookupT, int SU = NEO_FUSED_U, class LG = WaveLanes,
-          bool PAIRS32 = false, typename Num = double>
+          bool PAIRS32 = false, typename Num = double, class Plan = PlanDynamic>
 struct DevBackend {
   static constexpr int DL = LG::dl(D);
   static constexpr int kSlotsN = NS;
@@ -219,6 +219,7 @@
   __device__ __forceinline__ double *cost_store() { return cst; }
 
   __device__ __forceinline__ void note_eval(int nfev, int iter, double stp, double f, const Vec &x, const Vec &g) {
+    if constexpr (!Plan::dynamic && !Plan::trace) return;
     if (nfev > trace_cap) return;
     if (trace != nullptr && lane_id() == 0) {
       double *r = trace + (size_t)(nfev - 1) * 4;
@@ -269,7 +270,7 @@
     NEO_MARK("scatter_done");
     Num *xn = reinterpret_cast<Num *>(xs);
     double energy, tsum;
-    const int st = minco_forward<D, LG, Num, kPcr>(t, prm, energy, tsum);
+    const int st = minco_forward<D, LG, Num, kPcr, Plan>(t, prm, energy, tsum);
     NEO_MARK("forward_done");
     if (st != 0) {
       f = 0.0;
@@ -277,7 +278,7 @@
       for (int k = 0; k < 4; ++k) costs[k] = 0.0;
       return st;
     }
-    if (coeff_out != nullptr && p < t.M) {
+    if (plan_pick<Plan, Plan::coeff_out>(coeff_out != nullptr) && p < t.M) {
 #pragma unroll
       for (int k = 0; k < 6; ++k)
 #pragma unroll
@@ -299,7 +300,8 @@
       SampleLanes sl;
       bool cached = false;
       const int ns_key = lane < t.M ? ns_by_piece : 0;
-      if (sl_cache != nullptr) cached = __ballot(ns_key == (int)reinterpret_cast<const unsigned char *>(sl_cache)[lane]) == ~0ull;
+      const bool have_cache = plan_pick<Plan, Plan::sl_cache>(sl_cache != nullptr);
+      if (have_cache) cached = __ballot(ns_key == (int)reinterpret_cast<const unsigned char *>(sl_cache)[lane]) == ~0ull;
       if (cached) {
         const unsigned pk = (unsigned)sl_cache[kWave / 4 + lane];
         sl.piece = pk & 63;
@@ -313,7 +315,7 @@
         sl.total = __builtin_amdgcn_readfirstlane(sl_cache[kWave / 4 + kWave + 2]);
       } else {
         sl = balanced_sample_lanes(t.M, ns_by_piece, reinterpret_cast<int *>(xs));
-        if (sl_cache != nullptr) {
+        if (have_cache) {
           const bool fits = sl.lmax < 64 && ns_key < 255;
           reinterpret_cast<unsigned char *>(sl_cache)[lane] = (unsigned char)(__ballot(!fits) == 0 ? ns_key : 255);
           sl_cache[kWave / 4 + lane] = (int)((unsigned)sl.piece | ((unsigned)sl.r << 6) | ((unsigned)sl.L << 12) |
@@ -329,8 +331,9 @@
       last_ns = sl.total;
       samples += (long long)last_ns;
       NEO_MARK("assign_done");
-      minco_sample<Real, D, LookupT, SU, false, LG>(t.M, sl, t.ns, cr, prm, lk, gCr, gTr, cf, ck,
-                                                    fold_rows ? reinterpret_cast<Real *>(xs) : nullptr, fold_acc);
+      minco_sample<Real, D, LookupT, SU, false, LG, Plan>(
+          t.M, sl, t.ns, cr, prm, lk, gCr, gTr, cf, ck,
+          plan_pick<Plan, Plan::fold_rows>(fold_rows) ? reinterpret_cast<Real *>(xs) : nullptr, fold_acc);
 #pragma unroll
       for (int k = 0; k < 6; ++k)
 #pragma unroll
@@ -345,7 +348,7 @@
     Num gq[DL], gtau;
     NEO_MARK("sample_done");
     t.M = opaque_uniform(M_all);
-    const int bst = minco_backward<D, LG, Num, kPcr>(t, prm, gC, gT, gq, gtau);
+    const int bst = minco_backward<D, LG, Num, kPcr, Plan>(t, prm, gC, gT, gq, gtau);
     NEO_MARK("backward_done");
     if (bst != 0) return bst;
     lds_wave_sync();
@@ -508,22 +511,16 @@
   }
 }
 
-template <int D, int NS, typename Real, class MapT, class LookupT, int WAVES, class LG = WaveLanes, typename Num = double,
-          bool BUDGET = false>
-__global__ __launch_bounds__(kWave, (WAVES == 2 ? (sizeof(Num) == 4 && NS <= 2 ? NEO_X_OCC : NEO_W2_OCC) : 1)) void optimize_kernel(int B, int M, DevParams prm, const MapT *maps,
-                                                          const int *__restrict__ scene_slot, int nmaps,
-                                                          const double *x0, double *x,
-                                                          const double *__restrict__ head,
-                                                          const double *__restrict__ tail,
-                                                          double *__restrict__ costs4,
-                                                          double *__restrict__ costs4_last,
-                                                          int *__restrict__ nit, int *__restrict__ nfev,
-                                                          int *__restrict__ status,
-                                                          long long *__restrict__ nsamples,
-                                                          const int *__restrict__ order, double *__restrict__ trace,
-                                                          double *__restrict__ trace_xg, int trace_cap, int stage, int pcr_off,
-                                                          double *state, int state_doubles, int budget, int resume,
-                                                          int traj_total) {
+template <class Plan, int D, int NS, typename Real, class MapT, class LookupT, int WAVES, class LG, typename Num, bool BUDGET>
+__device__ __forceinline__ void optimize_body(int B, int M, const DevParams &prm, const MapT *maps,
+                                              const int *__restrict__ scene_slot, int nmaps, const double *x0, double *x,
+                                              const double *__restrict__ head, const double *__restrict__ tail,
+                                              double *__restrict__ costs4, double *__restrict__ costs4_last,
+                                              int *__restrict__ nit, int *__restrict__ nfev, int *__restrict__ status,
+                                              long long *__restrict__ nsamples, const int *__restrict__ order,
+                                              double *__restrict__ trace, double *__restrict__ trace_xg, int trace_cap, int stage,
+                                              int pcr_off, double *state, int state_doubles, int budget, int resume,
+                                              int traj_total) {
   extern __shared__ __attribute__((aligned(16))) double dyn_lds[];
   __shared__ LineSearchT<opt_scalar_t<Num, NS>> lsm;
   __shared__ double cst[12];
@@ -535,7 +532,7 @@
   if constexpr (BUDGET)
     if (b < 0 || b >= traj_total) return;
   using BE = DevBackend<D, NS, Real, MapT, LookupT, (WAVES == 2 ? NEO_W2_U : NEO_FUSED_U), LG,
-                        pairs_in_f32<Real, NS, WAVES>() || sizeof(Num) == 4, Num>;
+                        pairs_in_f32<Real, NS, WAVES>() || sizeof(Num) == 4, Num, Plan>;
   const int slot = scene_slot ? scene_slot[b] : 0;
   if (slot < 0 || slot >= nmaps) {
     if (lane_id() == 0) {
@@ -552,14 +549,15 @@
   be.xs = dyn_lds;
   be.fold_rows = stage >= stage_doubles<D, NS, Real>();
   if constexpr (sizeof(Num) == 4 && LG::S > 1) {
-    if (pcr_off != 0) {
+    if (plan_pick<Plan, Plan::pcr_mult>(pcr_off != 0)) {
       be.t.pcr_mult = reinterpret_cast<Num *>(dyn_lds + pcr_off);
       be.fold_rows = true;
       be.fold_acc = true;
     }
   }
   if constexpr (sizeof(Num) == 4 && LG::W == kWave)
-    if (be.fold_rows && pcr_xch_elems(M, LG::dl(D)) * (int)sizeof(Num) <= stage * 8) be.t.pcr_xch = reinterpret_cast<Num *>(dyn_lds);
+    if (plan_pick<Plan, Plan::pcr_xch>(be.fold_rows && pcr_xch_elems(M, LG::dl(D)) * (int)sizeof(Num) <= stage * 8))
+      be.t.pcr_xch = reinterpret_cast<Num *>(dyn_lds);
   be.lsp = &lsm;
   be.cst = cst;
   be.m = NEO_LBFGS_M;
@@ -568,9 +566,11 @@
     if (lane_id() < kWave / 4) slc[lane_id()] = -1;
     be.sl_cache = slc;
   }
-  be.trace = trace ? trace + (size_t)b * trace_cap * 4 : nullptr;
-  be.trace_cap = (trace != nullptr || trace_xg != nullptr) ? trace_cap : 0;
-  be.trace_xg = trace_xg ? trace_xg + (size_t)b * trace_cap * 2 * (D * (M - 1) + M) : nullptr;
+  if constexpr (Plan::dynamic || Plan::trace) {
+    be.trace = trace ? trace + (size_t)b * trace_cap * 4 : nullptr;
+    be.trace_cap = (trace != nullptr || trace_xg != nullptr) ? trace_cap : 0;
+    be.trace_xg = trace_xg ? trace_xg + (size_t)b * trace_cap * 2 * (D * (M - 1) + M) : nullptr;
+  }
   load_boundary<LG>(be.t, head + (size_t)b * 3 * D, tail + (size_t)b * 3 * D, M, bnd);
   const int n = be.t.n;
   be.npad = NS * kWave;
@@ -644,6 +644,56 @@
   }
 }
 
+template <int NS, class LG, typename Num, bool BUDGET>
+using opt_plan_t = std::conditional_t<sizeof(Num) == 4 && (LG::S > 1) && NS <= 2 && !BUDGET, PlanFixedX, PlanDynamic>;
+
+#define NEO_OPT_LAUNCH_BOUNDS __launch_bounds__(kWave, (WAVES == 2 ? (sizeof(Num) == 4 && NS <= 2 ? NEO_X_OCC : NEO_W2_OCC) : 1))
+
+template <int D, int NS, typename Real, class MapT, class LookupT, int WAVES, class LG = WaveLanes, typename Num = double,
+          bool BUDGET = false>
+__global__ NEO_OPT_LAUNCH_BOUNDS void optimize_kernel(int B, int M, DevParams prm, const MapT *maps,
+                                                          const int *__restrict__ scene_slot, int nmaps,
+                                                          const double *x0, double *x,
+                                                          const double *__restrict__ head,
+                                                          const double *__restrict__ tail,
+                                                          double *__restrict__ costs4,
+                                                          double *__restrict__ costs4_last,
+                                                          int *__restrict__ nit, int *__restrict__ nfev,
+                                                          int *__restrict__ status,
+                                                          long long *__restrict__ nsamples,
+                                                          const int *__restrict__ order, double *__restrict__ trace,
+                                                          double *__restrict__ trace_xg, int trace_cap,
+                                                          int stage, int pcr_off,
+                                                          double *state, int state_doubles, int budget, int resume,
+                                                          int traj_total) {
+  optimize_body<opt_plan_t<NS, LG, Num, BUDGET>, D, NS, Real, MapT, LookupT, WAVES, LG, Num, BUDGET>(
+      B, M, prm, maps, scene_slot, nmaps, x0, x, head, tail, costs4, costs4_last, nit, nfev, status, nsamples, order, trace,
+      trace_xg, trace_cap, stage, pcr_off, state, state_doubles, budget, resume, traj_total);
+}
+
+template <int D, int NS, typename Real, class MapT, class LookupT, int WAVES, class LG = WaveLanes, typename Num = double,
+          bool BUDGET = false>
+__global__ NEO_OPT_LAUNCH_BOUNDS void optimize_dyn_kernel(int B, int M, DevParams prm, const MapT *maps,
+                                                              const int *__restrict__ scene_slot, int nmaps,
+                                                              const double *x0, double *x,
+                                                              const double *__restrict__ head,
+                                                              const double *__restrict__ tail,
+                                                              double *__restrict__ costs4,
+                                                              double *__restrict__ costs4_last,
+                                                              int *__restrict__ nit, int *__restrict__ nfev,
+                                                              int *__restrict__ status,
+                                                              long long *__restrict__ nsamples,
+                                                              const int *__restrict__ order, double *__restrict__ trace,
+                                                              double *__restrict__ trace_xg, int trace_cap,
+                                                              int stage, int pcr_off,
+                                                              double *state, int state_doubles, int budget, int resume,
+                                                              int traj_total) {
+  optimize_body<PlanDynamic, D, NS, Real, MapT, LookupT, WAVES, LG, Num, BUDGET>(
+      B, M, prm, maps, scene_slot, nmaps, x0, x, head, tail, costs4, costs4_last, nit, nfev, status, nsamples, order, trace,
+      trace_xg, trace_cap, stage, pcr_off, state, state_doubles, budget, resume, traj_total);
+}
+#undef NEO_OPT_LAUNCH_BOUNDS
+
 #ifndef NEO_SAMPLE_U
 #define NEO_SAMPLE_U 1
 #endif
diff --git a/neo-planner_amd/csrc/neo_launch_opt.hpp b/neo-planner_amd/csrc/neo_launch_opt.hpp
--- a/neo-planner_amd/csrc/neo_launch_opt.hpp
+++ b/neo-planner_amd/csrc/neo_launch_opt.hpp
@@ -39,7 +39,16 @@
   const int n_launch = a.subset ? a.n_subset : a.B;
   const int *launch_order = a.subset ? a.subset : (c->order_B == a.B ? c->dispatch_order : nullptr);
   const OptLds l = opt_lds_plan<D, NS, Real, WAVES, LG, Num>(a.M, c->params.flags);
-  hipLaunchKernelGGL((optimize_kernel<D, NS, Real, MapT, LookupT, WAVES, LG, Num, BUDGET>), dim3(n_launch), dim3(kWave), l.dyn,
+  using Plan = opt_plan_t<NS, LG, Num, BUDGET>;
+  bool fixed = !Plan::dynamic;
+  if constexpr (!Plan::dynamic)
+    fixed = l.pcr_off != 0 && pcr_xch_elems(a.M, LG::dl(D)) * (int)sizeof(Num) <= l.stage * 8 && !c->trace && !c->trace_xg &&
+            !(c->params.flags & 4096);
+  auto kernel = optimize_kernel<D, NS, Real, MapT, LookupT, WAVES, LG, Num, BUDGET>;
+  if constexpr (!Plan::dynamic)
+    if (!fixed) kernel = optimize_dyn_kernel<D, NS, Real, MapT, LookupT, WAVES, LG, Num, BUDGET>;
+  ++c->opt_plan_launches[fixed ? 0 : 1];
+  hipLaunchKernelGGL(kernel, dim3(n_launch), dim3(kWave), l.dyn,
                      c->stream, n_launch, a.M, c->dev, static_cast<const MapT *>(a.table), a.slots, a.nmaps,
                      a.x0 ? a.x0 : a.x, a.x, a.head, a.tail, a.costs4, a.costs4_last, a.nit, a.nfev, a.status,
                      c->sample_counter, launch_order, c->trace, c->trace_xg, c->trace_cap, l.stage, l.pcr_off,
diff --git a/neo-planner_amd/neo_planner_amd/_lib.py b/neo-planner_amd/neo_planner_amd/_lib.py
--- a/neo-planner_amd/neo_planner_amd/_lib.py
+++ b/neo-planner_amd/neo_planner_amd/_lib.py
@@ -49,6 +49,7 @@
     "neo_plan_merge", "neo_plan_merge_dev", "neo_depth_render_batch", "neo_depth_render_batch_dev",
     "neo_depth_box_test_counter", "neo_onboard_integrate_batch", "neo_onboard_integrate_batch_dev",
     "neo_esdf_build_2d_batch_dev", "neo_fleet_pose_dev", "neo_record_state_dev", "neo_record_commit_dev",
+    "neo_optimize_plan_launches",
 ]
 
 
@@ -139,6 +140,7 @@
     L.neo_profile_enable.argtypes = [c_p, c_i]
     L.neo_profile_read.argtypes = [c_p, c_i, ctypes.POINTER(ctypes.c_int64), ctypes.POINTER(c_d)]
     L.neo_profile_reset.argtypes = [c_p]
+    L.neo_optimize_plan_launches.argtypes = [c_p, ctypes.POINTER(ctypes.c_int64), ctypes.POINTER(ctypes.c_int64)]
     L.neo_optimize_sample_counter.argtypes = [c_p, c_p]
     L.neo_optimize_trace.argtypes = [c_p, c_p, c_i]
     L.neo_optimize_trace_xg.argtypes = [c_p, c_p, c_i]
```

After: 1.536 million traj/s, median of 6. 1.02x the previous value.
